# MalvinaNikandrou/mafed

Measured on AMD Instinct MI355X. Metric: train samples/sec VLPythia-410M+MAFED, 256img+32txt tok, bs=32, 1/2/4/8 GPU, higher is better.
Workload: dtype bf16; 1 GPU; VLPythia-410m + MAFED distill step (student fwd+bwd, frozen-teacher fwd, replay CE, 23-layer per-modality MSE, clip 2.0, AdamW), 256 img + 32 txt tokens; global_batch=32, per_gpu_batch=32, seq_len=288, parallelism=dp1, random_init_weights=True

## Files before the change

### include/mafed_hip.h

```cpp
#ifndef MAFED_HIP_H
#define MAFED_HIP_H

#include <stddef.h>
#include <stdint.h>

#ifdef __cplusplus
extern "C" {
#endif

typedef enum { MAFED_F32 = 0, MAFED_BF16 = 1 } mafed_dtype;

enum {
  MAFED_OK = 0,
  MAFED_EINVAL = -1,
  MAFED_ELAUNCH = -2,
  MAFED_EWORKSPACE = -3
};

enum {
  MAFED_EPI_NONE = 0,
  MAFED_EPI_GELU = 1,
  MAFED_EPI_GELU_BWD = 2,
  MAFED_EPI_QUICK_GELU = 3,
  MAFED_EPI_RES1_BF16 = 0x100,
  MAFED_EPI_NO_PERSISTENT = 0x200,
  MAFED_EPI_TICKETED = 0x400
};

int mafed_version(void);
const char* mafed_last_error_string(void);

int mafed_gemm(mafed_dtype in_dtype, int transA, int transB, int64_t M, int64_t N, int64_t K,
               const void* A, int64_t lda, const void* B, int64_t ldb,
               void* C, int64_t ldc, mafed_dtype c_dtype,
               const float* bias, int epilogue, void* aux,
               const float* res1, const float* res2, float beta, void* stream);

int mafed_gemm_colsum(mafed_dtype in_dtype, int transA, int transB, int64_t M, int64_t N, int64_t K,
                      const void* A, int64_t lda, const void* B, int64_t ldb,
                      void* C, int64_t ldc, mafed_dtype c_dtype,
                      const float* bias, int epilogue, void* aux,
                      const float* res1, const float* res2, float beta, float* colsum, void* stream);

typedef struct mafed_gemm_problem {
  int64_t M, N, K;
  const void* A; int64_t lda;
  const void* B; int64_t ldb;
  void* C; int64_t ldc;
  const float* bias; int epilogue; void* aux;
  const float* res1; const float* res2; float beta; float* colsum;
  float* sumsq;
} mafed_gemm_problem;
int mafed_gemm_grouped(mafed_dtype in_dtype, int transA, int transB, mafed_dtype c_dtype,
                       const mafed_gemm_problem* problems, int n, void* stream);

size_t mafed_colsum_workspace_bytes(int64_t M, int64_t N);
int mafed_colsum(const void* X, mafed_dtype dtype, int64_t M, int64_t N, int64_t ldx, float* out,
                 void* workspace, size_t workspace_bytes, void* stream);

int mafed_layernorm_fwd(const float* x, int64_t rows, int h, float eps,
                        const float* w1, const float* b1, void* y1,
                        const float* w2, const float* b2, void* y2,
                        mafed_dtype out_dtype, float* mean, float* rstd, void* stream);
size_t mafed_layernorm_bwd_workspace_bytes(int64_t rows, int h);
int mafed_layernorm_bwd(const void* dy1, const void* dy2, mafed_dtype dy_dtype,
                        const float* x, const float* mean, const float* rstd,
                        const float* w1, const float* w2, int64_t rows, int h,
                        const float* dres, float* dx, void* dx_lp,
                        float* dw1, float* db1, float* dw2, float* db2,
                        const float* teacher, const int64_t* attention_mask, int S, int P, int T,
                        const float* inj_scale_dev , float inj_mul ,
                        float* dxsum_a, float* dxsum_b ,
                        void* workspace, size_t workspace_bytes, void* stream);
int mafed_layernorm_bwd_rows(const void* dy1, const void* dy2, mafed_dtype dy_dtype, const float* x, const float* mean, const float* rstd,
                             const float* w1, const float* w2, int64_t rows, int h, const float* dres, float* dx, void* dx_lp,
                             const float* teacher, const int64_t* attention_mask, int S, int P, int T, const float* inj_scale_dev,
                             float inj_mul, int want_dxsum, void* workspace, size_t workspace_bytes, void* stream);
int mafed_layernorm_bwd_params(int64_t rows, int h, float* dw1, float* db1, float* dw2, float* db2, float* dxsum_a, float* dxsum_b,
                               const void* workspace, size_t workspace_bytes, void* stream);
int mafed_layernorm_bwd_indexed(const void* dy1, const void* dy2, mafed_dtype dy_dtype,
                                const float* x, const float* mean, const float* rstd,
                                const float* w1, const float* w2, int64_t rows, int h,
                                const float* dres, float* dx, void* dx_lp,
                                float* dw1, float* db1, float* dw2, float* db2,
                                const void* teacher, mafed_dtype teacher_dtype, const int* sample_index,
                                const int64_t* attention_mask, int S, int P, int T,
                                const float* inj_scale_dev, float inj_mul, float* dxsum_a, float* dxsum_b,
                                void* workspace, size_t workspace_bytes, void* stream);
int mafed_layernorm_bwd_rows_indexed(const void* dy1, const void* dy2, mafed_dtype dy_dtype, const float* x, const float* mean,
                                     const float* rstd, const float* w1, const float* w2, int64_t rows, int h, const float* dres, float* dx,
                                     void* dx_lp, const void* teacher, mafed_dtype teacher_dtype, const int* sample_index,
                                     const int64_t* attention_mask, int S, int P, int T, const float* inj_scale_dev, float inj_mul,
                                     int want_dxsum, void* workspace, size_t workspace_bytes, void* stream);

int mafed_attn_fwd(const void* qkv, mafed_dtype dtype, int B, int S, int H, int D, int rot,
                   const float* rot_cos, const float* rot_sin, const int64_t* attention_mask, int T,
                   void* out, float* lse, void* stream);
int mafed_attn_bwd(const void* qkv, const void* out, const void* dout, const float* lse, mafed_dtype dtype,
                   int B, int S, int H, int D, int rot, const float* rot_cos, const float* rot_sin,
                   const int64_t* attention_mask, int T, void* dqkv, float* delta, void* stream);
int mafed_attn_bwd_colsum(const void* qkv, const void* out, const void* dout, const float* lse, mafed_dtype dtype,
                          int B, int S, int H, int D, int rot, const float* rot_cos, const float* rot_sin,
                          const int64_t* attention_mask, int T, void* dqkv, float* delta, float* dqkv_colsum, void* stream);

int mafed_attn_decode(const void* qkv_prefix, int S0, const void* qkv_new, int cap, int t, mafed_dtype dtype,
                      int B, int H, int D, int rot, const float* rot_cos, const float* rot_sin,
                      const int64_t* attention_mask, int T, void* out, void* stream);

int mafed_attn_decode_prerot(const void* qkv_prefix, int S0, void* qkv_new, int cap, int t, mafed_dtype dtype,
                             int B, int H, int D, int rot, const float* rot_cos, const float* rot_sin,
                             const int64_t* attention_mask, int T, void* out, void* stream);
int mafed_rotate_k_rows(void* qkv, mafed_dtype dtype, int B, int S, int H, int D, int rot, const float* rot_cos, const float* rot_sin,
                        void* stream);

int mafed_decode_supported(int M, int h, int n1);
int mafed_decode_ln_qkv_fc1(const float* x, int M, int h, float eps, const float* ln1_w, const float* ln1_b, const float* ln2_w,
                            const float* ln2_b, const void* wqkv, const float* bqkv, void* qkv_out, int64_t qkv_ld, const void* w1,
                            const float* b1, int n1, void* a_out, void* stream);
int mafed_decode_ln_linear(const float* x, int M, int h, float eps, const float* ln_w, const float* ln_b, const void* w, const float* bias,
                           int64_t N, void* out, int64_t ldo, void* stream);
size_t mafed_decode_out_workspace_bytes(int M, int h);
int mafed_decode_set_trace(void* buf);
int mafed_attn_decode_set_trace(void* buf);
int mafed_decode_out(const float* x, float* x_out, int M, int h, int n1, const void* ao, const void* act, const void* wd,
                     const float* bd, const void* w2, const float* b2, void* workspace, size_t workspace_bytes, void* stream);

int mafed_beam_candidates(const void* logits, mafed_dtype dtype, int64_t ldl, const float* score, int B, int kin, int V, int k,
                          float* out_score, int64_t* out_token, int* out_parent, void* stream);
int mafed_beam_update(const float* cand_score, const int64_t* cand_token, const int* cand_parent, int B, int k, int step, int cap,
                      int eos, int pad, int early_stopping, float length_penalty, float* run_score, const int* anc_in, int* anc_out,
                      const int64_t* hist_in, int64_t* hist_out, const int64_t* fin_tok_in, int64_t* fin_tok_out,
                      const float* fin_score_in, float* fin_score_out, const int* fin_len_in, int* fin_len_out, int* done,
                      int64_t* next_token, void* stream);
int mafed_attn_decode_beam(const void* qkv_prefix, int S0, void* qkv_new, int cap, int t, mafed_dtype dtype, int B, int k,
                           const int* anc, int H, int D, int rot, const float* rot_cos, const float* rot_sin,
                           const int64_t* attention_mask, int T, void* out, void* stream);

int mafed_attn_suffix_fwd(const void* qkv_img, const int64_t* image_index, int N, int P, const void* qkv_txt, int T, mafed_dtype dtype,
                          int B, int H, int D, int rot, const float* rot_cos, const float* rot_sin, const int64_t* attention_mask,
                          void* out, void* stream);
int mafed_prefix_gather(const void* qkv_img, const void* qkv_txt, const int64_t* image_index, int L, int N, int B, int P, int T, int64_t W,
                        mafed_dtype dtype, void* out, void* stream);

int mafed_attn_cand_fwd(const void* qkv_prefix, int S0, const void* qkv_cand, int C, int A, mafed_dtype dtype, int B, int H, int D, int rot,
                        const float* rot_cos, const float* rot_sin, const int64_t* attention_mask, int T, void* out, void* stream);
int mafed_token_logprob(const void* logits, mafed_dtype dtype, int64_t ldl, const int* logits_row, const int64_t* target, int R, int64_t V,
                        float* out, void* stream);
int mafed_score_reduce(const float* token_logprob, const int64_t* mask, int R, int A, int mean, float* out, void* stream);

int mafed_sample_token(const void* logits, mafed_dtype dtype, int64_t ldl, int R, int V, float temperature, int top_k, float top_p,
                       float min_p, const uint64_t* seed, int step, const float* uniforms, int64_t* unfinished, int eos, int pad,
                       int64_t* token, float* logprob, int* kept, void* stream);

size_t mafed_ewc_workspace_bytes(int64_t n);
int mafed_ewc_penalty_fwd(const float* p, const float* p_old, const float* fisher, int64_t n, float half_lambda, float beta,
                          float* out, void* workspace, size_t workspace_bytes, void* stream);
int mafed_ewc_penalty_bwd(const float* p, const float* p_old, const float* fisher, int64_t n, float lambda,
                          const float* coef_dev, float* grad, void* stream);

size_t mafed_agem_workspace_bytes(int64_t n);
int mafed_agem_blocks(int64_t n);
int mafed_agem_dots(const float* g, const float* r, int64_t n, float* stats4, void* workspace, size_t workspace_bytes, void* stream);
int mafed_agem_project(const float* g, const float* r, float* out, int64_t n, const float* stats4, float* sumsq_partials, void* stream);

int mafed_cka_pool(const float* const* hidden_host, int L, int B, int S, int P, int h, const int64_t* attention_mask, int T,
                   const int64_t* rows, int64_t n, float* out, void* stream);

size_t mafed_cka_stats_workspace_bytes(int64_t G, int64_t n, int64_t h);
int mafed_cka_stats(const float* X, int64_t G, int64_t n, int64_t h, int64_t ldx, int64_t set_stride, double* mean,
                    double* row_sqnorm, void* workspace, size_t workspace_bytes, void* stream);

typedef struct mafed_cka_product {
  const float* X; const double* mean_x; int64_t ldx; int64_t hx;
  const float* Y; const double* mean_y; int64_t ldy; int64_t hy;
  int64_t n;
} mafed_cka_product;

size_t mafed_cka_hsic_workspace_bytes(const mafed_cka_product* products, int count);
int mafed_cka_hsic(const mafed_cka_product* products, int count, double* out, void* workspace, size_t workspace_bytes, void* stream);

int mafed_embed_concat_fwd(const void* image, mafed_dtype img_dtype, const float* embed_in, const int64_t* input_ids,
                           int B, int P, int T, int h, int64_t V, float* h0, void* stream);
int mafed_embed_concat_bwd(const float* dh0, const int64_t* input_ids, int B, int P, int T, int h, int64_t V,
                           void* d_image, mafed_dtype img_dtype, float* d_embed_in, void* stream);

int mafed_ce_fwd(const void* logits, mafed_dtype dtype, const int64_t* labels, int B, int T, int64_t V,
                 float* lse, float* row_loss , float* loss_out, void* stream);
int mafed_ce_fwd_guarded(const void* logits, mafed_dtype dtype, const int64_t* labels, int B, int T, int64_t V,
                         float* lse, float* row_loss, float* loss_out, const int* poison_flag, void* stream);
int mafed_ce_bwd(const void* logits, mafed_dtype dtype, const int64_t* labels, const float* lse, int B, int T, int64_t V,
                 const float* gloss_dev, void* dlogits, void* stream);

int mafed_ce_kd_fwd(const void* student, const void* teacher, mafed_dtype dtype, const int64_t* labels, int B, int T, int64_t V,
                    float tau, float lambda, float* lse3, float* row_ce, float* row_kd, float* out3, const int* poison_flag,
                    void* stream);
int mafed_ce_kd_bwd(const void* student, const void* teacher, mafed_dtype dtype, const int64_t* labels, const float* lse3, int B, int T,
                    int64_t V, float tau, float lambda, const float* gloss_dev, void* dlogits, void* stream);

size_t mafed_distill_workspace_bytes(int64_t rows);
int mafed_distill_fwd(const float* s, const float* t, const int64_t* attention_mask, int B, int S, int P, int h,
                      int cosine, float* out4, void* workspace, size_t workspace_bytes, void* stream);
int mafed_distill_bwd(const float* s, const float* t, const int64_t* attention_mask, int B, int S, int P, int h,
                      int cosine, const float* coef_dev, float* ds, int accumulate, void* stream);
int mafed_distill_combine(const float* sums, int n_layers, const float* layer_coeff_dev, int modality_mode, float lang_weight,
                          const float* lang_weight_vec_dev, float* loss_out, float* per_layer_out, float* modality_out,
                          float* inject_out, void* stream);

int mafed_distill_cls_fwd(const float* s, const float* t, int B, int S, int h, float* out1, void* stream);
int mafed_distill_cls_bwd(const float* s, const float* t, int B, int S, int h, const float* coef_dev, float* ds,
                          int accumulate, void* stream);
int mafed_distill_fwd_indexed(const float* s, const void* teacher, mafed_dtype teacher_dtype, const int* sample_index,
                              const int64_t* attention_mask, int B, int S, int P, int h, int cosine, float* out4,
                              void* workspace, size_t workspace_bytes, void* stream);
int mafed_distill_bwd_indexed(const float* s, const void* teacher, mafed_dtype teacher_dtype, const int* sample_index,
                              const int64_t* attention_mask, int B, int S, int P, int h, int cosine, const float* coef_dev,
                              float* ds, int accumulate, void* stream);
int mafed_distill_cls_fwd_indexed(const float* s, const void* teacher, mafed_dtype teacher_dtype, const int* sample_index,
                                  int B, int S, int h, float* out1, void* stream);
int mafed_distill_cls_bwd_indexed(const float* s, const void* teacher, mafed_dtype teacher_dtype, const int* sample_index,
                                  int B, int S, int h, const float* coef_dev, float* ds, int accumulate, void* stream);

size_t mafed_gradnorm_workspace_bytes(int64_t n);
int mafed_gradnorm_clip(const float* g, int64_t n, float max_norm, float* out2, void* workspace, size_t workspace_bytes,
                        void* stream);
int mafed_gradnorm_blocks(int64_t n);
int mafed_gradnorm_partial(const float* g, int64_t n, float* partial_out, void* stream);
int mafed_gradnorm_finish(const float* partial, int n_partials, float max_norm, float* out2, void* stream);
int mafed_adamw_step(float* p, const float* g, float* m, float* v, int64_t n, const float* lr_dev, float beta1, float beta2,
                     float eps, float weight_decay, int step, const float* clip_dev ,
                     float grad_mul, void* p_bf16, void* stream);

int mafed_adamw_step_zero_grad(float* p, float* g, float* m, float* v, int64_t n, const float* lr_dev, float beta1, float beta2,
                               float eps, float weight_decay, int step, const float* clip_scale_dev, float grad_mul, void* p_bf16,
                               void* stream);

int mafed_adamw_step_partial_zero(float* p, float* g, float* m, float* v, int64_t n, const float* lr_dev, float beta1, float beta2,
                                  float eps, float weight_decay, int step, const float* clip_scale_dev, float grad_mul, void* p_bf16,
                                  int64_t zero_n, void* stream);

int mafed_adam_step(float* p, float* g, float* m, float* v, int64_t n, const float* lr_dev, double beta1, double beta2, float eps,
                    float weight_decay, int step, const float* clip_dev, float grad_mul, void* p_bf16, int64_t zero_n, void* stream);
int mafed_adamax_step(float* p, float* g, float* m, float* u, int64_t n, const float* lr_dev, double beta1, double beta2, float eps,
                      float weight_decay, int step, const float* clip_dev, float grad_mul, void* p_bf16, int64_t zero_n, void* stream);

int mafed_optim_advance(int64_t* state_dev, double base_lr, int64_t warmup_steps, int64_t total_steps, double beta1, double beta2,
                        float* hyper3_dev, void* stream);

int mafed_optim_advance_guarded(int64_t* state_dev, double base_lr, int64_t warmup_steps, int64_t total_steps, double beta1, double beta2,
                                float* hyper3_dev, const float* clip_dev, void* stream);

int mafed_sumsq_accumulate(const float* x, int64_t n, float* sumsq16, void* stream);
int mafed_gemm_grouped_fuses_sumsq(mafed_dtype in_dtype, int transA, int transB, mafed_dtype c_dtype, const int64_t* M, const int64_t* N,
                                   const int64_t* K, int n);

int mafed_gradnorm_finish_advance(const float* partial, int n_partials, float max_norm, float* out2, float* norm_log, int64_t* state_dev,
                                  double base_lr, int64_t warmup_steps, int64_t total_steps, double beta1, double beta2, float* hyper3_dev,
                                  void* stream);

int mafed_cast(const void* src, mafed_dtype src_dtype, void* dst, mafed_dtype dst_dtype, int64_t n, void* stream);
int mafed_pad_text_rows(const float* src, int B, int S, int P, int h, float* dst, void* dst_lp, void* stream);
int mafed_label_rows(const int64_t* labels, int B, int T, int Rc, int* row_of_slot, int* slot_of_row, int64_t* labels_c, int* overflow,
                     void* stream);
int mafed_gather_rows(const void* src, mafed_dtype dtype, const int* idx, int64_t n_out, int h, void* dst, void* stream);
int mafed_pad_text_batch(const int64_t* ids, const int64_t* mask, const int64_t* labels, int B, int T, int Tp, int64_t* ids_out,
                         int64_t* mask_out, int64_t* labels_out, void* stream);
int mafed_gelu(const void* x, void* y, mafed_dtype dtype, int64_t n, void* stream);

int mafed_patchify(const void* pixels, mafed_dtype pix_dtype, int B, int C, int H, int W, int patch, int64_t rows_out, int k_pad,
                   void* out, mafed_dtype out_dtype, void* stream);
int mafed_vit_assemble(const void* patch_emb, mafed_dtype pe_dtype, int64_t ld_pe, const float* class_embedding,
                       const float* position_embedding, int B, int num_patches, int h, float* tokens, void* stream);
int mafed_attn_fwd_bidir(const void* qkv, mafed_dtype dtype, int B, int S, int H, int D, void* out, float* lse, void* stream);

int mafed_prof_begin(int max_records);
int mafed_prof_end(void);
int mafed_prof_collect(int* tags_host, double* work_host, float* ms_host, float* start_ms_host, int max);
const char* mafed_prof_tag_name(int tag);

int mafed_gemm_set_variant(int variant);
int mafed_gemm_get_variant(int which);
int mafed_gemm_pp_launches(void);
int mafed_gemm_fallback_launches(void);

int mafed_attn_set_variant(int variant);

int mafed_attn_fwd_exact_bf16(const void* qkv, int B, int S, int H, int D, int rot, const float* rot_cos, const float* rot_sin,
                              const int64_t* attention_mask, int T, void* out, float* lse, void* stream);

int mafed_tune_occupy(int blocks, int lds_bytes, long long cycles, void* stream);

int mafed_tune_stream(const void* src, void* dst, long long n_bytes, int blocks, int threads, int unroll, int mode, void* stream);
int mafed_tune_stream_for(const void* src, void* dst, long long n_bytes, int blocks, int threads, double microseconds, void* stream);

#ifdef __cplusplus
}
#endif
#endif
```

### mafed_amd/_lib.py

```python
from __future__ import annotations

import ctypes as C
import os
from typing import Optional

_HERE = os.path.dirname(os.path.abspath(__file__))
LIB_PATH = os.environ.get("MAFED_HIP_LIB") or os.path.join(_HERE, "libmafed_hip.so")

F32, BF16 = 0, 1
EPI_NONE, EPI_GELU, EPI_GELU_BWD, EPI_QUICK_GELU = 0, 1, 2, 3
EPI_RES1_BF16 = 0x100
EPI_NO_PERSISTENT = 0x200
EPI_TICKETED = 0x400

_p, _i, _l, _f, _z, _d = C.c_void_p, C.c_int, C.c_int64, C.c_float, C.c_size_t, C.c_double

SIGNATURES = {
    "mafed_version": (_i, []),
    "mafed_last_error_string": (C.c_char_p, []),
    "mafed_gemm": (_i, [_i, _i, _i, _l, _l, _l, _p, _l, _p, _l, _p, _l, _i, _p, _i, _p, _p, _p, _f, _p]),
    "mafed_gemm_colsum": (_i, [_i, _i, _i, _l, _l, _l, _p, _l, _p, _l, _p, _l, _i, _p, _i, _p, _p, _p, _f, _p, _p]),
    "mafed_gemm_grouped": (_i, [_i, _i, _i, _i, _p, _i, _p]),
    "mafed_gemm_set_variant": (_i, [_i]),
    "mafed_gemm_get_variant": (_i, [_i]),
    "mafed_gemm_pp_launches": (_i, []),
    "mafed_gemm_fallback_launches": (_i, []),
    "mafed_attn_decode": (_i, [_p, _i, _p, _i, _i, _i, _i, _i, _i, _i, _p, _p, _p, _i, _p, _p]),
    "mafed_attn_decode_prerot": (_i, [_p, _i, _p, _i, _i, _i, _i, _i, _i, _i, _p, _p, _p, _i, _p, _p]),
    "mafed_rotate_k_rows": (_i, [_p, _i, _i, _i, _i, _i, _i, _p, _p, _p]),
    "mafed_gemm_grouped_fuses_sumsq": (_i, [_i, _i, _i, _i, _p, _p, _p, _i]),
    "mafed_decode_supported": (_i, [_i, _i, _i]),
    "mafed_decode_ln_qkv_fc1": (_i, [_p, _i, _i, _f, _p, _p, _p, _p, _p, _p, _p, _l, _p, _p, _i, _p, _p]),
    "mafed_decode_ln_linear": (_i, [_p, _i, _i, _f, _p, _p, _p, _p, _l, _p, _l, _p]),
    "mafed_decode_out_workspace_bytes": (_z, [_i, _i]),
    "mafed_decode_set_trace": (_i, [_p]),
    "mafed_attn_decode_set_trace": (_i, [_p]),
    "mafed_decode_out": (_i, [_p, _p, _i, _i, _i, _p, _p, _p, _p, _p, _p, _p, _z, _p]),
    "mafed_beam_candidates": (_i, [_p, _i, _l, _p, _i, _i, _i, _i, _p, _p, _p, _p]),
    "mafed_beam_update": (_i, [_p, _p, _p, _i, _i, _i, _i, _i, _i, _i, _f, _p, _p, _p, _p, _p, _p, _p, _p, _p, _p, _p, _p, _p, _p]),
    "mafed_attn_decode_beam": (_i, [_p, _i, _p, _i, _i, _i, _i, _i, _p, _i, _i, _i, _p, _p, _p, _i, _p, _p]),
    "mafed_attn_suffix_fwd": (_i, [_p, _p, _i, _i, _p, _i, _i, _i, _i, _i, _i, _p, _p, _p, _p, _p]),
    "mafed_prefix_gather": (_i, [_p, _p, _p, _i, _i, _i, _i, _i, _l, _i, _p, _p]),
    "mafed_attn_cand_fwd": (_i, [_p, _i, _p, _i, _i, _i, _i, _i, _i, _i, _p, _p, _p, _i, _p, _p]),
    "mafed_token_logprob": (_i, [_p, _i, _l, _p, _p, _i, _l, _p, _p]),
    "mafed_score_reduce": (_i, [_p, _p, _i, _i, _i, _p, _p]),
    "mafed_sample_token": (_i, [_p, _i, _l, _i, _i, _f, _i, _f, _f, _p, _i, _p, _p, _i, _i, _p, _p, _p, _p]),
    "mafed_ewc_workspace_bytes": (_z, [_l]),
    "mafed_ewc_penalty_fwd": (_i, [_p, _p, _p, _l, _f, _f, _p, _p, _z, _p]),
    "mafed_ewc_penalty_bwd": (_i, [_p, _p, _p, _l, _f, _p, _p, _p]),
    "mafed_agem_workspace_bytes": (_z, [_l]),
    "mafed_agem_blocks": (_i, [_l]),
    "mafed_agem_dots": (_i, [_p, _p, _l, _p, _p, _z, _p]),
    "mafed_agem_project": (_i, [_p, _p, _p, _l, _p, _p, _p]),
    "mafed_cka_pool": (_i, [_p, _i, _i, _i, _i, _i, _p, _i, _p, _l, _p, _p]),
    "mafed_cka_stats_workspace_bytes": (_z, [_l, _l, _l]),
    "mafed_cka_stats": (_i, [_p, _l, _l, _l, _l, _l, _p, _p, _p, _z, _p]),
    "mafed_cka_hsic_workspace_bytes": (_z, [_p, _i]),
    "mafed_cka_hsic": (_i, [_p, _i, _p, _p, _z, _p]),
    "mafed_colsum_workspace_bytes": (_z, [_l, _l]),
    "mafed_colsum": (_i, [_p, _i, _l, _l, _l, _p, _p, _z, _p]),
    "mafed_layernorm_fwd": (_i, [_p, _l, _i, _f, _p, _p, _p, _p, _p, _p, _i, _p, _p, _p]),
    "mafed_layernorm_bwd_workspace_bytes": (_z, [_l, _i]),
    "mafed_layernorm_bwd": (_i, [_p, _p, _i, _p, _p, _p, _p, _p, _l, _i, _p, _p, _p, _p, _p, _p, _p, _p, _p, _i, _i, _i, _p, _f, _p, _p, _p, _z, _p]),
    "mafed_layernorm_bwd_rows": (_i, [_p, _p, _i, _p, _p, _p, _p, _p, _l, _i, _p, _p, _p, _p, _p, _i, _i, _i, _p, _f, _i, _p, _z, _p]),
    "mafed_layernorm_bwd_params": (_i, [_l, _i, _p, _p, _p, _p, _p, _p, _p, _z, _p]),
    "mafed_layernorm_bwd_indexed": (_i, [_p, _p, _i, _p, _p, _p, _p, _p, _l, _i, _p, _p, _p, _p, _p, _p, _p, _p, _i, _p, _p, _i, _i, _i, _p, _f, _p, _p,
                                         _p, _z, _p]),
    "mafed_layernorm_bwd_rows_indexed": (_i, [_p, _p, _i, _p, _p, _p, _p, _p, _l, _i, _p, _p, _p, _p, _i, _p, _p, _i, _i, _i, _p, _f, _i, _p, _z, _p]),
    "mafed_attn_fwd": (_i, [_p, _i, _i, _i, _i, _i, _i, _p, _p, _p, _i, _p, _p, _p]),
    "mafed_attn_bwd": (_i, [_p, _p, _p, _p, _i, _i, _i, _i, _i, _i, _p, _p, _p, _i, _p, _p, _p]),
    "mafed_attn_bwd_colsum": (_i, [_p, _p, _p, _p, _i, _i, _i, _i, _i, _i, _p, _p, _p, _i, _p, _p, _p, _p]),
    "mafed_attn_set_variant": (_i, [_i]),
    "mafed_attn_fwd_exact_bf16": (_i, [_p, _i, _i, _i, _i, _i, _p, _p, _p, _i, _p, _p, _p]),
    "mafed_embed_concat_fwd": (_i, [_p, _i, _p, _p, _i, _i, _i, _i, _l, _p, _p]),
    "mafed_embed_concat_bwd": (_i, [_p, _p, _i, _i, _i, _i, _l, _p, _i, _p, _p]),
    "mafed_ce_fwd": (_i, [_p, _i, _p, _i, _i, _l, _p, _p, _p, _p]),
    "mafed_ce_fwd_guarded": (_i, [_p, _i, _p, _i, _i, _l, _p, _p, _p, _p, _p]),
    "mafed_ce_bwd": (_i, [_p, _i, _p, _p, _i, _i, _l, _p, _p, _p]),
    "mafed_ce_kd_fwd": (_i, [_p, _p, _i, _p, _i, _i, _l, _f, _f, _p, _p, _p, _p, _p, _p]),
    "mafed_ce_kd_bwd": (_i, [_p, _p, _i, _p, _p, _i, _i, _l, _f, _f, _p, _p, _p]),
    "mafed_distill_workspace_bytes": (_z, [_l]),
    "mafed_distill_fwd": (_i, [_p, _p, _p, _i, _i, _i, _i, _i, _p, _p, _z, _p]),
    "mafed_distill_bwd": (_i, [_p, _p, _p, _i, _i, _i, _i, _i, _p, _p, _i, _p]),
    "mafed_distill_cls_fwd": (_i, [_p, _p, _i, _i, _i, _p, _p]),
    "mafed_distill_cls_bwd": (_i, [_p, _p, _i, _i, _i, _p, _p, _i, _p]),
    "mafed_distill_fwd_indexed": (_i, [_p, _p, _i, _p, _p, _i, _i, _i, _i, _i, _p, _p, _z, _p]),
    "mafed_distill_bwd_indexed": (_i, [_p, _p, _i, _p, _p, _i, _i, _i, _i, _i, _p, _p, _i, _p]),
    "mafed_distill_cls_fwd_indexed": (_i, [_p, _p, _i, _p, _i, _i, _i, _p, _p]),
    "mafed_distill_cls_bwd_indexed": (_i, [_p, _p, _i, _p, _i, _i, _i, _p, _p, _i, _p]),
    "mafed_gradnorm_workspace_bytes": (_z, [_l]),
    "mafed_gradnorm_clip": (_i, [_p, _l, _f, _p, _p, _z, _p]),
    "mafed_gradnorm_blocks": (_i, [_l]),
    "mafed_gradnorm_partial": (_i, [_p, _l, _p, _p]),
    "mafed_gradnorm_finish": (_i, [_p, _i, _f, _p, _p]),
    "mafed_sumsq_accumulate": (_i, [_p, _l, _p, _p]),
    "mafed_adamw_step": (_i, [_p, _p, _p, _p, _l, _p, _f, _f, _f, _f, _i, _p, _f, _p, _p]),
    "mafed_adamw_step_zero_grad": (_i, [_p, _p, _p, _p, _l, _p, _f, _f, _f, _f, _i, _p, _f, _p, _p]),
    "mafed_adamw_step_partial_zero": (_i, [_p, _p, _p, _p, _l, _p, _f, _f, _f, _f, _i, _p, _f, _p, _l, _p]),
    "mafed_adam_step": (_i, [_p, _p, _p, _p, _l, _p, _d, _d, _f, _f, _i, _p, _f, _p, _l, _p]),
    "mafed_adamax_step": (_i, [_p, _p, _p, _p, _l, _p, _d, _d, _f, _f, _i, _p, _f, _p, _l, _p]),
    "mafed_distill_combine": (_i, [_p, _i, _p, _i, _f, _p, _p, _p, _p, _p, _p]),
    "mafed_optim_advance": (_i, [_p, _d, _l, _l, _d, _d, _p, _p]),
    "mafed_optim_advance_guarded": (_i, [_p, _d, _l, _l, _d, _d, _p, _p, _p]),
    "mafed_tune_occupy": (_i, [_i, _i, C.c_longlong, _p]),
    "mafed_tune_stream": (_i, [_p, _p, C.c_longlong, _i, _i, _i, _i, _p]),
    "mafed_tune_stream_for": (_i, [_p, _p, C.c_longlong, _i, _i, _d, _p]),
    "mafed_gradnorm_finish_advance": (_i, [_p, _i, _f, _p, _p, _p, _d, _l, _l, _d, _d, _p, _p]),
    "mafed_cast": (_i, [_p, _i, _p, _i, _l, _p]),
    "mafed_pad_text_rows": (_i, [_p, _i, _i, _i, _i, _p, _p, _p]),
    "mafed_label_rows": (_i, [_p, _i, _i, _i, _p, _p, _p, _p, _p]),
    "mafed_gather_rows": (_i, [_p, _i, _p, _l, _i, _p, _p]),
    "mafed_pad_text_batch": (_i, [_p, _p, _p, _i, _i, _i, _p, _p, _p, _p]),
    "mafed_gelu": (_i, [_p, _p, _i, _l, _p]),
    "mafed_patchify": (_i, [_p, _i, _i, _i, _i, _i, _i, _l, _i, _p, _i, _p]),
    "mafed_vit_assemble": (_i, [_p, _i, _l, _p, _p, _i, _i, _i, _p, _p]),
    "mafed_attn_fwd_bidir": (_i, [_p, _i, _i, _i, _i, _i, _p, _p, _p]),
    "mafed_prof_begin": (_i, [_i]),
    "mafed_prof_end": (_i, []),
    "mafed_prof_collect": (_i, [_p, _p, _p, _p, _i]),
    "mafed_prof_tag_name": (C.c_char_p, [_i]),
}



class GemmProblem(C.Structure):
    _fields_ = [("M", _l), ("N", _l), ("K", _l), ("A", _p), ("lda", _l), ("B", _p), ("ldb", _l), ("C", _p), ("ldc", _l),
                ("bias", _p), ("epilogue", _i), ("aux", _p), ("res1", _p), ("res2", _p), ("beta", _f), ("colsum", _p), ("sumsq", _p)]


class CkaProduct(C.Structure):
    _fields_ = [("X", _p), ("mean_x", _p), ("ldx", _l), ("hx", _l), ("Y", _p), ("mean_y", _p), ("ldy", _l), ("hy", _l), ("n", _l)]


_lib: Optional[C.CDLL] = None


class MafedHipError(RuntimeError):
    pass


def load() -> C.CDLL:
    global _lib
    if _lib is not None:
        return _lib
    if not os.path.exists(LIB_PATH):
        raise MafedHipError(
            f"{LIB_PATH} is missing: build it with `python -m mafed_amd.build` (or __graft_entry__.build()). "
            "mafed_amd has no CPU fallback.")
    lib = C.CDLL(LIB_PATH)
    loose = bool(os.environ.get("MAFED_HIP_LIB")) and os.environ.get("MAFED_HIP_LIB_LOOSE") == "1"
    for name, (res, args) in SIGNATURES.items():
        if loose and not hasattr(lib, name):
            continue
        fn = getattr(lib, name)
        fn.restype = res
        fn.argtypes = args
    _lib = lib
    return lib


def check(rc: int, what: str = "") -> None:
    if rc != 0:
        msg = load().mafed_last_error_string()
        raise MafedHipError(f"{what or 'mafed call'} failed (rc={rc}): {msg.decode() if msg else ''}")
```

### mafed_amd/csrc/attn.h

```cpp
#pragma once
#include "common.h"

namespace mafed {

struct AttnShape {
  int B, S, H, D, rot, T, P;
  int causal = 1;
};

template <typename T>
__device__ __forceinline__ float rot_elem(const T* __restrict__ row, int d, int rot, const float* __restrict__ c, const float* __restrict__ s) {
  const float x = Elem<T>::load(row + d);
  if (d >= rot) return x;
  const int half = rot >> 1;
  if (d < half) return x * c[d] - Elem<T>::load(row + d + half) * s[d];
  return x * c[d - half] + Elem<T>::load(row + d - half) * s[d - half];
}
__device__ __forceinline__ bool key_valid(const int64_t* __restrict__ am, int b, int j, int P, int T) {
  return j < P || am[(int64_t)b * T + (j - P)] != 0;
}

template <typename T>
struct AttnKey {
  const T* row;
  int pos;
  bool visible;
};
template <typename T, typename Key>
__device__ __forceinline__ void attn_exact_row(const float* __restrict__ qrow, float* __restrict__ sc, int nk, int D, int rot,
                                               const float* __restrict__ rc, const float* __restrict__ rs, Key key, T* __restrict__ op,
                                               int lane, float& m, float& l) {
  const int half = rot >> 1;
  const float scale = rsqrtf((float)D);
  m = -INFINITY;
  for (int k = lane; k < nk; k += 64) {
    float s = -INFINITY;
    const AttnKey<T> kk = key(k);
    if (kk.visible) {
      float acc = 0.f;
      for (int d = 0; d < D; ++d)
        acc = fmaf(qrow[d], rot_elem(kk.row + D, d, rot, rc + (int64_t)kk.pos * half, rs + (int64_t)kk.pos * half), acc);
      s = acc * scale;
    }
    sc[k] = s;
    m = fmaxf(m, s);
  }
  m = wave_max(m);
  l = 0.f;
  for (int k = lane; k < nk; k += 64) {
    const float p = expf(sc[k] - m);
    sc[k] = p;
    l += p;
  }
  l = wave_sum(l);
  __builtin_amdgcn_wave_barrier();
  const float inv = 1.0f / l;
  for (int d = lane; d < D; d += 64) {
    float acc = 0.f;
    for (int k = 0; k < nk; ++k) acc = fmaf(sc[k], Elem<T>::load(key(k).row + 2 * D + d), acc);
    Elem<T>::store(op + d, acc * inv);
  }
}

template <typename T>
int attn_ref_fwd_launch(const void* qkv, const AttnShape& sh, const float* rc, const float* rs, const int64_t* am, void* out, float* lse,
                        hipStream_t st);
template <typename T>
int attn_ref_bwd_launch(const void* qkv, const void* out, const void* dout, const float* lse, const AttnShape& sh, const float* rc,
                        const float* rs, const int64_t* am, void* dqkv, float* delta, hipStream_t st);

template <typename T>
int attn_decode_launch(const void* qkv_pre, int S0, const void* qkv_new, int cap, int t, int B, int H, int D, int rot, int P, int Tm,
                       const float* rc, const float* rs, const int64_t* am, void* out, hipStream_t st, bool prerot = false);
template <typename T>
int rotate_k_rows_launch(void* qkv, int64_t rows, int S, int H, int D, int rot, const float* rc, const float* rs, hipStream_t st);

int attn_mfma_fwd_launch(const void* qkv, const AttnShape& sh, const float* rc, const float* rs, const int64_t* am, void* out, float* lse,
                         hipStream_t st);
int attn_mfma_bwd_launch(const void* qkv, const void* out, const void* dout, const float* lse, const AttnShape& sh, const float* rc,
                         const float* rs, const int64_t* am, void* dqkv, float* delta, float* colsum, bool* colsum_done, hipStream_t st);

struct SuffixShape {
  int B, N, P, T, H, D, rot;
};
__device__ __forceinline__ int64_t suffix_image(const int64_t* __restrict__ image_index, int b, int N) {
  const int64_t n = image_index ? image_index[b] : (int64_t)b;
  return n < 0 ? 0 : (n >= N ? N - 1 : n);
}
template <typename T>
int attn_suffix_ref_launch(const void* qkv_img, const int64_t* image_index, const void* qkv_txt, const SuffixShape& sh, const float* rc,
                           const float* rs, const int64_t* am, void* out, hipStream_t st);
int attn_suffix_mfma_launch(const void* qkv_img, const int64_t* image_index, const void* qkv_txt, const SuffixShape& sh, const float* rc,
                            const float* rs, const int64_t* am, void* out, hipStream_t st);
int prefix_gather_launch(const void* img, const void* txt, const int64_t* image_index, int L, int N, int B, int P, int T, int64_t row_bytes,
                         void* out, hipStream_t st);

struct CandShape {
  int B, C, A, S0, T, H, D, rot;
};
template <typename T>
int attn_cand_ref_launch(const void* qkv_pre, const void* qkv_cand, const CandShape& sh, const float* rc, const float* rs, const int64_t* am,
                         void* out, hipStream_t st);
int attn_cand_mfma_launch(const void* qkv_pre, const void* qkv_cand, const CandShape& sh, const float* rc, const float* rs, const int64_t* am,
                          void* out, hipStream_t st);

void attn_mfma_set_variant(int v);

int attn_decode_set_trace(void* buf);

}
```

### mafed_amd/csrc/attn.hip

```cpp
#include "attn.h"

using namespace mafed;

static int check_common(const char* who, const void* qkv, int B, int S, int H, int D, int rot, const float* rc, const float* rs,
                        const int64_t* am, int T) {
  MAFED_CHECK_ARG(qkv && am, "%s: null pointer", who);
  MAFED_CHECK_ARG(B > 0 && S > 0 && H > 0 && D > 0 && T >= 0 && T <= S, "%s: bad shape B=%d S=%d H=%d D=%d T=%d", who, B, S, H, D, T);
  MAFED_CHECK_ARG(rot >= 0 && rot <= D && rot % 2 == 0, "%s: rotary dims %d invalid for D=%d", who, rot, D);
  MAFED_CHECK_ARG(rot == 0 || (rc && rs), "%s: rotary tables missing", who);
  return MAFED_OK;
}

static bool mfma_ok(int D, int rot) { return (D == 64 || D == 128 || D == 256) && (rot == 0 || rot == 16 || rot == 32 || rot == 64) && rot * 2 <= D * 2; }

extern "C" int mafed_attn_fwd(const void* qkv, mafed_dtype dtype, int B, int S, int H, int D, int rot, const float* rot_cos,
                              const float* rot_sin, const int64_t* attention_mask, int T, void* out, float* lse, void* stream) {
  int rc = check_common("attn_fwd", qkv, B, S, H, D, rot, rot_cos, rot_sin, attention_mask, T);
  if (rc) return rc;
  MAFED_CHECK_ARG(out && lse, "attn_fwd: null output");
  AttnShape sh{B, S, H, D, rot, T, S - T};
  hipStream_t st = as_stream(stream);
  if (dtype == MAFED_F32) {
    MAFED_CHECK_ARG(D <= 256, "attn_fwd(f32): D=%d > 256", D);
    rc = attn_ref_fwd_launch<float>(qkv, sh, rot_cos, rot_sin, attention_mask, out, lse, st);
// ... 10 lines not shown
}

extern "C" int mafed_attn_suffix_fwd(const void* qkv_img, const int64_t* image_index, int N, int P, const void* qkv_txt, int T,
                                     mafed_dtype dtype, int B, int H, int D, int rot, const float* rot_cos, const float* rot_sin,
                                     const int64_t* attention_mask, void* out, void* stream) {
  MAFED_CHECK_ARG(qkv_img && qkv_txt && attention_mask && out, "attn_suffix_fwd: null pointer");
  MAFED_CHECK_ARG(B > 0 && N > 0 && P > 0 && T > 0 && H > 0 && D > 0 && D <= 256, "attn_suffix_fwd: bad shape B=%d N=%d P=%d T=%d H=%d D=%d", B, N,
                  P, T, H, D);
  MAFED_CHECK_ARG(image_index || N == B, "attn_suffix_fwd: no image_index needs N == B (N=%d B=%d)", N, B);
  MAFED_CHECK_ARG(rot >= 0 && rot <= D && rot % 2 == 0 && (rot == 0 || (rot_cos && rot_sin)), "attn_suffix_fwd: rotary arguments invalid");
  SuffixShape sh{B, N, P, T, H, D, rot};
  hipStream_t st = as_stream(stream);
  int rc;
  if (dtype == MAFED_F32) {
    rc = attn_suffix_ref_launch<float>(qkv_img, image_index, qkv_txt, sh, rot_cos, rot_sin, attention_mask, out, st);
  } else if (mfma_ok(D, rot)) {
    MAFED_CHECK_ARG((((uintptr_t)qkv_img | (uintptr_t)qkv_txt | (uintptr_t)out) & 15) == 0, "attn_suffix_fwd(bf16): qkv/out must be 16-byte aligned");
    rc = attn_suffix_mfma_launch(qkv_img, image_index, qkv_txt, sh, rot_cos, rot_sin, attention_mask, out, st);
  } else {
    rc = attn_suffix_ref_launch<bf16_t>(qkv_img, image_index, qkv_txt, sh, rot_cos, rot_sin, attention_mask, out, st);
  }
  if (rc) return rc;
  MAFED_CHECK_LAUNCH("attn_suffix_fwd");
  return MAFED_OK;
}

extern "C" int mafed_attn_cand_fwd(const void* qkv_prefix, int S0, const void* qkv_cand, int C, int A, mafed_dtype dtype, int B, int H, int D,
                                   int rot, const float* rot_cos, const float* rot_sin, const int64_t* attention_mask, int T, void* out,
                                   void* stream) {
  MAFED_CHECK_ARG(qkv_prefix && qkv_cand && out, "attn_cand_fwd: null pointer");
  MAFED_CHECK_ARG(B > 0 && C > 0 && A > 0 && H > 0 && D > 0 && D <= 256 && (int64_t)C * A <= 0x7fffffffLL,
                  "attn_cand_fwd: bad shape B=%d C=%d A=%d H=%d D=%d", B, C, A, H, D);
  MAFED_CHECK_ARG(S0 > 0 && T >= 0 && T < S0, "attn_cand_fwd: the prefix needs an image key in front of its text (S0=%d T=%d)", S0, T);
  MAFED_CHECK_ARG(attention_mask || T == 0, "attn_cand_fwd: attention_mask missing (T=%d)", T);
  MAFED_CHECK_ARG(rot >= 0 && rot <= D && rot % 2 == 0 && (rot == 0 || (rot_cos && rot_sin)), "attn_cand_fwd: rotary arguments invalid");
  CandShape sh{B, C, A, S0, T, H, D, rot};
  hipStream_t st = as_stream(stream);
  int rc;
  if (dtype == MAFED_F32) {
    rc = attn_cand_ref_launch<float>(qkv_prefix, qkv_cand, sh, rot_cos, rot_sin, attention_mask, out, st);
  } else if (mfma_ok(D, rot) && (((uintptr_t)qkv_prefix | (uintptr_t)qkv_cand | (uintptr_t)out) & 15) == 0) {
    rc = attn_cand_mfma_launch(qkv_prefix, qkv_cand, sh, rot_cos, rot_sin, attention_mask, out, st);
  } else {
    rc = attn_cand_ref_launch<bf16_t>(qkv_prefix, qkv_cand, sh, rot_cos, rot_sin, attention_mask, out, st);
  }
  if (rc) return rc;
  MAFED_CHECK_LAUNCH("attn_cand_fwd");
  return MAFED_OK;
}

extern "C" int mafed_prefix_gather(const void* qkv_img, const void* qkv_txt, const int64_t* image_index, int L, int N, int B, int P, int T,
                                   int64_t W, mafed_dtype dtype, void* out, void* stream) {
  MAFED_CHECK_ARG(qkv_img && qkv_txt && out, "prefix_gather: null pointer");
  MAFED_CHECK_ARG(L > 0 && N > 0 && B > 0 && P > 0 && T > 0 && W > 0, "prefix_gather: bad shape L=%d N=%d B=%d P=%d T=%d", L, N, B, P, T);
  MAFED_CHECK_ARG(image_index || N == B, "prefix_gather: no image_index needs N == B (N=%d B=%d)", N, B);
  MAFED_CHECK_ARG((((uintptr_t)qkv_img | (uintptr_t)qkv_txt | (uintptr_t)out) & 15) == 0, "prefix_gather: tensors must be 16-byte aligned");
  int rc = prefix_gather_launch(qkv_img, qkv_txt, image_index, L, N, B, P, T, W * (dtype == MAFED_F32 ? 4 : 2), out, as_stream(stream));
  if (rc) return rc;
  MAFED_CHECK_LAUNCH("prefix_gather");
  return MAFED_OK;
}

extern "C" int mafed_attn_fwd_bidir(const void* qkv, mafed_dtype dtype, int B, int S, int H, int D, void* out, float* lse, void* stream) {
  MAFED_CHECK_ARG(qkv && out && lse, "attn_fwd_bidir: null pointer");
  MAFED_CHECK_ARG(B > 0 && S > 0 && H > 0 && D > 0 && D <= 256, "attn_fwd_bidir: bad shape B=%d S=%d H=%d D=%d", B, S, H, D);
  AttnShape sh{B, S, H, D, 0, 0, S};
  sh.causal = 0;
  const int64_t* dummy_mask = reinterpret_cast<const int64_t*>(qkv);
  hipStream_t st = as_stream(stream);
  int rc;
  if (dtype == MAFED_F32) {
    rc = attn_ref_fwd_launch<float>(qkv, sh, nullptr, nullptr, dummy_mask, out, lse, st);
  } else {
    MAFED_CHECK_ARG((((uintptr_t)qkv | (uintptr_t)out) & 15) == 0, "attn_fwd_bidir(bf16): qkv/out must be 16-byte aligned");
    rc = attn_mfma_fwd_launch(qkv, sh, nullptr, nullptr, dummy_mask, out, lse, st);
  }
  if (rc) return rc;
  MAFED_CHECK_LAUNCH("attn_fwd_bidir");
  return MAFED_OK;
}

static int attn_bwd_impl(const void* qkv, const void* out, const void* dout, const float* lse, mafed_dtype dtype, int B, int S, int H,
                         int D, int rot, const float* rot_cos, const float* rot_sin, const int64_t* attention_mask, int T, void* dqkv,
                         float* delta, float* dqkv_colsum, void* stream);

extern "C" int mafed_attn_bwd(const void* qkv, const void* out, const void* dout, const float* lse, mafed_dtype dtype, int B, int S, int H,
                              int D, int rot, const float* rot_cos, const float* rot_sin, const int64_t* attention_mask, int T, void* dqkv,
                              float* delta, void* stream) {
  return attn_bwd_impl(qkv, out, dout, lse, dtype, B, S, H, D, rot, rot_cos, rot_sin, attention_mask, T, dqkv, delta, nullptr, stream);
}

extern "C" int mafed_attn_bwd_colsum(const void* qkv, const void* out, const void* dout, const float* lse, mafed_dtype dtype, int B, int S,
                                     int H, int D, int rot, const float* rot_cos, const float* rot_sin, const int64_t* attention_mask, int T,
                                     void* dqkv, float* delta, float* dqkv_colsum, void* stream) {
  return attn_bwd_impl(qkv, out, dout, lse, dtype, B, S, H, D, rot, rot_cos, rot_sin, attention_mask, T, dqkv, delta, dqkv_colsum, stream);
}

static int attn_bwd_impl(const void* qkv, const void* out, const void* dout, const float* lse, mafed_dtype dtype, int B, int S, int H,
                         int D, int rot, const float* rot_cos, const float* rot_sin, const int64_t* attention_mask, int T, void* dqkv,
                         float* delta, float* dqkv_colsum, void* stream) {
  int rc = check_common("attn_bwd", qkv, B, S, H, D, rot, rot_cos, rot_sin, attention_mask, T);
  if (rc) return rc;
  MAFED_CHECK_ARG(out && dout && lse && dqkv && delta, "attn_bwd: null pointer");
  AttnShape sh{B, S, H, D, rot, T, S - T};
  hipStream_t st = as_stream(stream);
  bool colsum_done = false;
  if (dtype == MAFED_F32) {
    MAFED_CHECK_ARG(D <= 256, "attn_bwd(f32): D=%d > 256", D);
    rc = attn_ref_bwd_launch<float>(qkv, out, dout, lse, sh, rot_cos, rot_sin, attention_mask, dqkv, delta, st);
  } else if (mfma_ok(D, rot)) {
    MAFED_CHECK_ARG((((uintptr_t)qkv | (uintptr_t)out | (uintptr_t)dout | (uintptr_t)dqkv) & 15) == 0,
                    "attn_bwd(bf16): tensors must be 16-byte aligned");
    rc = attn_mfma_bwd_launch(qkv, out, dout, lse, sh, rot_cos, rot_sin, attention_mask, dqkv, delta, dqkv_colsum, &colsum_done, st);
  } else {
    MAFED_CHECK_ARG(D <= 256, "attn_bwd(bf16): D=%d > 256", D);
    rc = attn_ref_bwd_launch<bf16_t>(qkv, out, dout, lse, sh, rot_cos, rot_sin, attention_mask, dqkv, delta, st);
  }
  if (rc) return rc;
  MAFED_CHECK_LAUNCH("attn_bwd");
  if (dqkv_colsum && !colsum_done)
    return mafed_colsum(dqkv, dtype, (int64_t)B * S, (int64_t)3 * H * D, (int64_t)3 * H * D, dqkv_colsum, nullptr, 0, stream);
  return MAFED_OK;
}

extern "C" int mafed_attn_set_variant(int variant) {
  attn_mfma_set_variant(variant);
  return MAFED_OK;
}

extern "C" int mafed_attn_fwd_exact_bf16(const void* qkv, int B, int S, int H, int D, int rot, const float* rot_cos, const float* rot_sin,
                                         const int64_t* attention_mask, int T, void* out, float* lse, void* stream) {
  int rc = check_common("attn_fwd_exact_bf16", qkv, B, S, H, D, rot, rot_cos, rot_sin, attention_mask, T);
  if (rc) return rc;
  AttnShape sh{B, S, H, D, rot, T, S - T};
  rc = attn_ref_fwd_launch<bf16_t>(qkv, sh, rot_cos, rot_sin, attention_mask, out, lse, as_stream(stream));
  if (rc) return rc;
  MAFED_CHECK_LAUNCH("attn_fwd_exact_bf16");
  return MAFED_OK;
}

static int attn_decode_impl(const void* qkv_prefix, int S0, const void* qkv_new, int cap, int t, mafed_dtype dtype, int B, int H, int D,
                            int rot, const float* rot_cos, const float* rot_sin, const int64_t* attention_mask, int T, void* out,
                            void* stream, bool prerot) {
  MAFED_CHECK_ARG(qkv_prefix && qkv_new && out && attention_mask, "attn_decode: null pointer");
  MAFED_CHECK_ARG(B > 0 && H > 0 && D > 0 && D <= 256 && S0 > 0 && T >= 0 && T <= S0 && cap > 0 && t >= 0 && t < cap,
                  "attn_decode: bad shape B=%d H=%d D=%d S0=%d T=%d cap=%d t=%d", B, H, D, S0, T, cap, t);
  MAFED_CHECK_ARG(rot >= 0 && rot <= D && rot % 2 == 0 && (rot == 0 || (rot_cos && rot_sin)), "attn_decode: rotary arguments invalid");
  hipStream_t st = as_stream(stream);
  int rc = dtype == MAFED_F32 ? attn_decode_launch<float>(qkv_prefix, S0, qkv_new, cap, t, B, H, D, rot, S0 - T, T, rot_cos, rot_sin, attention_mask, out, st, prerot)
                              : attn_decode_launch<bf16_t>(qkv_prefix, S0, qkv_new, cap, t, B, H, D, rot, S0 - T, T, rot_cos, rot_sin, attention_mask, out, st, prerot);
  if (rc) return rc;
  MAFED_CHECK_LAUNCH("attn_decode");
  return MAFED_OK;
}

extern "C" int mafed_attn_decode(const void* qkv_prefix, int S0, const void* qkv_new, int cap, int t, mafed_dtype dtype, int B, int H, int D,
                                 int rot, const float* rot_cos, const float* rot_sin, const int64_t* attention_mask, int T, void* out,
                                 void* stream) {
  return attn_decode_impl(qkv_prefix, S0, qkv_new, cap, t, dtype, B, H, D, rot, rot_cos, rot_sin, attention_mask, T, out, stream, false);
}

extern "C" int mafed_attn_decode_prerot(const void* qkv_prefix, int S0, void* qkv_new, int cap, int t, mafed_dtype dtype, int B, int H, int D,
                                        int rot, const float* rot_cos, const float* rot_sin, const int64_t* attention_mask, int T, void* out,
                                        void* stream) {
  MAFED_CHECK_ARG(rot % 16 == 0 && (D == 64 || D == 128 || D == 256), "attn_decode_prerot: needs rot %% 16 == 0 and a head size of 64 / 128 / 256");
  return attn_decode_impl(qkv_prefix, S0, qkv_new, cap, t, dtype, B, H, D, rot, rot_cos, rot_sin, attention_mask, T, out, stream, true);
}

extern "C" int mafed_rotate_k_rows(void* qkv, mafed_dtype dtype, int B, int S, int H, int D, int rot, const float* rot_cos, const float* rot_sin,
                                   void* stream) {
  MAFED_CHECK_ARG(qkv && B > 0 && S > 0 && H > 0 && D > 0 && rot >= 0 && rot <= D && rot % 16 == 0 && (rot == 0 || (rot_cos && rot_sin)),
                  "rotate_k_rows: bad arguments");
  hipStream_t st = as_stream(stream);
  int rc = dtype == MAFED_F32 ? rotate_k_rows_launch<float>(qkv, (int64_t)B * S, S, H, D, rot, rot_cos, rot_sin, st)
                              : rotate_k_rows_launch<bf16_t>(qkv, (int64_t)B * S, S, H, D, rot, rot_cos, rot_sin, st);
  if (rc) return rc;
  MAFED_CHECK_LAUNCH("rotate_k_rows");
  return MAFED_OK;
}

extern "C" int mafed_attn_decode_set_trace(void* buf) { return mafed::attn_decode_set_trace(buf); }
```

### mafed_amd/csrc/attn_mfma.hip

```cpp
#include <type_traits>

#include "attn.h"
#include "row8.h"

namespace mafed {

namespace {

typedef __attribute__((address_space(3))) bf16x4* lds_bf16x4_ptr;

template <int D>
__device__ __forceinline__ int swz(int row) {
  if (D == 64) return ((row >> 1) & 3) << 1;
  if (D == 128) return (row & 7) << 1;
  return ((row & 7) << 1) | ((row >> 3) & 1);
}
template <int D>
__device__ __forceinline__ int tile_off(int row, int chunk) {
  if (D == 64) return row * 128 + ((chunk ^ swz<64>(row)) << 4);
  if (D == 128) return row * 256 + ((chunk ^ swz<128>(row)) << 4);
  return row * 512 + ((chunk ^ (((row & 7) << 1) | ((row >> 3) & 1))) << 4);
}

__device__ __forceinline__ uint4 load_chunk_rot(const bf16_t* __restrict__ rowp, int chunk, int rot, const float* __restrict__ rc,
// ... 494 lines not shown
  const int k0 = kt * 64 + wave * 16;
  const int mykey = k0 + (lane & 15);
  const int g = lane >> 4;
  const bool mykey_ok = key_ok(am, b, mykey, P, T, S);

  bf16x8 kf[D / 32], vf[D / 32];
  load_col_frags<D, true>(kf, kb, rstride, k0, S, rot, rc, rs, lane);
  load_col_frags<D, false>(vf, vb, rstride, k0, S, 0, rc, rs, lane);
  f32x4 dk[D / 16], dv[D / 16];
#pragma unroll
  for (int i = 0; i < D / 16; ++i) { dk[i] = (f32x4){0.f, 0.f, 0.f, 0.f}; dv[i] = (f32x4){0.f, 0.f, 0.f, 0.f}; }
  const float scale = rsqrtf((float)D);
  const int64_t lbase = ((int64_t)b * H + h) * S;

  for (int qt = kt; qt < nqt; ++qt) {
    __syncthreads();
    stage_rows<D, 64, true>(qimg, qb, rstride, qt * 64, S, rot, rc, rs, tid);
    stage_rows<D, 64, false>(doimg, dob, ostride, qt * 64, S, 0, rc, rs, tid);
    if (tid < 64) {
      const int q = qt * 64 + tid;
      Ls[tid] = q < S ? lse[lbase + q] : 0.f;
      dls[tid] = q < S ? delta[lbase + q] : 0.f;
    }
    __syncthreads();
    f32x4 p[4], ds[4];
#pragma unroll
    for (int j = 0; j < 4; ++j) {
      f32x4 s = (f32x4){0.f, 0.f, 0.f, 0.f}, dp = (f32x4){0.f, 0.f, 0.f, 0.f};
#pragma unroll
      for (int ks = 0; ks < D / 32; ++ks) {
        s = __builtin_amdgcn_mfma_f32_16x16x32_bf16(frag_row<D>(qimg, j, ks, lane), kf[ks], s, 0, 0, 0);
        dp = __builtin_amdgcn_mfma_f32_16x16x32_bf16(frag_row<D>(doimg, j, ks, lane), vf[ks], dp, 0, 0, 0);
      }
      const float4 Lq = *reinterpret_cast<const float4*>(Ls + j * 16 + 4 * g);
      const float4 Dq = *reinterpret_cast<const float4*>(dls + j * 16 + 4 * g);
      const float La[4] = {Lq.x, Lq.y, Lq.z, Lq.w}, Da[4] = {Dq.x, Dq.y, Dq.z, Dq.w};
#pragma unroll
      for (int r = 0; r < 4; ++r) {
        const int q = qt * 64 + j * 16 + 4 * g + r;
        float pv = __expf(s[r] * scale - La[r]);
        if (!mykey_ok || mykey > q || q >= S) pv = 0.f;
        p[j][r] = pv;
        ds[j][r] = pv * (dp[r] - Da[r]) * scale;
      }
    }
    const bf16x8 p0 = pack_acc(p[0], p[1]), p1 = pack_acc(p[2], p[3]);
    const bf16x8 d0 = pack_acc(ds[0], ds[1]), d1 = pack_acc(ds[2], ds[3]);
#pragma unroll
    for (int dt = 0; dt < D / 16; ++dt) {
      dv[dt] = __builtin_amdgcn_mfma_f32_16x16x32_bf16(frag_tr<D>(doimg, dt, 0, lane), p0, dv[dt], 0, 0, 0);
      dv[dt] = __builtin_amdgcn_mfma_f32_16x16x32_bf16(frag_tr<D>(doimg, dt, 1, lane), p1, dv[dt], 0, 0, 0);
      dk[dt] = __builtin_amdgcn_mfma_f32_16x16x32_bf16(frag_tr<D>(qimg, dt, 0, lane), d0, dk[dt], 0, 0, 0);
      dk[dt] = __builtin_amdgcn_mfma_f32_16x16x32_bf16(frag_tr<D>(qimg, dt, 1, lane), d1, dk[dt], 0, 0, 0);
    }
  }
  bf16_t* dkp = dqkv + ((int64_t)b * S * H + h) * 3 * D + (int64_t)mykey * rstride + D;
  store_grad_unrot<D>(dkp, dk, rot, rc, rs, mykey, lane, mykey < S);
  if (mykey < S) {
    bf16_t* dvp = dkp + D;
#pragma unroll
    for (int dt = 0; dt < D / 16; ++dt) store4(dvp + dt * 16 + 4 * g, make_float4(dv[dt][0], dv[dt][1], dv[dt][2], dv[dt][3]));
  }
}

typedef __attribute__((address_space(3))) void* lds_void_ptr;
typedef const __attribute__((address_space(1))) void* glb_void_ptr;
typedef unsigned u32x2 __attribute__((ext_vector_type(2)));

__device__ __forceinline__ float col_max_sw(float v) {
  u32x2 r = __builtin_amdgcn_permlane32_swap(__float_as_uint(v), __float_as_uint(v), false, false);
  v = fmaxf(__uint_as_float(r[0]), __uint_as_float(r[1]));
  r = __builtin_amdgcn_permlane16_swap(__float_as_uint(v), __float_as_uint(v), false, false);
  return fmaxf(__uint_as_float(r[0]), __uint_as_float(r[1]));
}
__device__ __forceinline__ float col_sum_sw(float v) {
  u32x2 r = __builtin_amdgcn_permlane32_swap(__float_as_uint(v), __float_as_uint(v), false, false);
  v = __uint_as_float(r[0]) + __uint_as_float(r[1]);
  r = __builtin_amdgcn_permlane16_swap(__float_as_uint(v), __float_as_uint(v), false, false);
  return __uint_as_float(r[0]) + __uint_as_float(r[1]);
}

template <int D, int NW = 4>
__device__ __forceinline__ void dma_rows(char* __restrict__ img, const bf16_t* __restrict__ base, int64_t rstride, int nrows, int S, int wave,
                                         int lane) {
  constexpr int RPP = 1024 / (2 * D);
  const int npieces = nrows / RPP;
  for (int j = wave; j < npieces; j += NW) {
    int row, logical;
    if (D == 64) {
      row = j * 8 + (lane >> 3);
      logical = (lane & 7) ^ swz<64>(row);
    } else {
      row = j * 4 + (lane >> 4);
      logical = (lane & 15) ^ swz<128>(row);
    }
    const int srow = row < S ? row : S - 1;
    __builtin_amdgcn_global_load_lds((glb_void_ptr)(base + (int64_t)srow * rstride + logical * 8), (lds_void_ptr)(img + j * 1024), 16, 0, 0);
  }
}

struct RotPre {
  float4 c0, c1, s0, s1;
};
__device__ __forceinline__ void rot_pre_load(RotPre& r, int it, int hc, int rot, const float* __restrict__ rc, const float* __restrict__ rs) {
  const int row = it / hc, c = it - row * hc;
  const float* cp = rc + (int64_t)row * (rot >> 1) + c * 8;
  const float* sp = rs + (int64_t)row * (rot >> 1) + c * 8;
  r.c0 = load4(cp); r.c1 = load4(cp + 4); r.s0 = load4(sp); r.s1 = load4(sp + 4);
}
template <int D>
__device__ __forceinline__ void rot_apply(char* __restrict__ img, int it, int hc, const RotPre& r) {
  const int row = it / hc, c = it - row * hc;
  uint4* p1 = reinterpret_cast<uint4*>(img + tile_off<D>(row, c));
  uint4* p2 = reinterpret_cast<uint4*>(img + tile_off<D>(row, c + hc));
  float x1[8], x2[8], o1[8], o2[8];
  unpack8(*p1, x1);
  unpack8(*p2, x2);
  const float cs[8] = {r.c0.x, r.c0.y, r.c0.z, r.c0.w, r.c1.x, r.c1.y, r.c1.z, r.c1.w};
  const float sn[8] = {r.s0.x, r.s0.y, r.s0.z, r.s0.w, r.s1.x, r.s1.y, r.s1.z, r.s1.w};
#pragma unroll
  for (int e = 0; e < 8; ++e) {
    o1[e] = x1[e] * cs[e] - x2[e] * sn[e];
    o2[e] = x2[e] * cs[e] + x1[e] * sn[e];
  }
  *p1 = pack8(o1);
  *p2 = pack8(o2);
}
template <int D, int NT = 256>
__device__ __forceinline__ void rot_fix_rows(char* __restrict__ img, int items, int hc, int rot, const float* __restrict__ rc,
                                             const float* __restrict__ rs, const RotPre (&pre)[2], int tid) {
#pragma unroll
  for (int u = 0; u < 2; ++u)
    if (tid + NT * u < items) rot_apply<D>(img, tid + NT * u, hc, pre[u]);
  for (int it = tid + 2 * NT; it < items; it += NT) {
    RotPre r;
    rot_pre_load(r, it, hc, rot, rc, rs);
    rot_apply<D>(img, it, hc, r);
  }
}

__device__ __forceinline__ float row16_sum(float v) {
  v += __builtin_bit_cast(float, __builtin_amdgcn_update_dpp(0, __builtin_bit_cast(int, v), 0xB1, 0xF, 0xF, true));
  v += __builtin_bit_cast(float, __builtin_amdgcn_update_dpp(0, __builtin_bit_cast(int, v), 0x4E, 0xF, 0xF, true));
  v += __builtin_bit_cast(float, __builtin_amdgcn_update_dpp(0, __builtin_bit_cast(int, v), 0x141, 0xF, 0xF, true));
  v += __builtin_bit_cast(float, __builtin_amdgcn_update_dpp(0, __builtin_bit_cast(int, v), 0x140, 0xF, 0xF, true));
  return v;
}

__device__ __forceinline__ void wait_vm0() { asm volatile("s_waitcnt vmcnt(0)" ::: "memory"); }

__device__ __forceinline__ int snake4(int w, int t) { return t * 4 + ((t & 1) ? 3 - w : w); }
template <int NW>
__device__ __forceinline__ int snake(int w, int t) { return t * NW + ((t & 1) ? NW - 1 - w : w); }

#define MAFED_LOG2E 1.4426950408889634f
#define MAFED_LN2 0.6931471805599453f

template <int D>
constexpr int attn_fwd_waves() { return D == 64 ? 8 : 4; }

template <int D, bool CAUSAL = true>
__global__ __launch_bounds__(attn_fwd_waves<D>() * 64, (D == 64 ? 2 : 1) * attn_fwd_waves<D>() / 4) void attn_fwd_res_kernel(const bf16_t* __restrict__ qkv, AttnShape sh, const float* __restrict__ rc,
                                                           const float* __restrict__ rs, const int64_t* __restrict__ am,
                                                           bf16_t* __restrict__ out, float* __restrict__ lse) {
  extern __shared__ __attribute__((aligned(16))) char lds[];
  constexpr int NW = attn_fwd_waves<D>(), NTH = NW * 64;
  const int tid = threadIdx.x, lane = tid & 63;
  const int wave = __builtin_amdgcn_readfirstlane(tid >> 6);
  const int S = sh.S, H = sh.H, rot = sh.rot, P = sh.P, T = sh.T;
  const int h = blockIdx.x, b = blockIdx.y;
  const int nrows = (S + 31) / 32 * 32;
  char* kimg = lds;
  char* vimg = lds + nrows * D * 2;
  float* kbias = reinterpret_cast<float*>(lds + 2 * nrows * D * 2);
  const int64_t rstride = (int64_t)H * 3 * D;
  const bf16_t* qb = qkv + ((int64_t)b * S * H + h) * 3 * D;
  const bf16_t* kb = qb + D;
  const bf16_t* vb = qb + 2 * D;
  const int nslices = (S + 15) / 16;
// ... 48 lines not shown
      constexpr bool MASK = decltype(mask_tag)::value;
      f32x4 s[4];
#pragma unroll
      for (int j = 0; j < 4; ++j) {
        s[j] = (f32x4){0.f, 0.f, 0.f, 0.f};
        if (!MASK || j < nj) {
#pragma unroll
          for (int ks = 0; ks < D / 32; ++ks)
            s[j] = __builtin_amdgcn_mfma_f32_16x16x32_bf16(frag_row<D>(kimg, kt * 4 + j, ks, lane), qf[ks], s[j], 0, 0, 0);
        }
      }
      float tmax = -INFINITY;
      if (MASK) {
#pragma unroll
        for (int j = 0; j < 4; ++j) {
          if (j < nj) {
            const float4 kb4 = *reinterpret_cast<const float4*>(kbias + kt * 64 + j * 16 + 4 * g);
            const float kbv[4] = {kb4.x, kb4.y, kb4.z, kb4.w};
#pragma unroll
            for (int r = 0; r < 4; ++r) {
              const int key = kt * 64 + j * 16 + 4 * g + r;
              float v = s[j][r] * scale2 + kbv[r];
              if (CAUSAL) v = key > myq ? -INFINITY : v;
              s[j][r] = v;
              tmax = fmaxf(tmax, v);
            }
          } else {
            s[j] = (f32x4){-INFINITY, -INFINITY, -INFINITY, -INFINITY};
          }
        }
      } else {
#pragma unroll
        for (int j = 0; j < 4; ++j)
#pragma unroll
          for (int r = 0; r < 4; ++r) tmax = fmaxf(tmax, s[j][r]);
        tmax *= scale2;
      }
      tmax = col_max_sw(tmax);
      if (__builtin_amdgcn_ballot_w64(tmax - m > 8.0f) != 0) {
        const float mn = fmaxf(m, tmax);
        const float alpha = __builtin_amdgcn_exp2f(m - mn);
        m = mn;
        lsum *= alpha;
#pragma unroll
        for (int i = 0; i < D / 16; ++i) o[i] *= alpha;
      }
#pragma unroll
      for (int j = 0; j < 4; ++j)
#pragma unroll
        for (int r = 0; r < 4; ++r) s[j][r] = __builtin_amdgcn_exp2f(MASK ? s[j][r] - m : fmaf(s[j][r], scale2, -m));
      const bf16x8 p0 = pack_acc(s[0], s[1]);
      lsum = __builtin_amdgcn_mfma_f32_16x16x32_bf16(ones, p0, lsum, 0, 0, 0);
#pragma unroll
      for (int dt = 0; dt < D / 16; ++dt) o[dt] = __builtin_amdgcn_mfma_f32_16x16x32_bf16(frag_tr<D>(vimg, dt, kt * 2, lane), p0, o[dt], 0, 0, 0);
      if (!MASK || nj > 2) {
        const bf16x8 p1 = pack_acc(s[2], s[3]);
        lsum = __builtin_amdgcn_mfma_f32_16x16x32_bf16(ones, p1, lsum, 0, 0, 0);
#pragma unroll
        for (int dt = 0; dt < D / 16; ++dt)
          o[dt] = __builtin_amdgcn_mfma_f32_16x16x32_bf16(frag_tr<D>(vimg, dt, kt * 2 + 1, lane), p1, o[dt], 0, 0, 0);
      }
    };
    const int kt_plain = CAUSAL ? (last_kt < P / 64 ? last_kt : P / 64) : (P / 64 <= last_kt ? P / 64 : last_kt + 1);
    const int klast = CAUSAL ? q0 + 15 : S - 1;
    for (int kt = 0; kt < kt_plain; ++kt) tile(kt, 4, std::false_type{});
    for (int kt = kt_plain; kt <= last_kt; ++kt) tile(kt, kt == last_kt ? ((klast - kt * 64) >> 4) + 1 : 4, std::true_type{});
    const float l = lsum[0];
    if (myq < S) {
      const float inv = 1.0f / l;
      bf16_t* op = out + ((int64_t)b * S + myq) * H * D + (int64_t)h * D;
#pragma unroll
      for (int dt = 0; dt < D / 16; ++dt)
        store4(op + dt * 16 + 4 * g, make_float4(o[dt][0] * inv, o[dt][1] * inv, o[dt][2] * inv, o[dt][3] * inv));
      if (g == 0) lse[((int64_t)b * H + h) * S + myq] = m * MAFED_LN2 + logf(l);
    }
  }
}

template <int D, int NW = 4>
__global__ __launch_bounds__(NW * 64, (D == 64 ? 2 : 1) * NW / 4) void attn_bwd_dq_res_kernel(const bf16_t* __restrict__ qkv, const bf16_t* __restrict__ out,
                                                              const bf16_t* __restrict__ dout, const float* __restrict__ lse, AttnShape sh,
                                                              const float* __restrict__ rc, const float* __restrict__ rs,
                                                              const int64_t* __restrict__ am, bf16_t* __restrict__ dqkv,
                                                              float* __restrict__ delta, float* __restrict__ bsum) {
  extern __shared__ __attribute__((aligned(16))) char lds[];
  constexpr int NTH = NW * 64;
  const int tid = threadIdx.x, lane = tid & 63;
  const int wave = __builtin_amdgcn_readfirstlane(tid >> 6);
  const int S = sh.S, H = sh.H, rot = sh.rot, P = sh.P, T = sh.T;
  const int h = blockIdx.x, b = blockIdx.y;
  const int nrows = (S + 31) / 32 * 32;
  char* kimg = lds;
  char* vimg = lds + nrows * D * 2;
  float* kbias = reinterpret_cast<float*>(lds + 2 * nrows * D * 2);
  float* red = kbias + 2 * nrows;
  if (bsum && tid < D) red[tid] = 0.f;
  const int64_t rstride = (int64_t)H * 3 * D;
  const bf16_t* qb = qkv + ((int64_t)b * S * H + h) * 3 * D;
  const bf16_t* kb = qb + D;
  const bf16_t* vb = qb + 2 * D;
  const int64_t ostride = (int64_t)H * D;
  const bf16_t* ob = out + (int64_t)b * S * ostride + (int64_t)h * D;
  const bf16_t* dob = dout + (int64_t)b * S * ostride + (int64_t)h * D;
  const float* Lrow = lse + ((int64_t)b * H + h) * S;
  const int nslices = (S + 15) / 16;
  const int hc = rot >> 4, items = S * hc;
  dma_rows<D, NW>(kimg, kb, rstride, nrows, S, wave, lane);
  dma_rows<D, NW>(vimg, vb, rstride, nrows, S, wave, lane);
  RotPre pre[2];
#pragma unroll
  for (int u = 0; u < 2; ++u)
    if (tid + NTH * u < items) rot_pre_load(pre[u], tid + NTH * u, hc, rot, rc, rs);
  for (int k = tid; k < nrows; k += NTH) kbias[k] = key_ok(am, b, k, P, T, S) ? 0.f : -INFINITY;
  constexpr bool PREFETCH = NW == 4;
  ColRaw<D> qraw, doraw, oraw;
  float Lnext = 0.f;
  if (PREFETCH) {
    const int s0 = nslices - 1 - snake<NW>(wave, 0);
    if (s0 >= 0) {
      col_raw_issue<D, true>(qraw, qb, rstride, s0 * 16, S, rot, rc, rs, lane);
      col_raw_issue<D, false>(doraw, dob, ostride, s0 * 16, S, 0, rc, rs, lane);
      col_raw_issue<D, false>(oraw, ob, ostride, s0 * 16, S, 0, rc, rs, lane);
      const int q = s0 * 16 + (lane & 15);
      Lnext = q < S ? Lrow[q] : 0.f;
    }
  }
  wait_vm0();
  __syncthreads();
  rot_fix_rows<D, NTH>(kimg, items, hc, rot, rc, rs, pre, tid);
  __syncthreads();
  const int g = lane >> 4;
  const float scale = rsqrtf((float)D);
  const float scale2 = scale * MAFED_LOG2E;
  for (int t = 0;; ++t) {
    const int slice = nslices - 1 - snake<NW>(wave, t);
    if (slice < 0) break;
    const int q0 = slice * 16;
    const int myq = q0 + (lane & 15);
    if (!PREFETCH) {
      col_raw_issue<D, true>(qraw, qb, rstride, q0, S, rot, rc, rs, lane);
      col_raw_issue<D, false>(doraw, dob, ostride, q0, S, 0, rc, rs, lane);
      col_raw_issue<D, false>(oraw, ob, ostride, q0, S, 0, rc, rs, lane);
      Lnext = myq < S ? Lrow[myq] : 0.f;
    }
    bf16x8 qf[D / 32], dof[D / 32];
    col_raw_finish<D, true>(qf, qraw, q0, S, rot, lane);
    col_raw_finish<D, false>(dof, doraw, q0, S, 0, lane);
    const float L2 = Lnext * MAFED_LOG2E;
    float dl = 0.f;
    {
      bf16x8 of[D / 32];
      col_raw_finish<D, false>(of, oraw, q0, S, 0, lane);
      const int nxt = nslices - 1 - snake<NW>(wave, t + 1);
      if (PREFETCH && nxt >= 0) {
        col_raw_issue<D, true>(qraw, qb, rstride, nxt * 16, S, rot, rc, rs, lane);
        col_raw_issue<D, false>(doraw, dob, ostride, nxt * 16, S, 0, rc, rs, lane);
        col_raw_issue<D, false>(oraw, ob, ostride, nxt * 16, S, 0, rc, rs, lane);
        const int q = nxt * 16 + (lane & 15);
        Lnext = q < S ? Lrow[q] : 0.f;
      }
#pragma unroll
      for (int ks = 0; ks < D / 32; ++ks)
#pragma unroll
        for (int e = 0; e < 8; ++e) dl += (float)dof[ks][e] * (float)of[ks][e];
      dl = col_sum_sw(dl);
    }
    if (myq < S && g == 0) delta[((int64_t)b * H + h) * S + myq] = dl;
    f32x4 dq[D / 16];
#pragma unroll
    for (int i = 0; i < D / 16; ++i) dq[i] = (f32x4){0.f, 0.f, 0.f, 0.f};
    const int last_kt = (q0 + 15) / 64;
    auto tile = [&](const int kt, const int nj, auto mask_tag) {
      constexpr bool MASK = decltype(mask_tag)::value;
      f32x4 ds[4];
#pragma unroll
      for (int j = 0; j < 4; ++j) {
        ds[j] = (f32x4){0.f, 0.f, 0.f, 0.f};
        if (!MASK || j < nj) {
          f32x4 s = (f32x4){0.f, 0.f, 0.f, 0.f}, dp = (f32x4){0.f, 0.f, 0.f, 0.f};
#pragma unroll
          for (int ks = 0; ks < D / 32; ++ks) {
            s = __builtin_amdgcn_mfma_f32_16x16x32_bf16(frag_row<D>(kimg, kt * 4 + j, ks, lane), qf[ks], s, 0, 0, 0);
            dp = __builtin_amdgcn_mfma_f32_16x16x32_bf16(frag_row<D>(vimg, kt * 4 + j, ks, lane), dof[ks], dp, 0, 0, 0);
          }
          if (MASK) {
            const float4 kb4 = *reinterpret_cast<const float4*>(kbias + kt * 64 + j * 16 + 4 * g);
            const float kbv[4] = {kb4.x, kb4.y, kb4.z, kb4.w};
#pragma unroll
            for (int r = 0; r < 4; ++r) {
              const int key = kt * 64 + j * 16 + 4 * g + r;
              float x = s[r] * scale2 - L2 + kbv[r];
              x = key > myq ? -INFINITY : x;
              ds[j][r] = __builtin_amdgcn_exp2f(x) * (dp[r] - dl) * scale;
            }
          } else {
#pragma unroll
            for (int r = 0; r < 4; ++r) ds[j][r] = __builtin_amdgcn_exp2f(s[r] * scale2 - L2) * (dp[r] - dl) * scale;
          }
        }
      }
      const bf16x8 d0 = pack_acc(ds[0], ds[1]);
#pragma unroll
      for (int dt = 0; dt < D / 16; ++dt) dq[dt] = __builtin_amdgcn_mfma_f32_16x16x32_bf16(frag_tr<D>(kimg, dt, kt * 2, lane), d0, dq[dt], 0, 0, 0);
      if (!MASK || nj > 2) {
        const bf16x8 d1 = pack_acc(ds[2], ds[3]);
#pragma unroll
        for (int dt = 0; dt < D / 16; ++dt)
          dq[dt] = __builtin_amdgcn_mfma_f32_16x16x32_bf16(frag_tr<D>(kimg, dt, kt * 2 + 1, lane), d1, dq[dt], 0, 0, 0);
      }
    };
    const int kt_plain = last_kt < P / 64 ? last_kt : P / 64;
    for (int kt = 0; kt < kt_plain; ++kt) tile(kt, 4, std::false_type{});
    for (int kt = kt_plain; kt <= last_kt; ++kt) tile(kt, kt == last_kt ? ((q0 + 15 - kt * 64) >> 4) + 1 : 4, std::true_type{});
    bf16_t* dqp = dqkv + ((int64_t)b * S * H + h) * 3 * D + (int64_t)myq * rstride;
    store_grad_unrot<D>(dqp, dq, rot, rc, rs, myq, lane, myq < S);
    if (bsum) {
#pragma unroll
      for (int dt = 0; dt < D / 16; ++dt)
#pragma unroll
        for (int r = 0; r < 4; ++r) {
          const float v = row16_sum(myq < S ? dq[dt][r] : 0.f);
          if ((lane & 15) == 0) atomicAdd(red + dt * 16 + 4 * g + r, v);
        }
    }
  }
  if (bsum) {
    __syncthreads();
    if (tid < D) atomicAdd(bsum + (int64_t)h * 3 * D + tid, red[tid]);
  }
}

template <int D, int NW = 4>
__global__ __launch_bounds__(NW * 64, (D == 64 ? 2 : 1) * NW / 4) void attn_bwd_dkv_res_kernel(const bf16_t* __restrict__ qkv, const bf16_t* __restrict__ dout,
                                                               const float* __restrict__ lse, const float* __restrict__ delta, AttnShape sh,
                                                               const float* __restrict__ rc, const float* __restrict__ rs,
                                                               const int64_t* __restrict__ am, bf16_t* __restrict__ dqkv,
                                                               float* __restrict__ bsum) {
  extern __shared__ __attribute__((aligned(16))) char lds[];
  constexpr int NTH = NW * 64;
  const int tid = threadIdx.x, lane = tid & 63;
  const int wave = __builtin_amdgcn_readfirstlane(tid >> 6);
  const int S = sh.S, H = sh.H, rot = sh.rot, P = sh.P, T = sh.T;
  const int h = blockIdx.x, b = blockIdx.y;
  const int nrows = (S + 31) / 32 * 32;
  char* qimg = lds;
  char* doimg = lds + nrows * D * 2;
  float* L2s = reinterpret_cast<float*>(lds + 2 * nrows * D * 2);
  float* Ds = L2s + nrows;
  float* red = Ds + nrows;
  if (bsum && tid < 2 * D) red[tid] = 0.f;
  const int64_t rstride = (int64_t)H * 3 * D;
  const bf16_t* qb = qkv + ((int64_t)b * S * H + h) * 3 * D;
  const bf16_t* kb = qb + D;
  const bf16_t* vb = qb + 2 * D;
  const int64_t ostride = (int64_t)H * D;
  const bf16_t* dob = dout + (int64_t)b * S * ostride + (int64_t)h * D;
  const float* Lrow = lse + ((int64_t)b * H + h) * S;
  const float* Drow = delta + ((int64_t)b * H + h) * S;
  const int nslices = (S + 15) / 16;
  const int hc = rot >> 4, items = S * hc;
  dma_rows<D, NW>(qimg, qb, rstride, nrows, S, wave, lane);
  dma_rows<D, NW>(doimg, dob, ostride, nrows, S, wave, lane);
  RotPre pre[2];
#pragma unroll
  for (int u = 0; u < 2; ++u)
    if (tid + NTH * u < items) rot_pre_load(pre[u], tid + NTH * u, hc, rot, rc, rs);
  for (int q = tid; q < nrows; q += NTH) {
    L2s[q] = q < S ? Lrow[q] * MAFED_LOG2E : INFINITY;
    Ds[q] = q < S ? Drow[q] : 0.f;
  }
  ColRaw<D> kraw, vraw;
  {
    const int s0 = snake<NW>(wave, 0);
    if (s0 < nslices) {
      col_raw_issue<D, true>(kraw, kb, rstride, s0 * 16, S, rot, rc, rs, lane);
      col_raw_issue<D, false>(vraw, vb, rstride, s0 * 16, S, 0, rc, rs, lane);
    }
  }
  wait_vm0();
  __syncthreads();
  rot_fix_rows<D, NTH>(qimg, items, hc, rot, rc, rs, pre, tid);
  __syncthreads();
  const int g = lane >> 4;
  const float scale = rsqrtf((float)D);
  const float scale2 = scale * MAFED_LOG2E;
  const int nqt = (nrows + 63) / 64;
  for (int t = 0;; ++t) {
    const int slice = snake<NW>(wave, t);
    if (slice >= nslices) break;
    const int k0 = slice * 16;
    const int mykey = k0 + (lane & 15);
    const int mykey_eff = key_ok(am, b, mykey, P, T, S) ? mykey : 0x7fffffff;
    bf16x8 kf[D / 32], vf[D / 32];
    col_raw_finish<D, true>(kf, kraw, k0, S, rot, lane);
    col_raw_finish<D, false>(vf, vraw, k0, S, 0, lane);
    {
      const int nxt = snake<NW>(wave, t + 1);
      if (nxt < nslices) {
        col_raw_issue<D, true>(kraw, kb, rstride, nxt * 16, S, rot, rc, rs, lane);
        col_raw_issue<D, false>(vraw, vb, rstride, nxt * 16, S, 0, rc, rs, lane);
      }
    }
    f32x4 dk[D / 16], dv[D / 16];
#pragma unroll
    for (int i = 0; i < D / 16; ++i) { dk[i] = (f32x4){0.f, 0.f, 0.f, 0.f}; dv[i] = (f32x4){0.f, 0.f, 0.f, 0.f}; }
    const int qt0 = k0 / 64;
    const bool text_keys = k0 + 15 >= P;
    auto tile = [&](const int qt, const int jlo, const int jhi, auto edge_tag) {
      constexpr bool EDGE = decltype(edge_tag)::value;
      f32x4 p[4], ds[4];
#pragma unroll
      for (int j = 0; j < 4; ++j) {
        p[j] = (f32x4){0.f, 0.f, 0.f, 0.f};
        ds[j] = (f32x4){0.f, 0.f, 0.f, 0.f};
        if (!EDGE || (j >= jlo && j < jhi)) {
          f32x4 s = (f32x4){0.f, 0.f, 0.f, 0.f}, dp = (f32x4){0.f, 0.f, 0.f, 0.f};
#pragma unroll
          for (int ks = 0; ks < D / 32; ++ks) {
            s = __builtin_amdgcn_mfma_f32_16x16x32_bf16(frag_row<D>(qimg, qt * 4 + j, ks, lane), kf[ks], s, 0, 0, 0);
            dp = __builtin_amdgcn_mfma_f32_16x16x32_bf16(frag_row<D>(doimg, qt * 4 + j, ks, lane), vf[ks], dp, 0, 0, 0);
          }
          const float4 L4 = *reinterpret_cast<const float4*>(L2s + qt * 64 + j * 16 + 4 * g);
          const float4 D4 = *reinterpret_cast<const float4*>(Ds + qt * 64 + j * 16 + 4 * g);
          const float Lv[4] = {L4.x, L4.y, L4.z, L4.w}, Dv[4] = {D4.x, D4.y, D4.z, D4.w};
#pragma unroll
          for (int r = 0; r < 4; ++r) {
            float x = s[r] * scale2 - Lv[r];
            if (EDGE) {
              const int q = qt * 64 + j * 16 + 4 * g + r;
              x = mykey_eff > q ? -INFINITY : x;
            }
            const float pv = __builtin_amdgcn_exp2f(x);
            p[j][r] = pv;
            ds[j][r] = pv * (dp[r] - Dv[r]) * scale;
          }
        }
      }
      if (!EDGE || jlo < 2) {
        const bf16x8 p0 = pack_acc(p[0], p[1]), d0 = pack_acc(ds[0], ds[1]);
#pragma unroll
        for (int dt = 0; dt < D / 16; ++dt) {
          dv[dt] = __builtin_amdgcn_mfma_f32_16x16x32_bf16(frag_tr<D>(doimg, dt, qt * 2, lane), p0, dv[dt], 0, 0, 0);
          dk[dt] = __builtin_amdgcn_mfma_f32_16x16x32_bf16(frag_tr<D>(qimg, dt, qt * 2, lane), d0, dk[dt], 0, 0, 0);
        }
      }
      if (!EDGE || jhi > 2) {
        const bf16x8 p1 = pack_acc(p[2], p[3]), d1 = pack_acc(ds[2], ds[3]);
#pragma unroll
        for (int dt = 0; dt < D / 16; ++dt) {
          dv[dt] = __builtin_amdgcn_mfma_f32_16x16x32_bf16(frag_tr<D>(doimg, dt, qt * 2 + 1, lane), p1, dv[dt], 0, 0, 0);
          dk[dt] = __builtin_amdgcn_mfma_f32_16x16x32_bf16(frag_tr<D>(qimg, dt, qt * 2 + 1, lane), d1, dk[dt], 0, 0, 0);
        }
      }
    };
    const int nfull = nrows / 64;
    for (int qt = qt0; qt < nqt; ++qt) {
      const int jlo = qt == qt0 ? (k0 - qt * 64) >> 4 : 0;
      const int jhi = (nrows - qt * 64) >> 4 < 4 ? (nrows - qt * 64) >> 4 : 4;
      if (qt == qt0 || text_keys || qt >= nfull) tile(qt, jlo, jhi, std::true_type{});
      else tile(qt, 0, 4, std::false_type{});
    }
    bf16_t* dkp = dqkv + ((int64_t)b * S * H + h) * 3 * D + (int64_t)mykey * rstride + D;
    store_grad_unrot<D>(dkp, dk, rot, rc, rs, mykey, lane, mykey < S);
    if (mykey < S) {
      bf16_t* dvp = dkp + D;
#pragma unroll
      for (int dt = 0; dt < D / 16; ++dt) store4(dvp + dt * 16 + 4 * g, make_float4(dv[dt][0], dv[dt][1], dv[dt][2], dv[dt][3]));
    }
    if (bsum) {
#pragma unroll
      for (int dt = 0; dt < D / 16; ++dt)
#pragma unroll
        for (int r = 0; r < 4; ++r) {
          const float vk = row16_sum(mykey < S ? dk[dt][r] : 0.f), vv = row16_sum(mykey < S ? dv[dt][r] : 0.f);
          if ((lane & 15) == 0) {
            atomicAdd(red + dt * 16 + 4 * g + r, vk);
            atomicAdd(red + D + dt * 16 + 4 * g + r, vv);
          }
        }
    }
  }
  if (bsum) {
    __syncthreads();
    if (tid < 2 * D) atomicAdd(bsum + (int64_t)h * 3 * D + D + tid, red[tid]);
  }
}

static double attn_fwd_flops(const AttnShape& sh) { return 4.0 * sh.D * ((double)sh.S * (sh.S + 1) / 2.0) * sh.H * sh.B; }

static bool attn_resident_fits(const AttnShape& sh, size_t* bytes) {
  const size_t nrows = (size_t)(sh.S + 31) / 32 * 32;
  *bytes = nrows * sh.D * 2 * 2 + nrows * 4 * 2 + (size_t)sh.D * 4 * 2;
  return sh.D <= 128 && *bytes <= 160 * 1024;
}
static int g_attn_variant = 0;

template <typename K>
static void set_lds_attr(K kfn, size_t bytes) {
  (void)hipFuncSetAttribute((const void*)kfn, hipFuncAttributeMaxDynamicSharedMemorySize, (int)bytes);
}

template <typename F>
static void dispatch_head_dim(int D, F f) {
  if (D == 64) f(std::integral_constant<int, 64>());
  else if (D == 128) f(std::integral_constant<int, 128>());
  else f(std::integral_constant<int, 256>());
}

int attn_mfma_fwd_launch(const void* qkv, const AttnShape& sh, const float* rc, const float* rs, const int64_t* am, void* out, float* lse,
                         hipStream_t st) {
  size_t bytes;
  if (g_attn_variant != 1 && attn_resident_fits(sh, &bytes)) {
    dim3 grid(sh.H, sh.B), block(attn_fwd_waves<64>() * 64);
    if (!sh.causal) {
      if (sh.D != 64) { set_error("attn_fwd (bidirectional, bf16): head_dim %d has no MFMA kernel (CLIP towers use 64)", sh.D); return MAFED_EINVAL; }
      set_lds_attr(attn_fwd_res_kernel<64, false>, bytes);
      launch(K_ATTN_FWD, 2.0 * attn_fwd_flops(sh), attn_fwd_res_kernel<64, false>, grid, block, bytes, st, (const bf16_t*)qkv, sh, rc, rs, am,
             (bf16_t*)out, lse);
      return MAFED_OK;
    }
    if (sh.D == 64) {
      set_lds_attr(attn_fwd_res_kernel<64>, bytes);
      launch(K_ATTN_FWD, attn_fwd_flops(sh), attn_fwd_res_kernel<64>, grid, block, bytes, st, (const bf16_t*)qkv, sh, rc, rs, am, (bf16_t*)out, lse);
    } else {
      set_lds_attr(attn_fwd_res_kernel<128>, bytes);
      launch(K_ATTN_FWD, attn_fwd_flops(sh), attn_fwd_res_kernel<128>, grid, dim3(attn_fwd_waves<128>() * 64), bytes, st, (const bf16_t*)qkv, sh, rc, rs, am, (bf16_t*)out, lse);
    }
    return MAFED_OK;
  }
  if (!sh.causal) { set_error("attn_fwd (bidirectional, bf16): S=%d D=%d does not fit the resident kernel", sh.S, sh.D); return MAFED_EINVAL; }
  dim3 grid((sh.S + 63) / 64, sh.H, sh.B), block(256);
  const size_t tb = (size_t)2 * 64 * sh.D * 2;
  dispatch_head_dim(sh.D, [&](auto dd) {
    constexpr int DD = decltype(dd)::value;
    set_lds_attr(attn_fwd_mfma_kernel<DD>, tb);
    launch(K_ATTN_FWD, attn_fwd_flops(sh), attn_fwd_mfma_kernel<DD>, grid, block, tb, st, (const bf16_t*)qkv, sh, rc, rs, am, (bf16_t*)out, lse);
  });
  return MAFED_OK;
}

int attn_suffix_mfma_launch(const void* qkv_img, const int64_t* image_index, const void* qkv_txt, const SuffixShape& sh, const float* rc,
                            const float* rs, const int64_t* am, void* out, hipStream_t st) {
  dim3 grid((sh.T + 63) / 64, sh.H, sh.B), block(256);
  const size_t tb = (size_t)2 * 64 * sh.D * 2;
  const double flops = 4.0 * sh.D * ((double)sh.T * sh.P + (double)sh.T * (sh.T + 1) / 2.0) * sh.H * sh.B;
  dispatch_head_dim(sh.D, [&](auto dd) {
    constexpr int DD = decltype(dd)::value;
    set_lds_attr(attn_suffix_mfma_kernel<DD>, tb);
    launch(K_ATTN_FWD, flops, attn_suffix_mfma_kernel<DD>, grid, block, tb, st, (const bf16_t*)qkv_img, image_index, (const bf16_t*)qkv_txt, sh,
           rc, rs, am, (bf16_t*)out);
  });
  return MAFED_OK;
}

int attn_cand_mfma_launch(const void* qkv_pre, const void* qkv_cand, const CandShape& sh, const float* rc, const float* rs, const int64_t* am,
                          void* out, hipStream_t st) {
  const int CA = sh.C * sh.A;
  dim3 grid((CA + 63) / 64, sh.H, sh.B), block(256);
  const size_t tb = (size_t)2 * 64 * sh.D * 2;
  const double flops = 4.0 * sh.D * ((double)CA * sh.S0 + (double)CA * (sh.A + 1) / 2.0) * sh.H * sh.B;
  dispatch_head_dim(sh.D, [&](auto dd) {
    constexpr int DD = decltype(dd)::value;
    set_lds_attr(attn_cand_mfma_kernel<DD>, tb);
    launch(K_ATTN_FWD, flops, attn_cand_mfma_kernel<DD>, grid, block, tb, st, (const bf16_t*)qkv_pre, (const bf16_t*)qkv_cand, sh, rc, rs, am,
           (bf16_t*)out);
  });
  return MAFED_OK;
}

int attn_mfma_bwd_launch(const void* qkv, const void* out, const void* dout, const float* lse, const AttnShape& sh, const float* rc,
                         const float* rs, const int64_t* am, void* dqkv, float* delta, float* colsum, bool* colsum_done, hipStream_t st) {
  size_t bytes;
  *colsum_done = false;
  if (g_attn_variant != 1 && attn_resident_fits(sh, &bytes)) {
    dim3 grid(sh.H, sh.B), block(256);
    if (sh.D == 64) {
      set_lds_attr(attn_bwd_dq_res_kernel<64>, bytes);
      set_lds_attr(attn_bwd_dkv_res_kernel<64>, bytes);
      launch(K_ATTN_BWD_DQ, attn_fwd_flops(sh), attn_bwd_dq_res_kernel<64>, grid, block, bytes, st, (const bf16_t*)qkv, (const bf16_t*)out, (const bf16_t*)dout, lse, sh, rc, rs, am,
                                                             (bf16_t*)dqkv, delta, colsum);
      launch(K_ATTN_BWD_DKV, attn_fwd_flops(sh), attn_bwd_dkv_res_kernel<64>, grid, block, bytes, st, (const bf16_t*)qkv, (const bf16_t*)dout, lse, delta, sh, rc, rs, am, (bf16_t*)dqkv, colsum);
    } else {
      set_lds_attr(attn_bwd_dq_res_kernel<128>, bytes);
      set_lds_attr(attn_bwd_dkv_res_kernel<128>, bytes);
      launch(K_ATTN_BWD_DQ, attn_fwd_flops(sh), attn_bwd_dq_res_kernel<128>, grid, block, bytes, st, (const bf16_t*)qkv, (const bf16_t*)out, (const bf16_t*)dout, lse, sh, rc, rs, am,
                                                              (bf16_t*)dqkv, delta, colsum);
      launch(K_ATTN_BWD_DKV, attn_fwd_flops(sh), attn_bwd_dkv_res_kernel<128>, grid, block, bytes, st, (const bf16_t*)qkv, (const bf16_t*)dout, lse, delta, sh, rc, rs, am, (bf16_t*)dqkv, colsum);
    }
    *colsum_done = colsum != nullptr;
    return MAFED_OK;
  }
  dim3 grid((sh.S + 63) / 64, sh.H, sh.B), block(256);
  const size_t tb = (size_t)2 * 64 * sh.D * 2, tb2 = tb + 2 * 64 * 4;
  dispatch_head_dim(sh.D, [&](auto dd) {
    constexpr int DD = decltype(dd)::value;
    set_lds_attr(attn_bwd_dq_mfma_kernel<DD>, tb);
    set_lds_attr(attn_bwd_dkv_mfma_kernel<DD>, tb2);
    launch(K_ATTN_BWD_DQ, attn_fwd_flops(sh), attn_bwd_dq_mfma_kernel<DD>, grid, block, tb, st, (const bf16_t*)qkv, (const bf16_t*)out,
           (const bf16_t*)dout, lse, sh, rc, rs, am, (bf16_t*)dqkv, delta);
    launch(K_ATTN_BWD_DKV, attn_fwd_flops(sh), attn_bwd_dkv_mfma_kernel<DD>, grid, block, tb2, st, (const bf16_t*)qkv, (const bf16_t*)dout, lse,
           delta, sh, rc, rs, am, (bf16_t*)dqkv);
  });
  return MAFED_OK;
}

void attn_mfma_set_variant(int v) { g_attn_variant = v; }


}
```

### mafed_amd/csrc/elementwise.hip

```cpp
#include "common.h"

namespace mafed {

template <typename SrcT, typename DstT>
__global__ __launch_bounds__(256) void cast_kernel(const SrcT* __restrict__ src, DstT* __restrict__ dst, int64_t n4, int64_t n) {
  const int64_t stride = (int64_t)gridDim.x * blockDim.x;
  for (int64_t i = (int64_t)blockIdx.x * blockDim.x + threadIdx.x; i < n4; i += stride) store4(dst + i * 4, load4(src + i * 4));
  if (blockIdx.x == 0 && threadIdx.x < (n - n4 * 4)) {
    const int64_t i = n4 * 4 + threadIdx.x;
    Elem<DstT>::store(dst + i, Elem<SrcT>::load(src + i));
  }
}

template <typename T>
__global__ __launch_bounds__(256) void gelu_kernel(const T* __restrict__ x, T* __restrict__ y, int64_t n) {
  const int64_t stride = (int64_t)gridDim.x * blockDim.x;
  for (int64_t i = (int64_t)blockIdx.x * blockDim.x + threadIdx.x; i < n; i += stride)
    Elem<T>::store(y + i, gelu_erf(Elem<T>::load(x + i)));
}

template <typename ImgT>
__global__ __launch_bounds__(256) void embed_concat_fwd_kernel(const ImgT* __restrict__ image, const float* __restrict__ embed_in,
                                                               const int64_t* __restrict__ input_ids, int B, int P, int T, int h,
                                                               int64_t V, float* __restrict__ h0) {
// ... 43 lines not shown
template <typename T>
__global__ __launch_bounds__(256) void colsum_kernel(const T* __restrict__ X, int64_t M, int64_t N, int64_t ldx, float* __restrict__ out) {
  __shared__ float4 sm[8][32];
  const int cq = threadIdx.x & 31, rg = threadIdx.x >> 5;
  const int64_t n = (int64_t)blockIdx.x * CS_COLS + cq * 4;
  const int64_t m0 = (int64_t)blockIdx.y * CS_ROWS;
  float4 s = make_float4(0.f, 0.f, 0.f, 0.f);
  if (n < N) {
    const int64_t m1 = m0 + CS_ROWS < M ? m0 + CS_ROWS : M;
    for (int64_t m = m0 + rg; m < m1; m += 8) {
      const float4 v = load4(X + m * ldx + n);
      s.x += v.x; s.y += v.y; s.z += v.z; s.w += v.w;
    }
  }
  sm[rg][cq] = s;
  __syncthreads();
  if (rg == 0 && n < N) {
#pragma unroll
    for (int r = 1; r < 8; ++r) {
      const float4 v = sm[r][cq];
      s.x += v.x; s.y += v.y; s.z += v.z; s.w += v.w;
    }
    atomicAdd(out + n, s.x); atomicAdd(out + n + 1, s.y); atomicAdd(out + n + 2, s.z); atomicAdd(out + n + 3, s.w);
  }
}

static int grid_for(int64_t n, int per_thread = 1) {
  int64_t g = cdiv(n, 256 * (int64_t)per_thread);
  if (g > 2048) g = 2048;
  if (g < 1) g = 1;
  return (int)g;
}

template <typename TI, typename TO>
__global__ __launch_bounds__(256) void patchify_kernel(const TI* __restrict__ pix, int B, int C, int H, int W, int ps, int gw, int np, int K,
                                                       int Kpad, int64_t rows_out, TO* __restrict__ out) {
  const int64_t idx = (int64_t)blockIdx.x * 256 + threadIdx.x;
  if (idx >= rows_out * Kpad) return;
  const int64_t row = idx / Kpad;
  const int k = (int)(idx - row * Kpad);
  float v = 0.f;
  if (k < K && row < (int64_t)B * np) {
    const int b = (int)(row / np), p = (int)(row - (int64_t)b * np);
    const int py = p / gw, px = p - py * gw;
    const int c = k / (ps * ps), r = k - c * ps * ps;
    const int i = r / ps, j = r - i * ps;
    v = Elem<TI>::load(pix + (((int64_t)b * C + c) * H + py * ps + i) * W + px * ps + j);
  }
  Elem<TO>::store(out + idx, v);
}

template <typename T>
__global__ __launch_bounds__(256) void vit_assemble_kernel(const T* __restrict__ pe, int64_t ld_pe, const float* __restrict__ cls,
                                                           const float* __restrict__ pos, int B, int np, int h, float* __restrict__ out) {
  const int64_t idx = ((int64_t)blockIdx.x * 256 + threadIdx.x) * 4;
  const int64_t total = (int64_t)B * (np + 1) * h;
  if (idx >= total) return;
  const int64_t row = idx / h;
  const int d = (int)(idx - row * h);
  const int b = (int)(row / (np + 1)), s = (int)(row - (int64_t)b * (np + 1));
  const float4 pv = load4(pos + (int64_t)s * h + d);
  float4 x = s == 0 ? load4(cls + d) : load4(pe + ((int64_t)b * np + s - 1) * ld_pe + d);
  x.x += pv.x; x.y += pv.y; x.z += pv.z; x.w += pv.w;
  store4(out + idx, x);
}

}

namespace mafed {
__global__ __launch_bounds__(256) void pad_text_rows_kernel(const float* __restrict__ src, int S, int P, int h4, int64_t n4, float* __restrict__ dst,
                                                            bf16_t* __restrict__ dst_lp) {
  const int T = S - P;
  for (int64_t i = (int64_t)blockIdx.x * 256 + threadIdx.x; i < n4; i += (int64_t)gridDim.x * 256) {
    const int64_t row = i / h4;
    const int c = (int)(i - row * h4);
    const int64_t b = row / S;
    const int s_ = (int)(row - b * S);
    float4 v = make_float4(0.f, 0.f, 0.f, 0.f);
    if (s_ >= P) v = load4(src + ((b * T + (s_ - P)) * (int64_t)h4 + c) * 4);
    store4(dst + i * 4, v);
    if (dst_lp) store4(dst_lp + i * 4, v);
  }
}
__global__ void label_rows_kernel(const int64_t* __restrict__ labels, int B, int T, int Rc, int* __restrict__ row_of_slot,
                                  int* __restrict__ slot_of_row, int64_t* __restrict__ labels_c, int* __restrict__ overflow) {
  const int b = blockIdx.x * blockDim.x + threadIdx.x;
  if (b >= B) return;
  int n = 0;
  labels_c[(int64_t)b * Rc] = -100;
  for (int t = 0; t < T; ++t) {
    const bool has = t + 1 < T && labels[(int64_t)b * T + t + 1] != -100;
    if (has && n < Rc - 1) {
      row_of_slot[b * Rc + n] = b * T + t;
      slot_of_row[b * T + t] = b * Rc + n;
      labels_c[(int64_t)b * Rc + n + 1] = labels[(int64_t)b * T + t + 1];
      ++n;
    } else {
      slot_of_row[b * T + t] = -1;
      if (has) overflow[0] = 1;
    }
  }
  for (int k = n; k < Rc; ++k) {
    row_of_slot[b * Rc + k] = -1;
    if (k + 1 < Rc) labels_c[(int64_t)b * Rc + k + 1] = -100;
  }
}

__global__ __launch_bounds__(256) void pad_text_batch_kernel(const int64_t* __restrict__ ids, const int64_t* __restrict__ mask,
                                                             const int64_t* __restrict__ labels, int T, int Tp, int64_t n,
                                                             int64_t* __restrict__ ids_out, int64_t* __restrict__ mask_out,
                                                             int64_t* __restrict__ labels_out) {
  for (int64_t i = (int64_t)blockIdx.x * 256 + threadIdx.x; i < n; i += (int64_t)gridDim.x * 256) {
    const int64_t b = i / Tp;
    const int t = (int)(i - b * Tp);
    const bool real = t < T;
    const int64_t j = b * T + t;
    ids_out[i] = real ? ids[j] : 0;
    mask_out[i] = real ? mask[j] : 0;
    if (labels_out) labels_out[i] = real ? labels[j] : -100;
  }
}

template <typename TT>
__global__ __launch_bounds__(256) void gather_rows_kernel(const TT* __restrict__ src, const int* __restrict__ idx, int64_t n_out, int hv,
                                                          TT* __restrict__ dst) {
  constexpr int EPV = 16 / sizeof(TT);
  const int64_t total = n_out * hv;
  for (int64_t i = (int64_t)blockIdx.x * 256 + threadIdx.x; i < total; i += (int64_t)gridDim.x * 256) {
    const int64_t r = i / hv;
    const int c = (int)(i - r * hv);
    const int j = idx[r];
    uint4 v = make_uint4(0u, 0u, 0u, 0u);
    if (j >= 0) v = *reinterpret_cast<const uint4*>(src + ((int64_t)j * hv + c) * EPV);
    *reinterpret_cast<uint4*>(dst + i * EPV) = v;
  }
}
}

using namespace mafed;

extern "C" int mafed_label_rows(const int64_t* labels, int B, int T, int Rc, int* row_of_slot, int* slot_of_row, int64_t* labels_c, int* overflow,
                                void* stream) {
  MAFED_CHECK_ARG(labels && row_of_slot && slot_of_row && labels_c && overflow && B > 0 && T > 1 && Rc >= 2, "label_rows: bad arguments");
  label_rows_kernel<<<dim3((B + 63) / 64), dim3(64), 0, as_stream(stream)>>>(labels, B, T, Rc, row_of_slot, slot_of_row, labels_c, overflow);
  MAFED_CHECK_LAUNCH("label_rows");
  return MAFED_OK;
}

extern "C" int mafed_gather_rows(const void* src, mafed_dtype dtype, const int* idx, int64_t n_out, int h, void* dst, void* stream) {
  MAFED_CHECK_ARG(src && idx && dst && n_out >= 0 && h > 0, "gather_rows: bad arguments");
  MAFED_CHECK_ARG(h % (dtype == MAFED_F32 ? 4 : 8) == 0, "gather_rows: h=%d must fill 16-byte pieces", h);
  if (n_out == 0) return MAFED_OK;
  const int hv = h / (dtype == MAFED_F32 ? 4 : 8);
  const dim3 grid(grid_for(n_out * hv)), block(256);
  if (dtype == MAFED_F32) gather_rows_kernel<float><<<grid, block, 0, as_stream(stream)>>>((const float*)src, idx, n_out, hv, (float*)dst);
  else gather_rows_kernel<bf16_t><<<grid, block, 0, as_stream(stream)>>>((const bf16_t*)src, idx, n_out, hv, (bf16_t*)dst);
  MAFED_CHECK_LAUNCH("gather_rows");
  return MAFED_OK;
}

extern "C" int mafed_pad_text_rows(const float* src, int B, int S, int P, int h, float* dst, void* dst_lp, void* stream) {
  MAFED_CHECK_ARG(src && dst && B > 0 && S > 0 && P >= 0 && P < S && h > 0 && h % 4 == 0, "pad_text_rows: bad arguments");
  const int64_t n4 = (int64_t)B * S * (h / 4);
  launch(K_CAST, (double)B * h * ((S - P) * 4.0 + S * (4.0 + (dst_lp ? 2.0 : 0.0))), pad_text_rows_kernel, dim3(grid_for(n4)), dim3(256), 0, as_stream(stream), src, S, P,
         h / 4, n4, dst, (bf16_t*)dst_lp);
  MAFED_CHECK_LAUNCH("pad_text_rows");
  return MAFED_OK;
}

extern "C" int mafed_pad_text_batch(const int64_t* ids, const int64_t* mask, const int64_t* labels, int B, int T, int Tp, int64_t* ids_out,
                                    int64_t* mask_out, int64_t* labels_out, void* stream) {
  MAFED_CHECK_ARG(ids && mask && ids_out && mask_out && B > 0 && T > 0 && Tp >= T, "pad_text_batch: bad arguments");
  MAFED_CHECK_ARG((labels != nullptr) == (labels_out != nullptr), "pad_text_batch: labels and labels_out go together");
  const int64_t n = (int64_t)B * Tp;
  pad_text_batch_kernel<<<dim3(grid_for(n)), dim3(256), 0, as_stream(stream)>>>(ids, mask, labels, T, Tp, n, ids_out, mask_out, labels_out);
  MAFED_CHECK_LAUNCH("pad_text_batch");
  return MAFED_OK;
}

extern "C" int mafed_cast(const void* src, mafed_dtype sd, void* dst, mafed_dtype dd, int64_t n, void* stream) {
  MAFED_CHECK_ARG(src && dst && n >= 0, "cast: bad arguments");
  if (n == 0) return MAFED_OK;
  hipStream_t st = as_stream(stream);
  const int64_t n4 = n / 4;
  dim3 grid(grid_for(n4)), block(256);
  const double cbytes = (double)n * ((sd == MAFED_F32 ? 4.0 : 2.0) + (dd == MAFED_F32 ? 4.0 : 2.0));
  if (sd == MAFED_F32 && dd == MAFED_BF16) launch(K_CAST, cbytes, cast_kernel<float, bf16_t>, grid, block, 0, st, (const float*)src, (bf16_t*)dst, n4, n);
  else if (sd == MAFED_BF16 && dd == MAFED_F32) launch(K_CAST, cbytes, cast_kernel<bf16_t, float>, grid, block, 0, st, (const bf16_t*)src, (float*)dst, n4, n);
  else if (sd == MAFED_F32 && dd == MAFED_F32) launch(K_CAST, cbytes, cast_kernel<float, float>, grid, block, 0, st, (const float*)src, (float*)dst, n4, n);
  else launch(K_CAST, cbytes, cast_kernel<bf16_t, bf16_t>, grid, block, 0, st, (const bf16_t*)src, (bf16_t*)dst, n4, n);
  MAFED_CHECK_LAUNCH("cast");
  return MAFED_OK;
}

extern "C" int mafed_gelu(const void* x, void* y, mafed_dtype dtype, int64_t n, void* stream) {
  MAFED_CHECK_ARG(x && y && n >= 0, "gelu: bad arguments");
  if (n == 0) return MAFED_OK;
  hipStream_t st = as_stream(stream);
  dim3 grid(grid_for(n)), block(256);
  if (dtype == MAFED_F32) gelu_kernel<float><<<grid, block, 0, st>>>((const float*)x, (float*)y, n);
  else gelu_kernel<bf16_t><<<grid, block, 0, st>>>((const bf16_t*)x, (bf16_t*)y, n);
  MAFED_CHECK_LAUNCH("gelu");
  return MAFED_OK;
}

extern "C" int mafed_embed_concat_fwd(const void* image, mafed_dtype img_dtype, const float* embed_in, const int64_t* input_ids,
                                      int B, int P, int T, int h, int64_t V, float* h0, void* stream) {
  MAFED_CHECK_ARG(image && embed_in && input_ids && h0, "embed_concat_fwd: null pointer");
  MAFED_CHECK_ARG(B >= 0 && P >= 0 && T >= 0 && h > 0 && h % 4 == 0 && V > 0, "embed_concat_fwd: bad shape (h must be a multiple of 4)");
  const int64_t rows = (int64_t)B * (P + T);
  if (rows == 0) return MAFED_OK;
  hipStream_t st = as_stream(stream);
  dim3 grid((unsigned)cdiv(rows, 4)), block(256);
  const double ebytes = (double)B * h * (P * (img_dtype == MAFED_F32 ? 4.0 : 2.0) + T * 4.0 + (P + T) * 4.0);
  if (img_dtype == MAFED_F32) launch(K_EMBED_FWD, ebytes, embed_concat_fwd_kernel<float>, grid, block, 0, st, (const float*)image, embed_in, input_ids, B, P, T, h, V, h0);
  else launch(K_EMBED_FWD, ebytes, embed_concat_fwd_kernel<bf16_t>, grid, block, 0, st, (const bf16_t*)image, embed_in, input_ids, B, P, T, h, V, h0);
  MAFED_CHECK_LAUNCH("embed_concat_fwd");
  return MAFED_OK;
}

extern "C" int mafed_embed_concat_bwd(const float* dh0, const int64_t* input_ids, int B, int P, int T, int h, int64_t V,
                                      void* d_image, mafed_dtype img_dtype, float* d_embed_in, void* stream) {
  MAFED_CHECK_ARG(dh0 && input_ids, "embed_concat_bwd: null pointer");
  MAFED_CHECK_ARG(B >= 0 && P >= 0 && T >= 0 && h > 0 && h % 4 == 0 && V > 0, "embed_concat_bwd: bad shape (h must be a multiple of 4)");
  const int64_t rows = (int64_t)B * (P + T);
  if (rows == 0) return MAFED_OK;
  hipStream_t st = as_stream(stream);
  dim3 grid((unsigned)cdiv(rows, 4)), block(256);
  const double ebytes = (double)B * h * ((P + T) * 4.0 + P * (img_dtype == MAFED_F32 ? 4.0 : 2.0) + T * 4.0);
  if (img_dtype == MAFED_F32) launch(K_EMBED_BWD, ebytes, embed_concat_bwd_kernel<float>, grid, block, 0, st, dh0, input_ids, B, P, T, h, V, (float*)d_image, d_embed_in);
  else launch(K_EMBED_BWD, ebytes, embed_concat_bwd_kernel<bf16_t>, grid, block, 0, st, dh0, input_ids, B, P, T, h, V, (bf16_t*)d_image, d_embed_in);
  MAFED_CHECK_LAUNCH("embed_concat_bwd");
  return MAFED_OK;
}

extern "C" size_t mafed_colsum_workspace_bytes(int64_t M, int64_t N) { (void)M; (void)N; return 0; }

extern "C" int mafed_colsum(const void* X, mafed_dtype dtype, int64_t M, int64_t N, int64_t ldx, float* out, void* workspace,
                            size_t workspace_bytes, void* stream) {
  (void)workspace; (void)workspace_bytes;
  MAFED_CHECK_ARG(X && out && M >= 0 && N > 0 && ldx >= N, "colsum: bad arguments");
  MAFED_CHECK_ARG(N % 4 == 0 && ldx % 4 == 0 && ((uintptr_t)X & 7) == 0, "colsum: N and ldx must be multiples of 4, X 8-byte aligned");
  if (M == 0) return MAFED_OK;
  hipStream_t st = as_stream(stream);
  dim3 grid((unsigned)cdiv(N, CS_COLS), (unsigned)cdiv(M, CS_ROWS)), block(256);
  const double sbytes = (double)M * N * (dtype == MAFED_F32 ? 4.0 : 2.0);
  if (dtype == MAFED_F32) launch(K_COLSUM, sbytes, colsum_kernel<float>, grid, block, 0, st, (const float*)X, M, N, ldx, out);
  else launch(K_COLSUM, sbytes, colsum_kernel<bf16_t>, grid, block, 0, st, (const bf16_t*)X, M, N, ldx, out);
  MAFED_CHECK_LAUNCH("colsum");
  return MAFED_OK;
}

// ... 38 lines not shown
```

### mafed_amd/engine.py

```python
from __future__ import annotations

from dataclasses import dataclass
from typing import Any, Dict, List, Optional, Sequence

import torch

from mafed_amd import ops
from mafed_amd._lib import EPI_GELU, EPI_GELU_BWD


def _trim(x: torch.Tensor, n: int) -> torch.Tensor:
    return x if x.shape[1] == n else x[:, :n].contiguous()


@dataclass
class SweepRecord:
    serial: int = 0
    filled_squares: bool = False
    dx_chain_event: Optional[torch.cuda.Event] = None


class SideWork:

    def __init__(self, main, sides, enter=torch.cuda.stream):
        self.main, self.sides, self.enter = main, sides, enter
        self.keep: List[Any] = []
        self._next = 0
        self._mark = None

    def main_moved(self) -> None:
        self._mark = None

    def on_side(self, fn, *tensors, k: Optional[int] = None) -> None:
        sides = self.sides
        if sides is None:
            fn()
            return
        if k is None:
            k = self._next % len(sides)
            self._next += 1
        if self._mark is None:
            self._mark = self.main.record_event()
        with self.enter(sides[k]):
            sides[k].wait_event(self._mark)
            fn()
        self.keep.extend(tensors)

    def after_all(self, fn) -> None:
        sides = self.sides or ()
        evs = [st.record_event() for st in sides[1:]]
        def run():
            for e in evs:
                sides[0].wait_event(e)
            fn()
        self.on_side(run, k=0)

    def join(self) -> None:
        if self.sides is not None:
            for st in self.sides:
                self.main.wait_stream(st)
        self.keep.clear()


class BackwardSweep:

    def __init__(self, model, sv, dhidden: Sequence[Optional[torch.Tensor]], taps=None):
        self.model, self.sv, self.dhidden, self.taps = model, sv, dhidden, taps
        self.record = model.last_sweep = SweepRecord(model.last_sweep.serial + 1)
        model.final_grad_sumsq = None
        cfg = self.cfg = model.config
        self.cd = model.compute_dtype
        self.B, self.T, self.P, self.S = sv["B"], sv["T"], sv["P"], sv["S"]
        self.h, self.L, self.rows = cfg.hidden_size, cfg.num_hidden_layers, self.B * self.S
        self.cos, self.sin = model.rotary_tables(self.S)
        self.wts, self.pars, self.grads = model._tensors(0), model._tensors(1), model._tensors(2)
        if len(dhidden) > self.L and dhidden[self.L] is not None:
            raise NotImplementedError("gradient w.r.t. the post-final-LayerNorm hidden state is not on the MAFED path")
        self.inject = sv.get("inject")
        self.inj_cos = bool(sv.get("inject_cosine", False))
        self.sched = SideWork(torch.cuda.current_stream(), model.side_streams() if model.overlap_param_grads else None)
        self._decide_policy()
        self.dx = self.dy = None
        self.dy_bias_done = False

    def _decide_policy(self) -> None:
        m, taps = self.model, self.taps
        self.group_dw = (self.cd == torch.bfloat16 and int(m.dw_group_layers) > 0
                         and m.contended_backward in (False, None, "ticketed"))
        self.overwrite = self.group_dw and bool(m.grad_overwrite) and taps is None
        if m._dw_stale and not self.overwrite:
            m._zero_layer_matrices(range(self.L))
        m._dw_stale = False
        self.dw_beta = 0.0 if self.overwrite else 1.0
        self.dw_sq = m.dw_sumsq if (self.group_dw and taps is None) else None
        if self.dw_sq is not None and not m._dw_group_fuses_squares(self.rows):
            self.dw_sq = None
        self.record.filled_squares = self.dw_sq is not None
        self.pending_dw, self.pending_layers = [], []
        self.defer_ln = (self.sched.sides is not None and m.defer_ln_param_reduce and taps is None
                         and not any(d is not None for d in self.dhidden))

    def wgrad(self, dY, X, gw, gb=None) -> None:
        def run():
            ops.gemm(dY, X, True, False, out=gw, beta=1.0)
            if gb is not None:
                ops.colsum_(dY, gb)
        self.sched.on_side(run, dY, X)

    def wgrad_layer(self, dY, X, i: int, slot: int, with_bias: bool = False) -> None:
        g = self.grads.layers[i]
        gw, gb = g.matrix(slot), g.bias(slot) if with_bias else None
        if not self.group_dw:
            self.wgrad(dY, X, gw, gb)
            return
        q = dict(A=dY, B=X, out=gw, beta=self.dw_beta)
        if self.dw_sq is not None:
            q["sumsq"] = self.dw_sq[i, slot]
        self.pending_dw.append(q)
        if gb is not None:
            self.sched.on_side(lambda: ops.colsum_(dY, gb), dY)

    def flush_dw(self) -> None:
        pending = self.pending_dw
        for c0 in range(0, len(pending), 16):
            ops.gemm_grouped(pending[c0:c0 + 16], True, False)
        if pending:
            pending.clear()
            self.sched.main_moved()
        for li in self.pending_layers:
            self.ready(li)
        self.pending_layers.clear()

    def ready(self, i: int) -> None:
        hook = self.model.grad_ready_hook
        if hook is not None:
            self.sched.after_all(lambda: hook(i))

    def run(self, dloss: Optional[torch.Tensor]) -> None:
        self.head(dloss)
        for i in range(self.L - 1, -1, -1):
            self.layer(i)
        self.flush_dw()
        self.record.dx_chain_event = self.sched.main.record_event()
        self.projector()
        self.finish()

    def head(self, dloss: Optional[torch.Tensor]) -> None:
        sv, cd, sched = self.sv, self.cd, self.sched
        if dloss is None or sv["loss"] is None:
            return
        B, T, h, V = self.B, self.T, self.h, self.cfg.vocab_size
        Wo, Po, Go = self.wts.outer, self.pars.outer, self.grads.outer
        xt, lnf, fmean, frstd = sv["final"]
        logits = sv["logits"]
        gl = dloss.reshape(1).to(torch.float32).contiguous()
        sp = sv.get("sparse_head")
        n_head = logits.shape[0] * logits.shape[1]
        head_labels = sp[1] if sp is not None else sv["labels"]
        kd = sv.pop("kd", None)
        if kd is not None:
            dlog = ops.ce_kd_bwd(logits, kd[0], head_labels, kd[1], kd[2], kd[3], gl).view(n_head, V)
        else:
            dlog = ops.ce_bwd(logits, head_labels, sv["ce_lse"], gl).view(n_head, V)
        self.wgrad(dlog, lnf, Go.embed_out)
        if cd == torch.bfloat16:
            dlnf = torch.zeros((n_head, h), dtype=torch.float32, device=self.model.flat_params.device)
            ops.gemm(dlog, Wo.embed_out, False, False, out=dlnf, beta=1.0)
        else:
            dlnf = ops.gemm(dlog, Wo.embed_out, False, False)
        if sp is not None:
            dlnf = ops.gather_rows(dlnf if dlnf.dtype == torch.float32 else dlnf.float(), sp[0])
        if self.defer_ln:
            dxt, _, fws = ops.layernorm_bwd_rows(dlnf, None, xt, fmean, frstd, Po.final_ln_w, None, None)
            sched.main_moved()
            sched.on_side(lambda ws=fws: ops.layernorm_bwd_params(ws, B * T, h, Go.final_ln_w, Go.final_ln_b), fws)
        else:
            dxt, _ = ops.layernorm_bwd(dlnf, None, xt, fmean, frstd, Po.final_ln_w, None, None,
                                       Go.final_ln_w, Go.final_ln_b)
        self.dx, self.dy = ops.pad_text_rows(dxt, B, self.S, self.P, cd if cd != torch.float32 else None)
        sched.main_moved()
        self.ready(self.L)

    def layer(self, i: int) -> None:
        inj = self.inject.get(i) if self.inject else None
        if self._gradient_into(i, inj):
            self._layer_backward(i, inj)

    def _gradient_into(self, i: int, inj) -> bool:
        sched, dhidden, rows, h, dx = self.sched, self.dhidden, self.rows, self.h, self.dx
        ext = dhidden[i + 1] if (i + 1) < min(len(dhidden), self.L) else None
        if ext is not None:
            ext = ext.reshape(rows, h)
            if dx is not None and self.dy_bias_done:
                ops.colsum_(ext.to(torch.float32).contiguous(), self.grads.layers[i].fc2_b)
                ops.colsum_(ext.to(torch.float32).contiguous(), self.grads.layers[i].dense_b)
            dx = self.dx = ext.to(torch.float32) if dx is None else dx.add_(ext)
            self.dy = None
            sched.main_moved()
        if dx is None:
            if inj is not None:
                x = self.sv["layers"][i]["x"].view(self.B, self.S, h)
                self.dx = ops.distill_bwd(x, inj[0], self.sv["attention_mask"], self.P, inj[1], cosine=self.inj_cos).view(rows, h)
                sched.main_moved()
            if self.overwrite:
                self.model._zero_layer_matrices([i])
                sched.main_moved()
            return False
        if self.dy is None:
            self.dy = dx if self.cd == torch.float32 else ops.cast(dx, self.cd)
            sched.main_moved()
        return True

    def _layer_backward(self, i: int, inj) -> None:
        sv, cd, sched, cfg, wgrad_layer = self.sv, self.cd, self.sched, self.cfg, self.wgrad_layer
        B, S, P, h, rows, am = self.B, self.S, self.P, self.h, self.rows, sv["attention_mask"]
        dx, dy, dy_bias_done, g = self.dx, self.dy, self.dy_bias_done, self.grads.layers[i]
        H, D, rot = cfg.num_attention_heads, cfg.head_dim, cfg.rotary_ndims
        w, p = self.wts.layers[i], self.pars.layers[i]
        s = sv["layers"][i]
        wgrad_layer(dy, s["a"], i, 3, with_bias=not dy_bias_done)
        wgrad_layer(dy, s["ao"], i, 1, with_bias=not dy_bias_done)
        du = ops.gemm(dy, w.fc2_w, False, False, epilogue=EPI_GELU_BWD, aux=s["u"], colsum=g.fc1_b)
        sched.main_moved()
        wgrad_layer(du, s["ln2"], i, 2)
        dln2 = ops.gemm(du, w.fc1_w, False, False)
        dao = ops.gemm(dy, w.dense_w, False, False)
        dqkv = ops.attn_bwd(s["qkv"], s["ao"], dao, s["lse"], B, S, H, D, rot, self.cos, self.sin, am, colsum=g.qkv_b)
        sched.main_moved()
        wgrad_layer(dqkv, s["ln1"], i, 0)
        dln1 = ops.gemm(dqkv, w.qkv_w, False, False)
        ln_kw = dict(want_lp=(cd != torch.float32), teacher=(inj[0].view(rows, h) if torch.is_tensor(inj[0]) else inj[0]) if inj is not None else None,
                     attention_mask=am if inj is not None else None, S=S, P=P, inj_scale=inj[1] if inj is not None else None,
                     inj_mul=-1.0 if self.inj_cos else 2.0 / h)
        below = self.grads.layers[i - 1] if i > 0 else None
        dxa, dxb = (below.fc2_b, below.dense_b) if i > 0 else (None, None)
        if self.defer_ln:
            dx, dy, ln_ws = ops.layernorm_bwd_rows(dln1, dln2, s["x"], s["mean"], s["rstd"], p.ln1_w, p.ln2_w, dx, want_dxsum=i > 0, **ln_kw)
            sched.main_moved()
            sched.on_side(lambda ws=ln_ws: ops.layernorm_bwd_params(
                ws, rows, h, g.ln1_w, g.ln1_b, g.ln2_w, g.ln2_b, dxa, dxb), ln_ws)
        else:
            dx, dy = ops.layernorm_bwd(dln1, dln2, s["x"], s["mean"], s["rstd"], p.ln1_w, p.ln2_w, dx, g.ln1_w, g.ln1_b, g.ln2_w, g.ln2_b,
                                       dxsum_a=dxa, dxsum_b=dxb, **ln_kw)
            sched.main_moved()
        self.dx, self.dy, self.dy_bias_done = dx, (dx if cd == torch.float32 else dy), i > 0
        if self.taps is not None and i in self.taps:
            self.taps[i] = dx
        if self.group_dw:
            self.pending_layers.append(i)
            if len(self.pending_layers) >= int(self.model.dw_group_layers):
                self.flush_dw()
        else:
            self.ready(i)

    def projector(self) -> None:
        sv, sched, dx = self.sv, self.sched, self.dx
        Wo, Go = self.wts.outer, self.grads.outer
        ext0 = self.dhidden[0] if len(self.dhidden) > 0 else None
        if ext0 is not None:
            ext0 = ext0.reshape(self.rows, self.h)
            dx = ext0.to(torch.float32).contiguous() if dx is None else dx.add_(ext0)
            sched.main_moved()
        if dx is not None:
            fc, u0, a0 = sv["proj"]
            dimg = ops.embed_concat_bwd(dx, sv["input_ids"], self.B, self.P, self.T, self.h, self.cfg.vocab_size, Go.embed_in, self.cd)
            sched.main_moved()
            self.wgrad(dimg, a0, Go.proj2_w, Go.proj2_b)
            du0 = ops.gemm(dimg, Wo.proj2_w, False, False, epilogue=EPI_GELU_BWD, aux=u0, colsum=Go.proj0_b)
            sched.main_moved()
            self.wgrad(du0, fc, Go.proj0_w)

    def finish(self) -> None:
        self.ready(-1)
        self.sched.join()


class EngineMixin:

    def _params_ready(self, st, lo: int, hi: int) -> None:
        pe, L = self._param_events, self.config.num_hidden_layers
        if pe is not None:
            for c in range(lo, hi):
                st.wait_event(pe["pre" if c < 0 else "head" if c == L else ("layer", c)])
            if hi > L:
                self._param_events = None
        if lo < 0 and self._shadow_dirty:
            self.sync_shadow()

    def _projector_forward(self, feats, n: int, train: bool):
        cfg, cd = self.config, self.compute_dtype
        Wo, Po = self._tensors(0).outer, self._tensors(1).outer
        f2 = feats.reshape(n * cfg.num_vision_tokens, cfg.vision_hidden_size)
        if f2.dtype not in (torch.float32, torch.bfloat16):
            f2 = f2.float()
        fc = f2.contiguous() if f2.dtype == cd else ops.cast(f2.contiguous(), cd)
        u0 = torch.empty((f2.shape[0], cfg.hidden_size), dtype=cd, device=fc.device) if train else None
        a0 = ops.gemm(fc, Wo.proj0_w, False, True, bias=Po.proj0_b, epilogue=EPI_GELU, aux=u0)
        return fc, u0, a0, ops.gemm(a0, Wo.proj2_w, False, True, bias=Po.proj2_b)

    def _layer_forward(self, wts, pars, i: int, x: torch.Tensor, attend, qkv_out: Optional[torch.Tensor] = None,
                       rec: Optional[dict] = None, train: bool = False) -> torch.Tensor:
        cfg, cd = self.config, self.compute_dtype
        w, p = wts.layers[i], pars.layers[i]
        ln1, ln2, mean, rstd = ops.layernorm_fwd(x, p.ln1_w, p.ln1_b, p.ln2_w, p.ln2_b, cfg.layer_norm_eps, cd, save_stats=train)
        qkv = ops.gemm(ln1, w.qkv_w, False, True, bias=p.qkv_b, out=qkv_out)
        ao, lse = attend(qkv)
        attn = ops.gemm(ao, w.dense_w, False, True, bias=p.dense_b, out_dtype=cd)
        u = torch.empty((x.shape[0], cfg.intermediate_size), dtype=cd, device=x.device) if train else None
        a = ops.gemm(ln2, w.fc1_w, False, True, bias=p.fc1_b, epilogue=EPI_GELU, aux=u)
        if rec is not None:
            rec["qkv"] = qkv
            if train:
                rec.update(x=x, mean=mean, rstd=rstd, ln1=ln1, ln2=ln2, ao=ao, lse=lse, u=u, a=a)
        return ops.gemm(a, w.fc2_w, False, True, bias=p.fc2_b, out_dtype=torch.float32, res1=attn, res2=x)

    def _final_ln(self, x: torch.Tensor, out_dtype, save_stats: bool = False):
        Po = self._tensors(1).outer
        return ops.layernorm_fwd(x, Po.final_ln_w, Po.final_ln_b, None, None, self.config.layer_norm_eps, out_dtype, save_stats=save_stats)

    def _lm_head(self, x: torch.Tensor) -> torch.Tensor:
        return ops.gemm(self._final_ln(x, self.compute_dtype)[0], self._tensors(0).outer.embed_out, False, True)

    def _engine_forward(self, feats, input_ids, attention_mask, labels, want_hidden, train, n_hidden: Optional[int] = None,
                        keep_qkv: bool = False, qkv_out: Optional[Sequence[torch.Tensor]] = None, label_rows_hint: Optional[int] = None,
                        last_only: bool = False, skip_head: bool = False, pad_text: bool = False, head_rows: Optional[torch.Tensor] = None):
        if not self.flat_params.is_cuda:
            raise RuntimeError("mafed_amd runs on the GPU only (no CPU fallback); move the model with .cuda()")
        pe, main_st = self._param_events, torch.cuda.current_stream()
        self._params_ready(main_st, -1, 0)
        cfg = self.config
        B, T_in = input_ids.shape
        P, h, H, D, L = cfg.num_vision_tokens, cfg.hidden_size, cfg.num_attention_heads, cfg.head_dim, cfg.num_hidden_layers
        T = self.padded_text_len(B, T_in) if pad_text else T_in
        if T != T_in:
            input_ids, attention_mask, labels = ops.pad_text_batch(input_ids, attention_mask, labels, T)
        S = P + T
# ... 3 lines not shown
        sv: Dict[str, Any] = {"B": B, "T": T, "T_in": T_in, "P": P, "S": S, "input_ids": input_ids, "attention_mask": attention_mask, "labels": labels,
                              "layers": [], "loss": None, "logits": None}
        fc, u0, a0, img = self._projector_forward(feats, B, train)
        x = ops.embed_concat_fwd(img, pars.outer.embed_in, input_ids, B, P, T)
        if train:
            sv["proj"] = (fc, u0, a0)
        hidden = [x.view(B, S, h)]
        hook = self.hidden_ready_hook if train else None
        if hook is not None:
            hook(0, x)
        attend = lambda qkv: ops.attn_fwd(qkv, B, S, H, D, rot, cos, sin, attention_mask)
        n_layers = L if n_hidden is None else max(0, min(L, n_hidden - 1))
        for i in range(n_layers):
            if pe is not None:
                self._params_ready(main_st, i, i + 1)
            rec = {} if (train or keep_qkv) else None
            if rec is not None:
                sv["layers"].append(rec)
            x = self._layer_forward(wts, pars, i, x, attend, qkv_out[i] if qkv_out is not None else None, rec, train)
            if i < L - 1:
                hidden.append(x.view(B, S, h))
                if hook is not None:
                    hook(i + 1, x)
        sv["hidden"] = hidden
        self._params_ready(main_st, n_layers, L + 1)
        if n_hidden is not None:
            return sv
        if last_only:
            sv["logits"] = self._lm_head(x.view(B, S, h)[:, -1, :].contiguous()).view(B, 1, cfg.vocab_size)
        elif skip_head:
            hidden.append(self._final_ln(x, torch.float32)[0].view(B, S, h))
        elif head_rows is not None:
            assert not train and labels is None
            sv["logits"] = self._lm_head(ops.gather_rows(x.view(B, S, h)[:, P:, :].reshape(B * T, h), head_rows))
        else:
            self._head_text(sv, x, feats, want_hidden, train, label_rows_hint)
        return sv

    def _head_text(self, sv, x, feats, want_hidden: bool, train: bool, label_rows_hint: Optional[int]) -> None:
        cd, labels = self.compute_dtype, sv["labels"]
        B, T, P, S, h = sv["B"], sv["T"], sv["P"], sv["S"], self.config.hidden_size
        xt = x.view(B, S, h)[:, P:, :].reshape(B * T, h)
        lnf, _, fmean, frstd = self._final_ln(xt, cd, save_stats=train)
        if want_hidden:
            sv["hidden"].append(self._final_ln(x, torch.float32)[0].view(B, S, h))
        Rc = None
        if train and labels is not None and label_rows_hint is not None:
            need = max(2, int(label_rows_hint) + 1)
            Rc = need if cd == torch.float32 else next((r for r in range(need, T + 1) if (B * r) % 128 == 0), None)
            if Rc is not None and Rc * 2 > T:
                Rc = None
        ros = ov = None
        if Rc is not None:
            ros, sor, labels, ov = ops.label_rows(labels, Rc)
            self.last_label_overflow = ov
            sv["sparse_head"] = (sor, labels)
        teacher = None
        if train and sv["labels"] is not None and self.logit_teacher is not None:
            t_logits, tau, lam = self.logit_teacher(feats, sv["input_ids"], sv["attention_mask"], ros)
            teacher = (t_logits.detach(), float(tau), float(lam))
        if ros is not None:
            lnf = ops.gather_rows(lnf, ros)
        logits = sv["logits"] = ops.gemm(lnf, self._tensors(0).outer.embed_out, False, True).view(B, Rc or T, self.config.vocab_size)
        if teacher is not None:
            self._head_kd_loss(sv, logits, labels, teacher, ov)
        elif labels is not None:
            sv["loss"], lse_ce = ops.ce_fwd(logits, labels, poison=ov)
            if train:
                sv["ce_lse"] = lse_ce
        if train:
            sv["final"] = (xt, lnf, fmean, frstd)
            sv["x_last"] = x

    def _head_kd_loss(self, sv, logits, labels, teacher, poison) -> None:
        t_logits, tau, lam = teacher
        if t_logits.dtype != logits.dtype or t_logits.numel() != logits.numel():
            raise ValueError(f"logit_teacher returned {tuple(t_logits.shape)} {t_logits.dtype} for head rows {tuple(logits.shape)} {logits.dtype}")
        t_logits = t_logits.contiguous().view(logits.shape)
        out3, lse3 = ops.ce_kd_fwd(logits, t_logits, labels, tau, lam, poison=poison)
        sv["loss"] = out3[0:1]
        sv["kd"] = (t_logits, lse3, tau, lam)
        self.last_head_losses = out3

    def _dw_group_fuses_squares(self, rows: int) -> bool:
        cache = self._dw_fuse_cache
        key = (int(rows), int(self.dw_group_layers or 0))
        if key not in cache:
            cfg = self.config
            h, f = cfg.hidden_size, cfg.intermediate_size
            per_layer = [(3 * h, h, rows), (h, h, rows), (f, h, rows), (h, f, rows)]
            n_layers = max(1, min(4, key[1]))
            cache[key] = bool(key[1]) and ops.gemm_grouped_fuses_sumsq(per_layer * n_layers, True, False)
        return cache[key]

    def _engine_backward(self, sv, dloss: Optional[torch.Tensor], dhidden: Sequence[Optional[torch.Tensor]], taps=None):
        cb = self.contended_backward
        if cb and self.flat_params.is_cuda:
            ctx = ops.ticketed_gemm() if cb == "ticketed" else ops.no_persistent_gemm()
            with ctx:
                return BackwardSweep(self, sv, dhidden, taps).run(dloss)
        return BackwardSweep(self, sv, dhidden, taps).run(dloss)


class _ModelFn(torch.autograd.Function):

    @staticmethod
    def forward(ctx, anchor, model, feats, input_ids, attention_mask, labels, want_hidden, ctx_box, label_rows_hint=None):
        sv = model._engine_forward(feats, input_ids, attention_mask, labels, want_hidden, train=True, label_rows_hint=label_rows_hint, pad_text=True)
        ctx.model, ctx.sv = model, sv
        ctx_box.append(sv)
        ctx.set_materialize_grads(False)
        loss = sv["loss"].reshape(()) if sv["loss"] is not None else torch.zeros((), device=anchor.device)
        pub = _trim(sv["logits"], sv["T_in"]) if sv.get("sparse_head") is None else torch.empty(0, device=anchor.device)
        outs = [loss, pub.detach(), model._hook_zero().view(())]
        ctx.mark_non_differentiable(outs[1])
        if want_hidden:
            outs += [x.detach() for x in sv["hidden"]]
        return tuple(outs)

    @staticmethod
    def backward(ctx, dloss, dlogits, dhook, *dhidden):
        sv = ctx.sv
        ctx.sv = None
        if sv is None:
            raise RuntimeError("mafed_amd: backward through the model twice (activations already released)")
        if sv["loss"] is None:
            dloss = None
        ctx.model._engine_backward(sv, dloss, list(dhidden))
        sv.pop("inject", None)
        return (None,) * 9
```

### mafed_amd/model.py

```python
from __future__ import annotations

import copy
import math
from dataclasses import dataclass, field
from collections import namedtuple
from typing import Any, Dict, List, Optional, Sequence, Tuple

import os as _os

import torch
from torch import nn

from mafed_amd import ops
from mafed_amd.engine import EngineMixin, SweepRecord, _ModelFn, _trim
from mafed_amd.generation import BeamSearchOutput, GenerationMixin, _DecodeCache, _GraphedDecode


@dataclass
class VLPythiaConfig:

    vocab_size: int = 50304
    hidden_size: int = 1024
    num_hidden_layers: int = 24
    num_attention_heads: int = 16
# ... 110 lines not shown
            ("vision_embed_tokens.2.weight", (h, h)), ("vision_embed_tokens.2.bias", (h,))]
    return out


class BufferViews:
    __slots__ = ("src", "layers", "outer", "by_name")

    def __init__(self, src: torch.Tensor, offsets: Dict[str, Tuple[int, int, Tuple[int, ...]]], n_layers: int):
        self.src = src
        self.by_name = {name: src[o:o + n].view(shape) for name, (o, n, shape) in offsets.items()}
        self.layers = [LayerTensors(*(self.by_name[layer_tensor_name(i, f)] for f in LayerTensors._fields)) for i in range(n_layers)]
        self.outer = OuterTensors(*(self.by_name[name] for name in OUTER_FIELD_NAMES.values()))
        if len(LayerTensors._fields) * n_layers + len(OuterTensors._fields) != len(offsets):
            raise KeyError("the parameter records do not cover every tensor of the flat layout")


TEXT_BUCKET_ROWS = 128
TEXT_BUCKET_MAX_PAD = 16


def bucket_text_len(text_bucket, B: int, P: int, T: int) -> int:
    if isinstance(text_bucket, str):
        if text_bucket != "auto":
            raise ValueError(f"text_bucket must be 'auto', 0 or a positive int, not {text_bucket!r}")
        for Tp in range(T, T + TEXT_BUCKET_MAX_PAD + 1):
            if (B * (P + Tp)) % TEXT_BUCKET_ROWS == 0:
                return Tp
        return T
    m = int(text_bucket or 0)
    if m < 0:
        raise ValueError(f"text_bucket must be 'auto', 0 or a positive int, not {text_bucket!r}")
    return T if m == 0 else T + (-(P + T)) % m


class VLPythiaForCausalLM(EngineMixin, GenerationMixin, nn.Module):

    def __init__(self, config: VLPythiaConfig, compute_dtype: torch.dtype = torch.bfloat16, device: Any = None,
                 vision_encoder: Optional[nn.Module] = None, seed: Optional[int] = None, text_bucket: Any = None):
        super().__init__()
        assert compute_dtype in (torch.bfloat16, torch.float32)
        self.text_bucket = text_bucket if text_bucket is not None else ("auto" if compute_dtype == torch.bfloat16 else 0)
        bucket_text_len(self.text_bucket, 1, 0, 1)
        assert config.use_parallel_residual, "GPT-NeoX sequential residual is not on the MAFED path (config/vlpythia-base.json:30)"
        self.config = config
        self.compute_dtype = compute_dtype
        dev = torch.device(device) if device is not None else torch.device("cuda" if torch.cuda.is_available() else "cpu")
        specs = _param_specs(config)
        order = [s for s in specs if not is_no_decay(s[0])] + [s for s in specs if is_no_decay(s[0])]
        offs, off = {}, 0
        n_decay_end = 0
        for name, shape in order:
            n = int(math.prod(shape))
            offs[name] = (off, n, shape)
            off += (n + 63) // 64 * 64
            if not is_no_decay(name):
                n_decay_end = off
        self._offsets = offs
        self._n_flat = off
        self._n_decay = n_decay_end
        self.flat_params = torch.zeros(off, dtype=torch.float32, device=dev)
        self.flat_grads = torch.zeros(off, dtype=torch.float32, device=dev)
        self.flat_shadow = torch.zeros(off, dtype=torch.bfloat16, device=dev) if compute_dtype == torch.bfloat16 else None
        self._shadow_dirty = True
        self._build_tree(specs)
        from mafed_amd.vision import ClipVisionTower
        if isinstance(vision_encoder, ClipVisionTower):
            if vision_encoder.config.hidden_size != config.vision_hidden_size or vision_encoder.config.num_patches != config.num_vision_tokens:
                raise ValueError("vision tower (hidden %d, %d patches) does not match the config (vision_hidden_size %d, num_vision_tokens %d)" % (
                    vision_encoder.config.hidden_size, vision_encoder.config.num_patches, config.vision_hidden_size, config.num_vision_tokens))
            self.vision_encoder = vision_encoder
        else:
            self.vision_encoder = _FrozenVision(vision_encoder)
        self._anchor = torch.zeros(1, device=dev, requires_grad=True)
        self._rot_cache: Dict[Tuple[int, str], Tuple[torch.Tensor, torch.Tensor]] = {}
        self.grad_ready_hook = None
        self.hidden_ready_hook = None
        self._param_events = None
        self._side = None
        self._hook_zero_t: Optional[torch.Tensor] = None
        self._views: List[Optional[BufferViews]] = [None, None, None]
        self._tensors(1)
        self.overlap_param_grads = True
        self.dw_group_layers = 2
        self._dw_fuse_cache: Dict[Tuple[int, int], bool] = {}
        self.sparse_lm_head = True
        self.last_label_overflow: Optional[torch.Tensor] = None
        self.logit_teacher = None
        self.last_head_losses: Optional[torch.Tensor] = None
        self.defer_ln_param_reduce = True
        self.beam_trace: Optional[List[Any]] = None
        self.prefill_trace: Optional[List[Any]] = None
        self.fused_decode = True
        self._decode_graphs: Dict[Tuple, Any] = {}
        self.contended_backward: Any = False
        self.grad_overwrite = False
        self._dw_stale = False
        self.dw_sumsq: Optional[torch.Tensor] = None
        self.final_grad_sumsq: Optional[torch.Tensor] = None
        self.last_sweep = SweepRecord()
        self.reset_parameters(seed)
        self.register_load_state_dict_post_hook(lambda m, ik: setattr(m, "_shadow_dirty", True))

    def _build_tree(self, specs):
        params: Dict[str, nn.Parameter] = {}
        for name, shape in specs:
            o, n, _ = self._offsets[name]
            p = nn.Parameter(self.flat_params[o:o + n].view(shape))
            p.grad = self.flat_grads[o:o + n].view(shape)
            params[name] = p
        self._params_by_name = params
        cfg = self.config
        neox = nn.Module()
        neox.embed_in = _Affine(params["gpt_neox.embed_in.weight"], None)
        layers = nn.ModuleList()
        for i in range(cfg.num_hidden_layers):
            t = LayerTensors(*(params[layer_tensor_name(i, f)] for f in LayerTensors._fields))
            lyr = nn.Module()
            lyr.input_layernorm = _Affine(t.ln1_w, t.ln1_b)
            lyr.post_attention_layernorm = _Affine(t.ln2_w, t.ln2_b)
            att = nn.Module()
            att.query_key_value = _Affine(t.qkv_w, t.qkv_b)
            att.dense = _Affine(t.dense_w, t.dense_b)
            lyr.attention = att
            mlp = nn.Module()
            mlp.dense_h_to_4h = _Affine(t.fc1_w, t.fc1_b)
            mlp.dense_4h_to_h = _Affine(t.fc2_w, t.fc2_b)
            lyr.mlp = mlp
            layers.append(lyr)
        neox.layers = layers
        neox.final_layer_norm = _Affine(params["gpt_neox.final_layer_norm.weight"], params["gpt_neox.final_layer_norm.bias"])
        self.gpt_neox = neox
        self.embed_out = _Affine(params["embed_out.weight"], None)
        vt = nn.Module()
        setattr(vt, "0", _Affine(params["vision_embed_tokens.0.weight"], params["vision_embed_tokens.0.bias"]))
        setattr(vt, "2", _Affine(params["vision_embed_tokens.2.weight"], params["vision_embed_tokens.2.bias"]))
        self.vision_embed_tokens = vt

    def reset_parameters(self, seed: Optional[int] = None):
        g = torch.Generator(device="cpu")
        g.manual_seed(0 if seed is None else int(seed))
        with torch.no_grad():
            for name, p in self._params_by_name.items():
                if "layernorm" in name or "layer_norm" in name:
                    p.fill_(1.0 if name.endswith("weight") else 0.0)
                elif name.endswith("bias"):
                    p.zero_()
                else:
                    p.copy_(torch.randn(p.shape, generator=g) * self.config.initializer_range)
        self._shadow_dirty = True

    @classmethod
    def from_pretrained(cls, pretrained_model_name: str, vision_encoder_name: str = "", select_layer: int = -2,
                        select_feature: str = "patch", use_flash_attention_2: bool = False, state_dict=None, **kw):
        import json
        import os
        if not os.path.isdir(pretrained_model_name):
            raise ValueError(f"{pretrained_model_name!r} is not a local directory (no network access on this path)")
        with open(os.path.join(pretrained_model_name, "config.json")) as fp:
            cfg = VLPythiaConfig.from_dict(json.load(fp))
        model = cls(cfg, **kw)
        st = os.path.join(pretrained_model_name, "model.safetensors")
        if os.path.exists(st):
            from safetensors.torch import load_file
            sd = load_file(st)
        else:
            sd = torch.load(os.path.join(pretrained_model_name, "pytorch_model.bin"), map_location="cpu")
        model.load_state_dict({k: v for k, v in sd.items() if not k.startswith("vision_encoder.")}, strict=False)
        if state_dict is not None:
            model.load_state_dict(state_dict, strict=False)
        return model

    def __deepcopy__(self, memo):
# ... 211 lines not shown
```

### mafed_amd/ops.py

```python
from __future__ import annotations

from typing import Optional, Sequence, Tuple

import torch

from mafed_amd import _lib
import contextlib
import ctypes as C
import threading

from mafed_amd._lib import BF16, EPI_GELU, EPI_GELU_BWD, EPI_NO_PERSISTENT, EPI_NONE, EPI_QUICK_GELU, EPI_RES1_BF16, EPI_TICKETED, F32, check


def _dt(t: torch.Tensor) -> int:
    if t.dtype == torch.float32:
        return F32
    if t.dtype == torch.bfloat16:
        return BF16
    raise TypeError(f"unsupported dtype {t.dtype}")


def _ptr(t: Optional[torch.Tensor]) -> int:
    if t is None:
        return 0
# ... 171 lines not shown
    def record_stream(self, stream) -> None:
        self.states.record_stream(stream)
        if self.index is not None:
            self.index.record_stream(stream)

    def materialize(self) -> torch.Tensor:
        n, S, h = self.states.shape
        if self.index is None:
            return self.states if self.states.dtype == torch.float32 else cast(self.states, torch.float32)
        if n * S >= 2 ** 31:
            raise RuntimeError(f"TeacherRows.materialize: {n} samples x {S} tokens exceed the 32-bit row ids of the gather kernel")
        B = self.index.numel()
        rows = (self.index.view(B, 1) * S + torch.arange(S, device=self.index.device, dtype=torch.int32).view(1, S)).view(-1)
        out = gather_rows(self.states.view(n * S, h), rows)
        return (out if out.dtype == torch.float32 else cast(out, torch.float32)).view(B, S, h)


def _teacher(t, B: Optional[int] = None, S: Optional[int] = None, h: Optional[int] = None):
    if t is None:
        return 0, F32, 0
    if isinstance(t, TeacherRows):
        if (B is not None and t.shape[0] != B) or (S is not None and t.shape[1] != S) or (h is not None and t.shape[2] != h):
            raise ValueError(f"TeacherRows of shape {t.shape} for a batch of [{B}, {S}, {h}]")
        return _ptr(t.states), _dt(t.states), _ptr(t.index)
    assert t.dtype == torch.float32 and t.is_contiguous()
    return _ptr(t), F32, 0


def layernorm_bwd(dy1, dy2, x, mean, rstd, w1, w2, dres, dw1, db1, dw2=None, db2=None, want_lp: bool = False,
                  teacher=None, attention_mask=None, S: int = 0, P: int = 0, inj_scale=None, inj_mul: float = 1.0,
                  dxsum_a=None, dxsum_b=None):
    rows, h = x.shape
    dx = torch.empty((rows, h), dtype=torch.float32, device=x.device)
    dx_lp = torch.empty((rows, h), dtype=dy1.dtype, device=x.device) if want_lp else None
    lib = _lib.load()
    nb = lib.mafed_layernorm_bwd_workspace_bytes(rows, h)
    ws = workspace(x.device).get(nb)
    tp, tdt, tix = _teacher(teacher, rows // S if S else None, S or None, h)
    check(lib.mafed_layernorm_bwd_indexed(_ptr(dy1), _ptr(dy2), _dt(dy1), _ptr(x), _ptr(mean), _ptr(rstd), _ptr(w1), _ptr(w2), rows, h,
                                          _ptr(dres), _ptr(dx), _ptr(dx_lp), _ptr(dw1), _ptr(db1), _ptr(dw2), _ptr(db2), tp, tdt, tix,
                                          _ptr(attention_mask), S, P, S - P, _ptr(inj_scale), float(inj_mul), _ptr(dxsum_a), _ptr(dxsum_b), _ptr(ws),
                                          ws.numel(), _stream()),
          "mafed_layernorm_bwd")
    return dx, dx_lp


def layernorm_bwd_rows(dy1, dy2, x, mean, rstd, w1, w2, dres, want_lp: bool = False, teacher=None, attention_mask=None, S: int = 0, P: int = 0,
                       inj_scale=None, inj_mul: float = 1.0, want_dxsum: bool = False):
    rows, h = x.shape
    dx = torch.empty((rows, h), dtype=torch.float32, device=x.device)
    dx_lp = torch.empty((rows, h), dtype=dy1.dtype, device=x.device) if want_lp else None
    lib = _lib.load()
    ws = torch.empty(lib.mafed_layernorm_bwd_workspace_bytes(rows, h), dtype=torch.uint8, device=x.device)
    tp, tdt, tix = _teacher(teacher, rows // S if S else None, S or None, h)
    check(lib.mafed_layernorm_bwd_rows_indexed(_ptr(dy1), _ptr(dy2), _dt(dy1), _ptr(x), _ptr(mean), _ptr(rstd), _ptr(w1), _ptr(w2), rows, h,
                                               _ptr(dres), _ptr(dx), _ptr(dx_lp), tp, tdt, tix, _ptr(attention_mask), S, P, S - P, _ptr(inj_scale),
                                               float(inj_mul), 1 if want_dxsum else 0, _ptr(ws), ws.numel(), _stream()), "mafed_layernorm_bwd_rows")
    return dx, dx_lp, ws


def layernorm_bwd_params(ws: torch.Tensor, rows: int, h: int, dw1, db1, dw2=None, db2=None, dxsum_a=None, dxsum_b=None) -> None:
    check(_lib.load().mafed_layernorm_bwd_params(rows, h, _ptr(dw1), _ptr(db1), _ptr(dw2), _ptr(db2), _ptr(dxsum_a), _ptr(dxsum_b), _ptr(ws),
                                                 ws.numel(), _stream()), "mafed_layernorm_bwd_params")


def attn_fwd(qkv: torch.Tensor, B: int, S: int, H: int, D: int, rot: int, cos, sin, attention_mask: torch.Tensor):
    T = attention_mask.shape[1]
    out = torch.empty((B * S, H * D), dtype=qkv.dtype, device=qkv.device)
    lse = torch.empty((B, H, S), dtype=torch.float32, device=qkv.device)
    check(_lib.load().mafed_attn_fwd(_ptr(qkv), _dt(qkv), B, S, H, D, rot, _ptr(cos), _ptr(sin), _ptr(attention_mask), T, _ptr(out),
                                     _ptr(lse), _stream()), "mafed_attn_fwd")
    return out, lse


def attn_fwd_exact_bf16(qkv, B, S, H, D, rot, cos, sin, attention_mask):
    T = attention_mask.shape[1]
    out = torch.empty((B * S, H * D), dtype=qkv.dtype, device=qkv.device)
    lse = torch.empty((B, H, S), dtype=torch.float32, device=qkv.device)
    check(_lib.load().mafed_attn_fwd_exact_bf16(_ptr(qkv), B, S, H, D, rot, _ptr(cos), _ptr(sin), _ptr(attention_mask), T, _ptr(out),
                                                _ptr(lse), _stream()), "mafed_attn_fwd_exact_bf16")
    return out, lse


def attn_bwd(qkv, out, dout, lse, B, S, H, D, rot, cos, sin, attention_mask, colsum: Optional[torch.Tensor] = None):
    T = attention_mask.shape[1]
    dqkv = torch.empty_like(qkv)
    delta = torch.empty((B, H, S), dtype=torch.float32, device=qkv.device)
    if colsum is None:
        check(_lib.load().mafed_attn_bwd(_ptr(qkv), _ptr(out), _ptr(dout), _ptr(lse), _dt(qkv), B, S, H, D, rot, _ptr(cos), _ptr(sin),
                                         _ptr(attention_mask), T, _ptr(dqkv), _ptr(delta), _stream()), "mafed_attn_bwd")
    else:
        assert colsum.dtype == torch.float32 and colsum.numel() == 3 * H * D and colsum.is_contiguous()
        check(_lib.load().mafed_attn_bwd_colsum(_ptr(qkv), _ptr(out), _ptr(dout), _ptr(lse), _dt(qkv), B, S, H, D, rot, _ptr(cos),
                                                _ptr(sin), _ptr(attention_mask), T, _ptr(dqkv), _ptr(delta), _ptr(colsum), _stream()),
              "mafed_attn_bwd_colsum")
    return dqkv


def attn_fwd_bidir(qkv: torch.Tensor, B: int, S: int, H: int, D: int, out: Optional[torch.Tensor] = None):
    assert qkv.dim() == 2 and qkv.shape[1] == 3 * H * D and qkv.shape[0] >= B * S and qkv.is_contiguous()
    if out is None:
        out = torch.empty((B * S, H * D), dtype=qkv.dtype, device=qkv.device)
    assert out.dtype == qkv.dtype and out.shape[0] >= B * S and out.shape[1] == H * D and out.is_contiguous()
    lse = torch.empty((B, H, S), dtype=torch.float32, device=qkv.device)
    check(_lib.load().mafed_attn_fwd_bidir(_ptr(qkv), _dt(qkv), B, S, H, D, _ptr(out), _ptr(lse), _stream()), "mafed_attn_fwd_bidir")
    return out


def patchify(pixels: torch.Tensor, patch: int, rows_out: int, k_pad: int, out_dtype: torch.dtype) -> torch.Tensor:
    B, C, H, W = pixels.shape
    assert pixels.is_contiguous()
    out = torch.empty((rows_out, k_pad), dtype=out_dtype, device=pixels.device)
    check(_lib.load().mafed_patchify(_ptr(pixels), _dt(pixels), B, C, H, W, int(patch), int(rows_out), int(k_pad), _ptr(out), _dt(out), _stream()),
          "mafed_patchify")
    return out


def vit_assemble(patch_emb: torch.Tensor, class_embedding: torch.Tensor, position_embedding: torch.Tensor, B: int, num_patches: int, h: int,
                 out: torch.Tensor) -> torch.Tensor:
    assert out.dtype == torch.float32 and out.is_contiguous() and out.shape[0] >= B * (num_patches + 1) and out.shape[1] == h
    assert class_embedding.dtype == torch.float32 and position_embedding.dtype == torch.float32 and position_embedding.is_contiguous()
    check(_lib.load().mafed_vit_assemble(_ptr(patch_emb), _dt(patch_emb), patch_emb.stride(0), _ptr(class_embedding), _ptr(position_embedding), B,
                                         num_patches, h, _ptr(out), _stream()), "mafed_vit_assemble")
    return out


def rotate_k_rows_(qkv: torch.Tensor, B: int, S: int, H: int, D: int, rot: int, cos, sin) -> None:
    assert qkv.is_contiguous() and qkv.numel() == B * S * H * 3 * D and cos.shape[0] >= S
    check(_lib.load().mafed_rotate_k_rows(_ptr(qkv), _dt(qkv), B, S, H, D, rot, _ptr(cos), _ptr(sin), _stream()), "mafed_rotate_k_rows")


def attn_decode(qkv_prefix: torch.Tensor, S0: int, qkv_new: torch.Tensor, t: int, B: int, H: int, D: int, rot: int, cos, sin,
                attention_mask: torch.Tensor, prerot: bool = False) -> torch.Tensor:
    cap = qkv_new.shape[1]
    assert qkv_new.dim() == 3 and qkv_new.is_contiguous() and qkv_prefix.is_contiguous() and qkv_new.dtype == qkv_prefix.dtype
    assert cos.shape[0] >= S0 + t + 1
    out = torch.empty((B, H * D), dtype=qkv_new.dtype, device=qkv_new.device)
    fn = _lib.load().mafed_attn_decode_prerot if prerot else _lib.load().mafed_attn_decode
    check(fn(_ptr(qkv_prefix), S0, _ptr(qkv_new), cap, t, _dt(qkv_new), B, H, D, rot, _ptr(cos), _ptr(sin),
             _ptr(attention_mask), attention_mask.shape[1], _ptr(out), _stream()), "mafed_attn_decode")
    return out


def attn_decode_beam(qkv_prefix: torch.Tensor, S0: int, qkv_new: torch.Tensor, t: int, B: int, k: int, anc: torch.Tensor, H: int, D: int,
                     rot: int, cos, sin, attention_mask: torch.Tensor) -> torch.Tensor:
    cap = qkv_new.shape[1]
    assert qkv_new.dim() == 3 and qkv_new.shape[0] == B * k and qkv_new.is_contiguous() and qkv_prefix.is_contiguous()
    assert qkv_new.dtype == qkv_prefix.dtype and anc.dtype == torch.int32 and anc.shape == (B * k, cap) and anc.is_contiguous()
    assert cos.shape[0] >= S0 + t + 1
    out = torch.empty((B * k, H * D), dtype=qkv_new.dtype, device=qkv_new.device)
    check(_lib.load().mafed_attn_decode_beam(_ptr(qkv_prefix), S0, _ptr(qkv_new), cap, t, _dt(qkv_new), B, k, _ptr(anc), H, D, rot, _ptr(cos),
                                             _ptr(sin), _ptr(attention_mask), attention_mask.shape[1], _ptr(out), _stream()), "mafed_attn_decode_beam")
    return out


def _image_index(image_index: Optional[torch.Tensor], N: int, B: int, device) -> Optional[torch.Tensor]:
    if image_index is None:
        assert N == B, f"no image_index: N ({N}) must equal B ({B})"
        return None
    assert image_index.dtype == torch.int64 and image_index.shape == (B,) and image_index.is_contiguous() and image_index.device == device
    return image_index


def attn_suffix_fwd(qkv_img: torch.Tensor, image_index: Optional[torch.Tensor], N: int, P: int, qkv_txt: torch.Tensor, T: int, B: int, H: int,
                    D: int, rot: int, cos, sin, attention_mask: torch.Tensor) -> torch.Tensor:
    assert qkv_img.is_contiguous() and qkv_txt.is_contiguous() and qkv_img.dtype == qkv_txt.dtype
    assert qkv_img.numel() == N * P * 3 * H * D and qkv_txt.numel() == B * T * 3 * H * D
    assert attention_mask.shape == (B, T) and attention_mask.dtype == torch.int64 and attention_mask.is_contiguous()
    assert cos.shape[0] >= P + T
    image_index = _image_index(image_index, N, B, qkv_txt.device)
    out = torch.empty((B * T, H * D), dtype=qkv_txt.dtype, device=qkv_txt.device)
# ... 327 lines not shown
    return stats4


def agem_project(g: torch.Tensor, r: torch.Tensor, stats4: torch.Tensor, out: Optional[torch.Tensor] = None,
                 sumsq_partials: Optional[torch.Tensor] = None) -> torch.Tensor:
    _agem_flat(g, r)
    if out is None:
        out = torch.empty_like(g)
    _agem_flat(g, out)
    assert stats4.dtype == torch.float32 and stats4.numel() == 4 and stats4.is_contiguous()
    if sumsq_partials is not None:
        assert sumsq_partials.dtype == torch.float32 and sumsq_partials.is_contiguous() and sumsq_partials.numel() >= agem_blocks(g.numel())
    check(_lib.load().mafed_agem_project(_ptr(g), _ptr(r), _ptr(out), g.numel(), _ptr(stats4), _ptr(sumsq_partials), _stream()),
          "mafed_agem_project")
    return out


def cka_pool(hidden: Sequence[torch.Tensor], attention_mask: torch.Tensor, P: int, out: torch.Tensor, rows: Optional[torch.Tensor] = None) -> None:
    L = len(hidden)
    B, S, h = hidden[0].shape
    T = attention_mask.shape[1]
    assert all(x.shape == (B, S, h) and x.dtype == torch.float32 and x.is_contiguous() for x in hidden)
    assert attention_mask.dtype == torch.int64 and attention_mask.shape == (B, T) and attention_mask.is_contiguous()
    assert out.dtype == torch.float32 and out.is_contiguous() and out.dim() == 4 and out.shape[0] == 2 and out.shape[1] == L and out.shape[3] == h
    if rows is not None:
        assert rows.dtype == torch.int64 and rows.shape == (B,) and rows.is_contiguous()
    ptrs = (C.c_void_p * L)(*[_ptr(x) for x in hidden])
    check(_lib.load().mafed_cka_pool(ptrs, L, B, S, int(P), h, _ptr(attention_mask), T, _ptr(rows), out.shape[2], _ptr(out), _stream()),
          "mafed_cka_pool")


def cka_stats(X: torch.Tensor, row_norms: bool = True) -> Tuple[torch.Tensor, Optional[torch.Tensor]]:
    assert X.dtype == torch.float32 and X.dim() in (2, 3) and X.stride(-1) == 1
    X3 = X if X.dim() == 3 else X.unsqueeze(0)
    G, n, h = X3.shape
    lib = _lib.load()
    mean = torch.empty((G, h), dtype=torch.float64, device=X.device)
    rsq = torch.empty((G, n), dtype=torch.float64, device=X.device) if row_norms else None
    ws = workspace(X.device).get(lib.mafed_cka_stats_workspace_bytes(G, n, h))
    check(lib.mafed_cka_stats(_ptr(X3), G, n, h, X3.stride(1), X3.stride(0), _ptr(mean), _ptr(rsq), _ptr(ws), ws.numel(), _stream()),
          "mafed_cka_stats")
    return mean, rsq


def cka_hsic(products: Sequence[Tuple[torch.Tensor, torch.Tensor, torch.Tensor, torch.Tensor]], out: Optional[torch.Tensor] = None) -> torch.Tensor:
    descs = (_lib.CkaProduct * max(1, len(products)))()
    dev = None
    for i, (X, mx, Y, my) in enumerate(products):
        assert X.dtype == torch.float32 and Y.dtype == torch.float32 and X.dim() == 2 and Y.dim() == 2 and X.shape[0] == Y.shape[0]
        assert X.stride(1) == 1 and Y.stride(1) == 1
        assert mx.dtype == torch.float64 and my.dtype == torch.float64 and mx.shape == (X.shape[1],) and my.shape == (Y.shape[1],)
        assert mx.is_contiguous() and my.is_contiguous()
        descs[i] = _lib.CkaProduct(_ptr(X), _ptr(mx), X.stride(0), X.shape[1], _ptr(Y), _ptr(my), Y.stride(0), Y.shape[1], X.shape[0])
        dev = X.device
    if out is None:
        out = torch.empty(len(products), dtype=torch.float64, device=dev)
    assert out.dtype == torch.float64 and out.is_contiguous() and out.numel() == len(products)
    if not products:
        return out
    lib = _lib.load()
    ws = workspace(dev).get(lib.mafed_cka_hsic_workspace_bytes(descs, len(products)))
    check(lib.mafed_cka_hsic(descs, len(products), _ptr(out), _ptr(ws), ws.numel(), _stream()), "mafed_cka_hsic")
    return out


def gradnorm_clip(g: torch.Tensor, max_norm: float, out2: Optional[torch.Tensor] = None) -> torch.Tensor:
    lib = _lib.load()
    if out2 is None:
        out2 = torch.empty(2, dtype=torch.float32, device=g.device)
    nb = lib.mafed_gradnorm_workspace_bytes(g.numel())
    ws = workspace(g.device).get(nb)
    check(lib.mafed_gradnorm_clip(_ptr(g), g.numel(), float(max_norm), _ptr(out2), _ptr(ws), ws.numel(), _stream()), "mafed_gradnorm_clip")
    return out2


def pad_text_rows(src: torch.Tensor, B: int, S: int, P: int, lp_dtype=None):
    h = src.shape[-1]
    dst = torch.empty((B * S, h), dtype=torch.float32, device=src.device)
    lp = torch.empty((B * S, h), dtype=lp_dtype, device=src.device) if lp_dtype == torch.bfloat16 else None
    check(_lib.load().mafed_pad_text_rows(_ptr(src), B, S, P, h, _ptr(dst), _ptr(lp), _stream()), "mafed_pad_text_rows")
    return dst, lp


def label_rows(labels: torch.Tensor, Rc: int):
    B, T = labels.shape
    dev = labels.device
    ros = torch.empty(B * Rc, dtype=torch.int32, device=dev)
    sor = torch.empty(B * T, dtype=torch.int32, device=dev)
    lc = torch.empty((B, Rc), dtype=torch.int64, device=dev)
    ov = torch.zeros(1, dtype=torch.int32, device=dev)
    check(_lib.load().mafed_label_rows(_ptr(labels), B, T, Rc, _ptr(ros), _ptr(sor), _ptr(lc), _ptr(ov), _stream()), "mafed_label_rows")
    return ros, sor, lc, ov


def pad_text_batch(input_ids: torch.Tensor, attention_mask: torch.Tensor, labels: Optional[torch.Tensor], Tp: int):
    B, T = input_ids.shape
    dev = input_ids.device
    out = torch.empty((3 if labels is not None else 2, B, Tp), dtype=torch.int64, device=dev)
    check(_lib.load().mafed_pad_text_batch(_ptr(input_ids), _ptr(attention_mask), _ptr(labels), B, T, int(Tp), _ptr(out[0]), _ptr(out[1]),
                                           _ptr(out[2]) if labels is not None else 0, _stream()), "mafed_pad_text_batch")
    return out[0], out[1], (out[2] if labels is not None else None)


def gemm_fallback_launches() -> int:
    return int(_lib.load().mafed_gemm_fallback_launches())


def gather_rows(src: torch.Tensor, idx: torch.Tensor) -> torch.Tensor:
    h = src.shape[-1]
    dst = torch.empty((idx.numel(), h), dtype=src.dtype, device=src.device)
    check(_lib.load().mafed_gather_rows(_ptr(src), _dt(src), _ptr(idx), idx.numel(), h, _ptr(dst), _stream()), "mafed_gather_rows")
    return dst


def gradnorm_blocks(n: int) -> int:
    return int(_lib.load().mafed_gradnorm_blocks(int(n)))


def gradnorm_partial(g: torch.Tensor, partial_out: torch.Tensor) -> None:
    check(_lib.load().mafed_gradnorm_partial(_ptr(g), g.numel(), _ptr(partial_out), _stream()), "mafed_gradnorm_partial")


def gradnorm_finish(partials: torch.Tensor, max_norm: float, out2: torch.Tensor, advance=None, norm_log: Optional[torch.Tensor] = None) -> torch.Tensor:
    if advance is None:
        check(_lib.load().mafed_gradnorm_finish(_ptr(partials), partials.numel(), float(max_norm), _ptr(out2), _stream()), "mafed_gradnorm_finish")
        if norm_log is not None:
            norm_log.copy_(out2[0:1])
    else:
        state, base_lr, warmup, total, b1, b2, hyper = advance
        check(_lib.load().mafed_gradnorm_finish_advance(_ptr(partials), partials.numel(), float(max_norm), _ptr(out2), _ptr(norm_log), _ptr(state),
                                                        float(base_lr), int(warmup), int(total), float(b1), float(b2), _ptr(hyper), _stream()),
              "mafed_gradnorm_finish_advance")
    return out2


def adamw_step_(p, g, m, v, lr_dev, beta1, beta2, eps, weight_decay, step, clip=None, grad_mul=1.0, p_bf16=None, zero_grad: bool = False,
                zero_n: Optional[int] = None) -> None:
    if zero_grad and zero_n is not None and zero_n < p.numel():
        check(_lib.load().mafed_adamw_step_partial_zero(_ptr(p), _ptr(g), _ptr(m), _ptr(v), p.numel(), _ptr(lr_dev), beta1, beta2, eps, weight_decay,
                                                        int(step), _ptr(clip), float(grad_mul), _ptr(p_bf16), int(zero_n), _stream()), "mafed_adamw_step")
        return
    fn = _lib.load().mafed_adamw_step_zero_grad if zero_grad else _lib.load().mafed_adamw_step
    check(fn(_ptr(p), _ptr(g), _ptr(m), _ptr(v), p.numel(), _ptr(lr_dev), beta1, beta2, eps, weight_decay,
             int(step), _ptr(clip), float(grad_mul), _ptr(p_bf16), _stream()), "mafed_adamw_step")


def adam_family_step_(rule: str, p, g, m, s, lr_dev, beta1, beta2, eps, weight_decay, step, clip=None, grad_mul=1.0, p_bf16=None,
                      zero_n: int = 0) -> None:
    fn = {"adam": "mafed_adam_step", "adamax": "mafed_adamax_step"}[rule]
    check(getattr(_lib.load(), fn)(_ptr(p), _ptr(g), _ptr(m), _ptr(s), p.numel(), _ptr(lr_dev), float(beta1), float(beta2), eps, weight_decay, int(step),
                                   _ptr(clip), float(grad_mul), _ptr(p_bf16), int(zero_n), _stream()), fn)


def optim_advance_(state: torch.Tensor, base_lr: float, warmup: int, total: int, beta1: float, beta2: float, hyper: torch.Tensor,
                   clip: Optional[torch.Tensor] = None) -> None:
    check(_lib.load().mafed_optim_advance_guarded(_ptr(state), float(base_lr), int(warmup), int(total), float(beta1), float(beta2),
                                                  _ptr(hyper), _ptr(clip), _stream()), "mafed_optim_advance")


def cast(src: torch.Tensor, dtype: torch.dtype, out: Optional[torch.Tensor] = None) -> torch.Tensor:
    assert src.is_contiguous()
    if out is None:
        out = torch.empty(src.shape, dtype=dtype, device=src.device)
    check(_lib.load().mafed_cast(_ptr(src), _dt(src), _ptr(out), _dt(out), src.numel(), _stream()), "mafed_cast")
    return out

# ... 6 lines not shown
```

Baseline: 1007 samples/s.

## Restrict top decoder layer backward to text rows and skip image-query attention

In the top transformer layer only the text positions carry loss gradient, so the backward for that layer now gathers the text rows and runs the MLP/dense gradient GEMMs on B*T rows instead of B*S. It then scatters the results back with zeros. The attention backward gains a first-query bound so the dQ and dK/dV kernels skip query slices below the text start and write zeros there. This cuts GEMM and attention work in the last layer, at the cost of extra gather/scatter kernels and more code paths with alignment constraints.

```diff
diff --git a/include/mafed_hip.h b/include/mafed_hip.h
--- a/include/mafed_hip.h
+++ b/include/mafed_hip.h
@@ -103,6 +103,11 @@
                           int B, int S, int H, int D, int rot, const float* rot_cos, const float* rot_sin,
                           const int64_t* attention_mask, int T, void* dqkv, float* delta, float* dqkv_colsum, void* stream);
 
+int mafed_attn_bwd_first_query(mafed_dtype dtype, int B, int S, int H, int D, int rot, int T, int q_lo_want);
+int mafed_attn_bwd_from(const void* qkv, const void* out, const void* dout, const float* lse, mafed_dtype dtype,
+                        int B, int S, int H, int D, int rot, const float* rot_cos, const float* rot_sin,
+                        const int64_t* attention_mask, int T, void* dqkv, float* delta, float* dqkv_colsum, int q_lo, void* stream);
+
 int mafed_attn_decode(const void* qkv_prefix, int S0, const void* qkv_new, int cap, int t, mafed_dtype dtype,
                       int B, int H, int D, int rot, const float* rot_cos, const float* rot_sin,
                       const int64_t* attention_mask, int T, void* out, void* stream);
@@ -259,6 +264,8 @@
 
 int mafed_cast(const void* src, mafed_dtype src_dtype, void* dst, mafed_dtype dst_dtype, int64_t n, void* stream);
 int mafed_pad_text_rows(const float* src, int B, int S, int P, int h, float* dst, void* dst_lp, void* stream);
+int mafed_gather_text_rows(const void* const* src, void* const* dst, const int64_t* row_bytes, int n, int B, int S, int P, void* stream);
+int mafed_scatter_text_rows(const void* src, int64_t row_bytes, int B, int S, int P, int lo, void* dst, void* stream);
 int mafed_label_rows(const int64_t* labels, int B, int T, int Rc, int* row_of_slot, int* slot_of_row, int64_t* labels_c, int* overflow,
                      void* stream);
 int mafed_gather_rows(const void* src, mafed_dtype dtype, const int* idx, int64_t n_out, int h, void* dst, void* stream);
diff --git a/mafed_amd/_lib.py b/mafed_amd/_lib.py
--- a/mafed_amd/_lib.py
+++ b/mafed_amd/_lib.py
@@ -71,6 +71,8 @@
     "mafed_attn_bwd": (_i, [_p, _p, _p, _p, _i, _i, _i, _i, _i, _i, _p, _p, _p, _i, _p, _p, _p]),
     "mafed_attn_bwd_colsum": (_i, [_p, _p, _p, _p, _i, _i, _i, _i, _i, _i, _p, _p, _p, _i, _p, _p, _p, _p]),
     "mafed_attn_set_variant": (_i, [_i]),
+    "mafed_attn_bwd_first_query": (_i, [_i, _i, _i, _i, _i, _i, _i, _i]),
+    "mafed_attn_bwd_from": (_i, [_p, _p, _p, _p, _i, _i, _i, _i, _i, _i, _p, _p, _p, _i, _p, _p, _p, _i, _p]),
     "mafed_attn_fwd_exact_bf16": (_i, [_p, _i, _i, _i, _i, _i, _p, _p, _p, _i, _p, _p, _p]),
     "mafed_embed_concat_fwd": (_i, [_p, _i, _p, _p, _i, _i, _i, _i, _l, _p, _p]),
     "mafed_embed_concat_bwd": (_i, [_p, _p, _i, _i, _i, _i, _l, _p, _i, _p, _p]),
@@ -108,6 +110,8 @@
     "mafed_gradnorm_finish_advance": (_i, [_p, _i, _f, _p, _p, _p, _d, _l, _l, _d, _d, _p, _p]),
     "mafed_cast": (_i, [_p, _i, _p, _i, _l, _p]),
     "mafed_pad_text_rows": (_i, [_p, _i, _i, _i, _i, _p, _p, _p]),
+    "mafed_gather_text_rows": (_i, [_p, _p, _p, _i, _i, _i, _i, _p]),
+    "mafed_scatter_text_rows": (_i, [_p, _l, _i, _i, _i, _i, _p, _p]),
     "mafed_label_rows": (_i, [_p, _i, _i, _i, _p, _p, _p, _p, _p]),
     "mafed_gather_rows": (_i, [_p, _i, _p, _l, _i, _p, _p]),
     "mafed_pad_text_batch": (_i, [_p, _p, _p, _i, _i, _i, _p, _p, _p, _p]),
diff --git a/mafed_amd/csrc/attn.h b/mafed_amd/csrc/attn.h
--- a/mafed_amd/csrc/attn.h
+++ b/mafed_amd/csrc/attn.h
@@ -78,7 +78,8 @@
 int attn_mfma_fwd_launch(const void* qkv, const AttnShape& sh, const float* rc, const float* rs, const int64_t* am, void* out, float* lse,
                          hipStream_t st);
 int attn_mfma_bwd_launch(const void* qkv, const void* out, const void* dout, const float* lse, const AttnShape& sh, const float* rc,
-                         const float* rs, const int64_t* am, void* dqkv, float* delta, float* colsum, bool* colsum_done, hipStream_t st);
+                         const float* rs, const int64_t* am, void* dqkv, float* delta, float* colsum, bool* colsum_done, hipStream_t st, int q_lo = 0);
+int attn_mfma_bwd_first_query(const AttnShape& sh, int q_lo_want);
 
 struct SuffixShape {
   int B, N, P, T, H, D, rot;
diff --git a/mafed_amd/csrc/attn.hip b/mafed_amd/csrc/attn.hip
--- a/mafed_amd/csrc/attn.hip
+++ b/mafed_amd/csrc/attn.hip
@@ -116,7 +116,7 @@
 
 static int attn_bwd_impl(const void* qkv, const void* out, const void* dout, const float* lse, mafed_dtype dtype, int B, int S, int H,
                          int D, int rot, const float* rot_cos, const float* rot_sin, const int64_t* attention_mask, int T, void* dqkv,
-                         float* delta, float* dqkv_colsum, void* stream);
+                         float* delta, float* dqkv_colsum, void* stream, int q_lo = 0);
 
 extern "C" int mafed_attn_bwd(const void* qkv, const void* out, const void* dout, const float* lse, mafed_dtype dtype, int B, int S, int H,
                               int D, int rot, const float* rot_cos, const float* rot_sin, const int64_t* attention_mask, int T, void* dqkv,
@@ -130,9 +130,23 @@
   return attn_bwd_impl(qkv, out, dout, lse, dtype, B, S, H, D, rot, rot_cos, rot_sin, attention_mask, T, dqkv, delta, dqkv_colsum, stream);
 }
 
+extern "C" int mafed_attn_bwd_first_query(mafed_dtype dtype, int B, int S, int H, int D, int rot, int T, int q_lo_want) {
+  if (dtype != MAFED_BF16 || !mfma_ok(D, rot) || B <= 0 || S <= 0 || H <= 0 || T < 0 || T > S) return 0;
+  AttnShape sh{B, S, H, D, rot, T, S - T};
+  return attn_mfma_bwd_first_query(sh, q_lo_want);
+}
+
+extern "C" int mafed_attn_bwd_from(const void* qkv, const void* out, const void* dout, const float* lse, mafed_dtype dtype, int B, int S,
+                                   int H, int D, int rot, const float* rot_cos, const float* rot_sin, const int64_t* attention_mask, int T,
+                                   void* dqkv, float* delta, float* dqkv_colsum, int q_lo, void* stream) {
+  MAFED_CHECK_ARG(q_lo == mafed_attn_bwd_first_query(dtype, B, S, H, D, rot, T, q_lo),
+                  "attn_bwd_from: q_lo=%d is not the bound this shape honours (mafed_attn_bwd_first_query)", q_lo);
+  return attn_bwd_impl(qkv, out, dout, lse, dtype, B, S, H, D, rot, rot_cos, rot_sin, attention_mask, T, dqkv, delta, dqkv_colsum, stream, q_lo);
+}
+
 static int attn_bwd_impl(const void* qkv, const void* out, const void* dout, const float* lse, mafed_dtype dtype, int B, int S, int H,
                          int D, int rot, const float* rot_cos, const float* rot_sin, const int64_t* attention_mask, int T, void* dqkv,
-                         float* delta, float* dqkv_colsum, void* stream) {
+                         float* delta, float* dqkv_colsum, void* stream, int q_lo) {
   int rc = check_common("attn_bwd", qkv, B, S, H, D, rot, rot_cos, rot_sin, attention_mask, T);
   if (rc) return rc;
   MAFED_CHECK_ARG(out && dout && lse && dqkv && delta, "attn_bwd: null pointer");
@@ -145,7 +159,7 @@
   } else if (mfma_ok(D, rot)) {
     MAFED_CHECK_ARG((((uintptr_t)qkv | (uintptr_t)out | (uintptr_t)dout | (uintptr_t)dqkv) & 15) == 0,
                     "attn_bwd(bf16): tensors must be 16-byte aligned");
-    rc = attn_mfma_bwd_launch(qkv, out, dout, lse, sh, rot_cos, rot_sin, attention_mask, dqkv, delta, dqkv_colsum, &colsum_done, st);
+    rc = attn_mfma_bwd_launch(qkv, out, dout, lse, sh, rot_cos, rot_sin, attention_mask, dqkv, delta, dqkv_colsum, &colsum_done, st, q_lo);
   } else {
     MAFED_CHECK_ARG(D <= 256, "attn_bwd(bf16): D=%d > 256", D);
     rc = attn_ref_bwd_launch<bf16_t>(qkv, out, dout, lse, sh, rot_cos, rot_sin, attention_mask, dqkv, delta, st);
diff --git a/mafed_amd/csrc/attn_mfma.hip b/mafed_amd/csrc/attn_mfma.hip
--- a/mafed_amd/csrc/attn_mfma.hip
+++ b/mafed_amd/csrc/attn_mfma.hip
@@ -600,10 +600,10 @@
 
 template <int D, int NW = 4>
 __device__ __forceinline__ void dma_rows(char* __restrict__ img, const bf16_t* __restrict__ base, int64_t rstride, int nrows, int S, int wave,
-                                         int lane) {
+                                         int lane, int lo = 0) {
   constexpr int RPP = 1024 / (2 * D);
   const int npieces = nrows / RPP;
-  for (int j = wave; j < npieces; j += NW) {
+  for (int j = (lo & ~31) / RPP + wave; j < npieces; j += NW) {
     int row, logical;
     if (D == 64) {
       row = j * 8 + (lane >> 3);
@@ -612,7 +612,7 @@
       row = j * 4 + (lane >> 4);
       logical = (lane & 15) ^ swz<128>(row);
     }
-    const int srow = row < S ? row : S - 1;
+    const int srow = row < S ? (row < lo ? lo : row) : S - 1;
     __builtin_amdgcn_global_load_lds((glb_void_ptr)(base + (int64_t)srow * rstride + logical * 8), (lds_void_ptr)(img + j * 1024), 16, 0, 0);
   }
 }
@@ -827,7 +827,7 @@
                                                               const bf16_t* __restrict__ dout, const float* __restrict__ lse, AttnShape sh,
                                                               const float* __restrict__ rc, const float* __restrict__ rs,
                                                               const int64_t* __restrict__ am, bf16_t* __restrict__ dqkv,
-                                                              float* __restrict__ delta, float* __restrict__ bsum) {
+                                                              float* __restrict__ delta, float* __restrict__ bsum, const int q_lo) {
   extern __shared__ __attribute__((aligned(16))) char lds[];
   constexpr int NTH = NW * 64;
   const int tid = threadIdx.x, lane = tid & 63;
@@ -857,12 +857,13 @@
   for (int u = 0; u < 2; ++u)
     if (tid + NTH * u < items) rot_pre_load(pre[u], tid + NTH * u, hc, rot, rc, rs);
   for (int k = tid; k < nrows; k += NTH) kbias[k] = key_ok(am, b, k, P, T, S) ? 0.f : -INFINITY;
+  const int sl_lo = q_lo >> 4;
   constexpr bool PREFETCH = NW == 4;
   ColRaw<D> qraw, doraw, oraw;
   float Lnext = 0.f;
   if (PREFETCH) {
     const int s0 = nslices - 1 - snake<NW>(wave, 0);
-    if (s0 >= 0) {
+    if (s0 >= sl_lo) {
       col_raw_issue<D, true>(qraw, qb, rstride, s0 * 16, S, rot, rc, rs, lane);
       col_raw_issue<D, false>(doraw, dob, ostride, s0 * 16, S, 0, rc, rs, lane);
       col_raw_issue<D, false>(oraw, ob, ostride, s0 * 16, S, 0, rc, rs, lane);
@@ -882,6 +883,13 @@
     if (slice < 0) break;
     const int q0 = slice * 16;
     const int myq = q0 + (lane & 15);
+    if (slice < sl_lo) {
+      bf16_t* zp = dqkv + ((int64_t)b * S * H + h) * 3 * D + (int64_t)myq * rstride;
+#pragma unroll
+      for (int dt = 0; dt < D / 16; ++dt) store4(zp + dt * 16 + 4 * (lane >> 4), make_float4(0.f, 0.f, 0.f, 0.f));
+      if ((lane >> 4) == 0) delta[((int64_t)b * H + h) * S + myq] = 0.f;
+      continue;
+    }
     if (!PREFETCH) {
       col_raw_issue<D, true>(qraw, qb, rstride, q0, S, rot, rc, rs, lane);
       col_raw_issue<D, false>(doraw, dob, ostride, q0, S, 0, rc, rs, lane);
@@ -897,7 +905,7 @@
       bf16x8 of[D / 32];
       col_raw_finish<D, false>(of, oraw, q0, S, 0, lane);
       const int nxt = nslices - 1 - snake<NW>(wave, t + 1);
-      if (PREFETCH && nxt >= 0) {
+      if (PREFETCH && nxt >= sl_lo) {
         col_raw_issue<D, true>(qraw, qb, rstride, nxt * 16, S, rot, rc, rs, lane);
         col_raw_issue<D, false>(doraw, dob, ostride, nxt * 16, S, 0, rc, rs, lane);
         col_raw_issue<D, false>(oraw, ob, ostride, nxt * 16, S, 0, rc, rs, lane);
@@ -980,7 +988,7 @@
                                                                const float* __restrict__ lse, const float* __restrict__ delta, AttnShape sh,
                                                                const float* __restrict__ rc, const float* __restrict__ rs,
                                                                const int64_t* __restrict__ am, bf16_t* __restrict__ dqkv,
-                                                               float* __restrict__ bsum) {
+                                                               float* __restrict__ bsum, const int q_lo) {
   extern __shared__ __attribute__((aligned(16))) char lds[];
   constexpr int NTH = NW * 64;
   const int tid = threadIdx.x, lane = tid & 63;
@@ -1005,7 +1013,7 @@
   const int nslices = (S + 15) / 16;
   const int hc = rot >> 4, items = S * hc;
   dma_rows<D, NW>(qimg, qb, rstride, nrows, S, wave, lane);
-  dma_rows<D, NW>(doimg, dob, ostride, nrows, S, wave, lane);
+  dma_rows<D, NW>(doimg, dob, ostride, nrows, S, wave, lane, q_lo);
   RotPre pre[2];
 #pragma unroll
   for (int u = 0; u < 2; ++u)
@@ -1049,7 +1057,6 @@
     f32x4 dk[D / 16], dv[D / 16];
 #pragma unroll
     for (int i = 0; i < D / 16; ++i) { dk[i] = (f32x4){0.f, 0.f, 0.f, 0.f}; dv[i] = (f32x4){0.f, 0.f, 0.f, 0.f}; }
-    const int qt0 = k0 / 64;
     const bool text_keys = k0 + 15 >= P;
     auto tile = [&](const int qt, const int jlo, const int jhi, auto edge_tag) {
       constexpr bool EDGE = decltype(edge_tag)::value;
@@ -1099,10 +1106,12 @@
       }
     };
     const int nfull = nrows / 64;
-    for (int qt = qt0; qt < nqt; ++qt) {
-      const int jlo = qt == qt0 ? (k0 - qt * 64) >> 4 : 0;
+    const int qs = k0 > q_lo ? k0 : q_lo;
+    const int qts = qs / 64;
+    for (int qt = qts; qt < nqt; ++qt) {
+      const int jlo = qt == qts ? (qs - qt * 64) >> 4 : 0;
       const int jhi = (nrows - qt * 64) >> 4 < 4 ? (nrows - qt * 64) >> 4 : 4;
-      if (qt == qt0 || text_keys || qt >= nfull) tile(qt, jlo, jhi, std::true_type{});
+      if (qt == qts || text_keys || qt >= nfull) tile(qt, jlo, jhi, std::true_type{});
       else tile(qt, 0, 4, std::false_type{});
     }
     bf16_t* dkp = dqkv + ((int64_t)b * S * H + h) * 3 * D + (int64_t)mykey * rstride + D;
@@ -1213,25 +1222,34 @@
   return MAFED_OK;
 }
 
+int attn_mfma_bwd_first_query(const AttnShape& sh, int q_lo_want) {
+  size_t bytes;
+  if (g_attn_variant == 1 || !attn_resident_fits(sh, &bytes) || q_lo_want <= 0) return 0;
+  return (q_lo_want < sh.S ? q_lo_want : sh.S - 1) & ~15;
+}
+
 int attn_mfma_bwd_launch(const void* qkv, const void* out, const void* dout, const float* lse, const AttnShape& sh, const float* rc,
-                         const float* rs, const int64_t* am, void* dqkv, float* delta, float* colsum, bool* colsum_done, hipStream_t st) {
+                         const float* rs, const int64_t* am, void* dqkv, float* delta, float* colsum, bool* colsum_done, hipStream_t st,
+                         int q_lo) {
   size_t bytes;
   *colsum_done = false;
+  if (q_lo != attn_mfma_bwd_first_query(sh, q_lo)) {
+    set_error("attn_bwd: first-query bound %d is not what this shape's kernels honour (mafed_attn_bwd_first_query)", q_lo);
+    return MAFED_EINVAL;
+  }
   if (g_attn_variant != 1 && attn_resident_fits(sh, &bytes)) {
     dim3 grid(sh.H, sh.B), block(256);
-    if (sh.D == 64) {
-      set_lds_attr(attn_bwd_dq_res_kernel<64>, bytes);
-      set_lds_attr(attn_bwd_dkv_res_kernel<64>, bytes);
-      launch(K_ATTN_BWD_DQ, attn_fwd_flops(sh), attn_bwd_dq_res_kernel<64>, grid, block, bytes, st, (const bf16_t*)qkv, (const bf16_t*)out, (const bf16_t*)dout, lse, sh, rc, rs, am,
-                                                             (bf16_t*)dqkv, delta, colsum);
-      launch(K_ATTN_BWD_DKV, attn_fwd_flops(sh), attn_bwd_dkv_res_kernel<64>, grid, block, bytes, st, (const bf16_t*)qkv, (const bf16_t*)dout, lse, delta, sh, rc, rs, am, (bf16_t*)dqkv, colsum);
-    } else {
-      set_lds_attr(attn_bwd_dq_res_kernel<128>, bytes);
-      set_lds_attr(attn_bwd_dkv_res_kernel<128>, bytes);
-      launch(K_ATTN_BWD_DQ, attn_fwd_flops(sh), attn_bwd_dq_res_kernel<128>, grid, block, bytes, st, (const bf16_t*)qkv, (const bf16_t*)out, (const bf16_t*)dout, lse, sh, rc, rs, am,
-                                                              (bf16_t*)dqkv, delta, colsum);
-      launch(K_ATTN_BWD_DKV, attn_fwd_flops(sh), attn_bwd_dkv_res_kernel<128>, grid, block, bytes, st, (const bf16_t*)qkv, (const bf16_t*)dout, lse, delta, sh, rc, rs, am, (bf16_t*)dqkv, colsum);
-    }
+    auto resident = [&](auto dd) {
+      constexpr int DD = decltype(dd)::value;
+      set_lds_attr(attn_bwd_dq_res_kernel<DD>, bytes);
+      set_lds_attr(attn_bwd_dkv_res_kernel<DD>, bytes);
+      launch(K_ATTN_BWD_DQ, attn_fwd_flops(sh), attn_bwd_dq_res_kernel<DD>, grid, block, bytes, st, (const bf16_t*)qkv, (const bf16_t*)out,
+             (const bf16_t*)dout, lse, sh, rc, rs, am, (bf16_t*)dqkv, delta, colsum, q_lo);
+      launch(K_ATTN_BWD_DKV, attn_fwd_flops(sh), attn_bwd_dkv_res_kernel<DD>, grid, block, bytes, st, (const bf16_t*)qkv, (const bf16_t*)dout, lse,
+             delta, sh, rc, rs, am, (bf16_t*)dqkv, colsum, q_lo);
+    };
+    if (sh.D == 64) resident(std::integral_constant<int, 64>());
+    else resident(std::integral_constant<int, 128>());
     *colsum_done = colsum != nullptr;
     return MAFED_OK;
   }
diff --git a/mafed_amd/csrc/elementwise.hip b/mafed_amd/csrc/elementwise.hip
--- a/mafed_amd/csrc/elementwise.hip
+++ b/mafed_amd/csrc/elementwise.hip
@@ -149,6 +149,43 @@
     if (dst_lp) store4(dst_lp + i * 4, v);
   }
 }
+struct TextGather {
+  const uint4* src[4];
+  uint4* dst[4];
+  int hv[4];
+  int64_t end[4];
+};
+__global__ __launch_bounds__(256) void gather_text_rows_kernel(TextGather g, int n, int S, int P, int64_t total) {
+  const int T = S - P;
+  for (int64_t i = (int64_t)blockIdx.x * 256 + threadIdx.x; i < total; i += (int64_t)gridDim.x * 256) {
+    const uint4* sp = g.src[0];
+    uint4* dp = g.dst[0];
+    int hv = g.hv[0];
+    int64_t base = 0;
+#pragma unroll
+    for (int k = 1; k < 4; ++k)
+      if (k < n && i >= g.end[k - 1]) { sp = g.src[k]; dp = g.dst[k]; hv = g.hv[k]; base = g.end[k - 1]; }
+    const int64_t j = i - base;
+    const int64_t row = j / hv;
+    const int c = (int)(j - row * hv);
+    const int64_t b = row / T;
+    const int t = (int)(row - b * T);
+    dp[j] = sp[(b * S + P + t) * (int64_t)hv + c];
+  }
+}
+__global__ __launch_bounds__(256) void scatter_text_rows_kernel(const uint4* __restrict__ src, int hv, int S, int P, int lo, int64_t total,
+                                                                uint4* __restrict__ dst) {
+  const int T = S - P, span = S - lo;
+  for (int64_t i = (int64_t)blockIdx.x * 256 + threadIdx.x; i < total; i += (int64_t)gridDim.x * 256) {
+    const int64_t row = i / hv;
+    const int c = (int)(i - row * hv);
+    const int64_t b = row / span;
+    const int s_ = lo + (int)(row - b * span);
+    uint4 v = make_uint4(0u, 0u, 0u, 0u);
+    if (s_ >= P) v = src[(b * T + (s_ - P)) * (int64_t)hv + c];
+    dst[(b * S + s_) * (int64_t)hv + c] = v;
+  }
+}
 __global__ void label_rows_kernel(const int64_t* __restrict__ labels, int B, int T, int Rc, int* __restrict__ row_of_slot,
                                   int* __restrict__ slot_of_row, int64_t* __restrict__ labels_c, int* __restrict__ overflow) {
   const int b = blockIdx.x * blockDim.x + threadIdx.x;
@@ -235,6 +272,38 @@
   return MAFED_OK;
 }
 
+extern "C" int mafed_gather_text_rows(const void* const* src, void* const* dst, const int64_t* row_bytes, int n, int B, int S, int P, void* stream) {
+  MAFED_CHECK_ARG(src && dst && row_bytes && n >= 1 && n <= 4 && B > 0 && S > 0 && P >= 0 && P < S, "gather_text_rows: bad arguments");
+  TextGather g{};
+  int64_t end = 0;
+  for (int k = 0; k < n; ++k) {
+    MAFED_CHECK_ARG(src[k] && dst[k] && row_bytes[k] > 0 && row_bytes[k] % 16 == 0 && row_bytes[k] / 16 <= 0x7fffffff,
+                    "gather_text_rows: tensor %d: null pointer or a row of %lld bytes (must fill 16-byte pieces)", k, (long long)row_bytes[k]);
+    MAFED_CHECK_ARG((((uintptr_t)src[k] | (uintptr_t)dst[k]) & 15) == 0, "gather_text_rows: tensor %d must be 16-byte aligned", k);
+    g.src[k] = (const uint4*)src[k];
+    g.dst[k] = (uint4*)dst[k];
+    g.hv[k] = (int)(row_bytes[k] / 16);
+    end += (int64_t)B * (S - P) * g.hv[k];
+    g.end[k] = end;
+  }
+  launch(K_CAST, 32.0 * end, gather_text_rows_kernel, dim3(grid_for(end)), dim3(256), 0, as_stream(stream), g, n, S, P, end);
+  MAFED_CHECK_LAUNCH("gather_text_rows");
+  return MAFED_OK;
+}
+
+extern "C" int mafed_scatter_text_rows(const void* src, int64_t row_bytes, int B, int S, int P, int lo, void* dst, void* stream) {
+  MAFED_CHECK_ARG(src && dst && B > 0 && S > 0 && P >= 0 && P < S && lo >= 0 && lo <= P, "scatter_text_rows: bad arguments");
+  MAFED_CHECK_ARG(row_bytes > 0 && row_bytes % 16 == 0 && row_bytes / 16 <= 0x7fffffff, "scatter_text_rows: a row of %lld bytes must fill 16-byte pieces",
+                  (long long)row_bytes);
+  MAFED_CHECK_ARG((((uintptr_t)src | (uintptr_t)dst) & 15) == 0, "scatter_text_rows: tensors must be 16-byte aligned");
+  const int hv = (int)(row_bytes / 16);
+  const int64_t total = (int64_t)B * (S - lo) * hv;
+  launch(K_CAST, 16.0 * ((double)total + (double)B * (S - P) * hv), scatter_text_rows_kernel, dim3(grid_for(total)), dim3(256), 0, as_stream(stream),
+         (const uint4*)src, hv, S, P, lo, total, (uint4*)dst);
+  MAFED_CHECK_LAUNCH("scatter_text_rows");
+  return MAFED_OK;
+}
+
 extern "C" int mafed_pad_text_batch(const int64_t* ids, const int64_t* mask, const int64_t* labels, int B, int T, int Tp, int64_t* ids_out,
                                     int64_t* mask_out, int64_t* labels_out, void* stream) {
   MAFED_CHECK_ARG(ids && mask && ids_out && mask_out && B > 0 && T > 0 && Tp >= T, "pad_text_batch: bad arguments");
diff --git a/mafed_amd/engine.py b/mafed_amd/engine.py
--- a/mafed_amd/engine.py
+++ b/mafed_amd/engine.py
@@ -18,6 +18,18 @@
     serial: int = 0
     filled_squares: bool = False
     dx_chain_event: Optional[torch.cuda.Event] = None
+
+
+def top_layer_text_rows(enabled: bool, from_head: bool, B: int, T: int, bf16: bool) -> bool:
+    return bool(enabled and from_head and B * T > 0 and (not bf16 or (B * T) % 128 == 0))
+
+
+def dw_group_shapes(h: int, f: int, rows: int, n_layers: int, top_rows: Optional[int] = None):
+    out = []
+    for li in range(n_layers):
+        k = top_rows if (top_rows is not None and li == 0) else rows
+        out += [(h, f, k), (h, h, k), (f, h, k), (3 * h, h, rows)]
+    return out
 
 
 class SideWork:
@@ -80,6 +92,7 @@
         self.inj_cos = bool(sv.get("inject_cosine", False))
         self.sched = SideWork(torch.cuda.current_stream(), model.side_streams() if model.overlap_param_grads else None)
         self._decide_policy()
+        self.dxt = None
         self.dx = self.dy = None
         self.dy_bias_done = False
 
@@ -95,6 +108,12 @@
         self.dw_sq = m.dw_sumsq if (self.group_dw and taps is None) else None
         if self.dw_sq is not None and not m._dw_group_fuses_squares(self.rows):
             self.dw_sq = None
+        sv = self.sv
+        self.top_rows = top_layer_text_rows(getattr(m, "top_layer_text_rows", True), sv.get("loss") is not None and sv.get("final") is not None,
+                                            self.B, self.T, self.cd == torch.bfloat16)
+        if (self.top_rows and self.group_dw and m._dw_group_fuses_squares(self.rows)
+                and not m._dw_group_fuses_squares(self.rows, self.B * self.T)):
+            self.top_rows = False
         self.record.filled_squares = self.dw_sq is not None
         self.pending_dw, self.pending_layers = [], []
         self.defer_ln = (self.sched.sides is not None and m.defer_ln_param_reduce and taps is None
@@ -177,13 +196,16 @@
         else:
             dxt, _ = ops.layernorm_bwd(dlnf, None, xt, fmean, frstd, Po.final_ln_w, None, None,
                                        Go.final_ln_w, Go.final_ln_b)
-        self.dx, self.dy = ops.pad_text_rows(dxt, B, self.S, self.P, cd if cd != torch.float32 else None)
+        if self.top_rows:
+            self.dxt = dxt
+        else:
+            self.dx, self.dy = ops.pad_text_rows(dxt, B, self.S, self.P, cd if cd != torch.float32 else None)
         sched.main_moved()
         self.ready(self.L)
 
     def layer(self, i: int) -> None:
         inj = self.inject.get(i) if self.inject else None
-        if self._gradient_into(i, inj):
+        if self.dxt is not None or self._gradient_into(i, inj):
             self._layer_backward(i, inj)
 
     def _gradient_into(self, i: int, inj) -> bool:
@@ -218,14 +240,18 @@
         H, D, rot = cfg.num_attention_heads, cfg.head_dim, cfg.rotary_ndims
         w, p = self.wts.layers[i], self.pars.layers[i]
         s = sv["layers"][i]
-        wgrad_layer(dy, s["a"], i, 3, with_bias=not dy_bias_done)
-        wgrad_layer(dy, s["ao"], i, 1, with_bias=not dy_bias_done)
-        du = ops.gemm(dy, w.fc2_w, False, False, epilogue=EPI_GELU_BWD, aux=s["u"], colsum=g.fc1_b)
-        sched.main_moved()
-        wgrad_layer(du, s["ln2"], i, 2)
-        dln2 = ops.gemm(du, w.fc1_w, False, False)
-        dao = ops.gemm(dy, w.dense_w, False, False)
-        dqkv = ops.attn_bwd(s["qkv"], s["ao"], dao, s["lse"], B, S, H, D, rot, self.cos, self.sin, am, colsum=g.qkv_b)
+        q_lo = 0
+        if self.dxt is not None:
+            dx, dln2, dao, q_lo = self._top_layer_branches(i, s, w, g)
+        else:
+            wgrad_layer(dy, s["a"], i, 3, with_bias=not dy_bias_done)
+            wgrad_layer(dy, s["ao"], i, 1, with_bias=not dy_bias_done)
+            du = ops.gemm(dy, w.fc2_w, False, False, epilogue=EPI_GELU_BWD, aux=s["u"], colsum=g.fc1_b)
+            sched.main_moved()
+            wgrad_layer(du, s["ln2"], i, 2)
+            dln2 = ops.gemm(du, w.fc1_w, False, False)
+            dao = ops.gemm(dy, w.dense_w, False, False)
+        dqkv = ops.attn_bwd(s["qkv"], s["ao"], dao, s["lse"], B, S, H, D, rot, self.cos, self.sin, am, colsum=g.qkv_b, q_lo=q_lo)
         sched.main_moved()
         wgrad_layer(dqkv, s["ln1"], i, 0)
         dln1 = ops.gemm(dqkv, w.qkv_w, False, False)
@@ -252,6 +278,24 @@
                 self.flush_dw()
         else:
             self.ready(i)
+
+    def _top_layer_branches(self, i: int, s, w, g):
+        B, S, P, cd, sched, wgrad_layer = self.B, self.S, self.P, self.cd, self.sched, self.wgrad_layer
+        dxt, self.dxt = self.dxt, None
+        dy_t = dxt if cd == torch.float32 else ops.cast(dxt, cd)
+        a_t, u_t, ao_t, ln2_t = ops.gather_text_rows([s["a"], s["u"], s["ao"], s["ln2"]], B, S, P)
+        sched.main_moved()
+        wgrad_layer(dy_t, a_t, i, 3, with_bias=True)
+        wgrad_layer(dy_t, ao_t, i, 1, with_bias=True)
+        du_t = ops.gemm(dy_t, w.fc2_w, False, False, epilogue=EPI_GELU_BWD, aux=u_t, colsum=g.fc1_b)
+        sched.main_moved()
+        wgrad_layer(du_t, ln2_t, i, 2)
+        dln2 = ops.scatter_text_rows(ops.gemm(du_t, w.fc1_w, False, False), B, S, P)
+        cfg = self.cfg
+        q_lo = ops.attn_bwd_first_query(cd, B, S, cfg.num_attention_heads, cfg.head_dim, cfg.rotary_ndims, self.T, P)
+        dao = ops.scatter_text_rows(ops.gemm(dy_t, w.dense_w, False, False), B, S, P, q_lo)
+        dx, _ = ops.pad_text_rows(dxt, B, S, P, None)
+        return dx, dln2, dao, q_lo
 
     def projector(self) -> None:
         sv, sched, dx = self.sv, self.sched, self.dx
@@ -421,15 +465,14 @@
         sv["kd"] = (t_logits, lse3, tau, lam)
         self.last_head_losses = out3
 
-    def _dw_group_fuses_squares(self, rows: int) -> bool:
+    def _dw_group_fuses_squares(self, rows: int, top_rows: Optional[int] = None) -> bool:
         cache = self._dw_fuse_cache
-        key = (int(rows), int(self.dw_group_layers or 0))
+        key = (int(rows), int(self.dw_group_layers or 0)) if top_rows is None else (int(rows), int(self.dw_group_layers or 0), int(top_rows))
         if key not in cache:
             cfg = self.config
-            h, f = cfg.hidden_size, cfg.intermediate_size
-            per_layer = [(3 * h, h, rows), (h, h, rows), (f, h, rows), (h, f, rows)]
             n_layers = max(1, min(4, key[1]))
-            cache[key] = bool(key[1]) and ops.gemm_grouped_fuses_sumsq(per_layer * n_layers, True, False)
+            shapes = dw_group_shapes(cfg.hidden_size, cfg.intermediate_size, int(rows), n_layers, top_rows)
+            cache[key] = bool(key[1]) and ops.gemm_grouped_fuses_sumsq(shapes, True, False)
         return cache[key]
 
     def _engine_backward(self, sv, dloss: Optional[torch.Tensor], dhidden: Sequence[Optional[torch.Tensor]], taps=None):
diff --git a/mafed_amd/model.py b/mafed_amd/model.py
--- a/mafed_amd/model.py
+++ b/mafed_amd/model.py
@@ -216,12 +216,13 @@
         self._tensors(1)
         self.overlap_param_grads = True
         self.dw_group_layers = 2
-        self._dw_fuse_cache: Dict[Tuple[int, int], bool] = {}
+        self._dw_fuse_cache: Dict[Tuple[int, ...], bool] = {}
         self.sparse_lm_head = True
         self.last_label_overflow: Optional[torch.Tensor] = None
         self.logit_teacher = None
         self.last_head_losses: Optional[torch.Tensor] = None
         self.defer_ln_param_reduce = True
+        self.top_layer_text_rows = True
         self.beam_trace: Optional[List[Any]] = None
         self.prefill_trace: Optional[List[Any]] = None
         self.fused_decode = True
diff --git a/mafed_amd/ops.py b/mafed_amd/ops.py
--- a/mafed_amd/ops.py
+++ b/mafed_amd/ops.py
@@ -277,11 +277,20 @@
     return out, lse
 
 
-def attn_bwd(qkv, out, dout, lse, B, S, H, D, rot, cos, sin, attention_mask, colsum: Optional[torch.Tensor] = None):
+def attn_bwd_first_query(dtype: torch.dtype, B: int, S: int, H: int, D: int, rot: int, T: int, want: int) -> int:
+    return int(_lib.load().mafed_attn_bwd_first_query(BF16 if dtype == torch.bfloat16 else F32, B, S, H, D, rot, T, int(want)))
+
+
+def attn_bwd(qkv, out, dout, lse, B, S, H, D, rot, cos, sin, attention_mask, colsum: Optional[torch.Tensor] = None, q_lo: int = 0):
     T = attention_mask.shape[1]
     dqkv = torch.empty_like(qkv)
     delta = torch.empty((B, H, S), dtype=torch.float32, device=qkv.device)
-    if colsum is None:
+    if q_lo:
+        assert colsum is None or (colsum.dtype == torch.float32 and colsum.numel() == 3 * H * D and colsum.is_contiguous())
+        check(_lib.load().mafed_attn_bwd_from(_ptr(qkv), _ptr(out), _ptr(dout), _ptr(lse), _dt(qkv), B, S, H, D, rot, _ptr(cos), _ptr(sin),
+                                              _ptr(attention_mask), T, _ptr(dqkv), _ptr(delta), _ptr(colsum), int(q_lo), _stream()),
+              "mafed_attn_bwd_from")
+    elif colsum is None:
         check(_lib.load().mafed_attn_bwd(_ptr(qkv), _ptr(out), _ptr(dout), _ptr(lse), _dt(qkv), B, S, H, D, rot, _ptr(cos), _ptr(sin),
                                          _ptr(attention_mask), T, _ptr(dqkv), _ptr(delta), _stream()), "mafed_attn_bwd")
     else:
@@ -775,6 +784,26 @@
     return dst, lp
 
 
+def gather_text_rows(srcs: Sequence[torch.Tensor], B: int, S: int, P: int):
+    n = len(srcs)
+    assert 1 <= n <= 4 and all(x.dim() == 2 and x.is_contiguous() and x.shape[0] == B * S for x in srcs)
+    dsts = [torch.empty((B * (S - P), x.shape[1]), dtype=x.dtype, device=x.device) for x in srcs]
+    sp = (C.c_void_p * n)(*[_ptr(x) for x in srcs])
+    dp = (C.c_void_p * n)(*[_ptr(x) for x in dsts])
+    rb = (C.c_int64 * n)(*[x.shape[1] * x.element_size() for x in srcs])
+    check(_lib.load().mafed_gather_text_rows(C.cast(sp, C.c_void_p), C.cast(dp, C.c_void_p), C.cast(rb, C.c_void_p), n, B, S, P, _stream()),
+          "mafed_gather_text_rows")
+    return dsts
+
+
+def scatter_text_rows(src: torch.Tensor, B: int, S: int, P: int, lo: int = 0) -> torch.Tensor:
+    assert src.dim() == 2 and src.is_contiguous() and src.shape[0] == B * (S - P) and 0 <= lo <= P
+    dst = torch.empty((B * S, src.shape[1]), dtype=src.dtype, device=src.device)
+    check(_lib.load().mafed_scatter_text_rows(_ptr(src), src.shape[1] * src.element_size(), B, S, P, lo, _ptr(dst), _stream()),
+          "mafed_scatter_text_rows")
+    return dst
+
+
 def label_rows(labels: torch.Tensor, Rc: int):
     B, T = labels.shape
     dev = labels.device
```

Measured after the change: 1014 samples/s (median of 4 runs). About the same (+0.7%).
